# YOUNESELBOUKNIFY/Ctr_recommendation

Hardware: AMD Instinct MI355X
Metric: training samples/sec (FiBiNET d=128, MicroLens-shaped synthetic, full train step) (higher is better)
Workload: dtype bf16; 1 GPU; C3: FiBiNET emb_dim=128 + item_emb_d128, batch 8192/GPU, history 20, every GEMM operand bf16 (forward and backward) / fp32 accumulation + fp32 master weights, gradients and Adam; model=MM_FiBiNET, global_batch=8192, seq_len=20, item_rows=1250000, item_rows_per_gpu=1250000, emb_dim=128, parallelism=single, hipgraph=False, launch_mode=program

## Files before the change

ctr_recommendation_amd/_lib.py:

```python
from __future__ import annotations

import contextlib
import ctypes
import os
import struct
import threading
from typing import Optional

import torch

_HERE = os.path.dirname(os.path.abspath(__file__))
LIB_PATH = os.environ.get("FBN_LIB_PATH") or os.path.join(_HERE, "libfibinet_hip.so")

P = ctypes.c_void_p
I = ctypes.c_int
LL = ctypes.c_longlong
F = ctypes.c_float
D = ctypes.c_double
SZ = ctypes.c_size_t
U = ctypes.c_uint

SIGNATURES = {
    "fbn_version": (I, []),
    "fbn_last_error": (ctypes.c_char_p, []),
    "fbn_device_ok": (I, []),
    "fbn_gemm_workspace_size": (SZ, [I, I, I, I]),
    "fbn_gemm": (I, [P, P, P, P, I, I, I, I, I, I, I, I, I, I, I, I, I, I, F, I, I, I, P, P, SZ, P]),
    "fbn_gemm_split": (I, [P, P, P, P, I, I, I, I, I, I, I, I, I, I, I, F, P, P, SZ, P, I, I, P, I, I, P]),
    "fbn_gemm_bf16out": (I, [P, P, P, I, I, I, I, I, I, I, I, P]),
    "fbn_gemm_s3": (I, [P, P, P, I, I, I, I, I, I, I, I, LL, LL, F, P, SZ, P]),
    "fbn_gemm_bn_bwd_part_supported": (I, [I, I, I, I, I, I, I]),
    "fbn_gemm_bn_bwd_part": (I, [P, P, P, I, I, I, I, I, I, I, I, P, P, P, F, P, P]),
    "fbn_bn_tile_stats": (I, [P, I, I, P, P, P]),
    "fbn_bn_tile_moments": (I, [P, I, I, P, P]),
    "fbn_bn_moments_finalize": (I, [P, D, I, P, P, P, P, F, F, I, P]),
    "fbn_bn_tile_finalize": (I, [P, I, I, D, P, P, P, P, F, F, I, P]),
    "fbn_bn_colpart_size": (SZ, [I, I]),
    "fbn_row_chunks": (I, [I]),
    "fbn_bn_bwd_chunks": (I, [I, I]),
    "fbn_bn_bwd_fused": (I, [P, P, P, P, P, F, P, P, P, P, I, I, D, P, P, P, P, P, P, P, P, P]),
    "fbn_bn_bwd_fused_img": (I, [P, P, P, P, P, F, P, P, P, P, I, I, D, P, P, P, P, P, P, P, P, P]),
    "fbn_colsum_partial": (I, [P, I, I, I, P, P]),
    "fbn_sum_jobs": (I, [P, I, P]),
    "fbn_sum_jobs2": (I, [P, I, P, I, P]),
    "fbn_sum_jobs_sq": (I, [P, I, P, I, P, I, P, P]),
    "fbn_gemm_slabs_size": (SZ, [I, I, I]),
    "fbn_gemm_slabs": (I, [P, P, I, I, I, I, I, I, I, P, SZ, P, I, I, P, I, I, P, P]),
    "fbn_gemm_slabs_split": (I, [I, I, I]),
    "fbn_gemm_slabs_group": (I, [P, I, P]),
    "fbn_gemm_slabs_group_split": (I, [I, I, I]),
    "fbn_fields_fwd": (I, [P, P, P, P, P, P, P, F, P, I, P, LL, P, P, P, P, P, I, P, P, P, P, I, I, P, P, P, P, P, I, I, I, I,
                           P]),
    "fbn_fields_fwd_hot": (I, [P, P, P, P, P, P, P, F, P, I, P, LL, P, P, P, P, I, P, P, P, P, I, I, P, P, P, P, P,
                               I, I, I, P, P, I, P]),
    "fbn_hot_rows": (I, [P, P, I, I, LL, P, P, P, I, I, I, P]),
    "fbn_fields_bwd_partials_size": (I, [I, I, I]),
    "fbn_fields_bwd_grid": (I, [I, I]),
    "fbn_fields_bwd": (I, [P, P, P, P, P, P, P, F, P, P, P, I, I, P, P, P, P, P, P, P, P, P, P, P, P, LL, P, P, I, I,
                           I, I, P]),
    "fbn_fields_bwd_img": (I, [P, P, P, P, P, P, P, F, P, P, P, I, I, P, P, P, P, P, P, P, P, P, P, P, P, LL, P, P, I,
                               I, I, I, P]),
    "fbn_fields_bwd_slot": (I, [P, P, P, P, P, P, P, F, P, P, P, I, I, P, P, P, P, P, P, P, I, P, P, P, I, LL, P, P, P,
                                LL, I, I, I, P]),
    "fbn_pairs_fwd": (I, [P, P, P, P, I, I, I, I, I, P]),
    "fbn_pairs_bwd": (I, [P, P, P, P, P, P, P, I, I, I, I, P]),
    "fbn_pairs_fwd_img": (I, [P, P, P, P, I, I, I, P]),
    "fbn_pairs_bwd_img": (I, [P, P, P, P, P, I, I, I, P]),
    "fbn_bn_workspace_size": (SZ, [I, I]),
    "fbn_bn_stats_pass": (I, [P, I, I, P, P, P, P]),
    "fbn_bn_mean": (I, [P, D, I, P, P]),
    "fbn_bn_finalize": (I, [P, P, D, I, P, P, P, P, F, F, I, P]),
    "fbn_bn_stats": (I, [P, I, I, P, P, P, P, F, F, I, P, P]),
    "fbn_bn_eval_params": (I, [P, P, P, P, I, F, P]),
    "fbn_bn_act_fwd": (I, [P, P, I, I, P, P, P, P, F, P, U, P, P, P, P]),
    "fbn_bn_act_fwd_img": (I, [P, P, I, I, P, P, P, P, F, P, U, P, P, P, P]),
    "fbn_bn_act_head_fwd": (I, [P, P, I, I, P, P, P, P, F, P, U, P, P, P, P, P, P, P, P, P, F, P, F, P]),
    "fbn_bn_bwd_reduce": (I, [P, P, P, P, F, P, P, I, I, P, P, P]),
    "fbn_bn_bwd_apply": (I, [P, P, P, P, F, P, P, P, P, I, I, P, D, P, P, P, P, P, P, P]),
    "fbn_convert_bf16": (I, [P, I, P]),
    "fbn_bn_bwd": (I, [P, P, P, P, F, P, P, P, P, I, I, P, P, P, P, P, P]),
    "fbn_colsum_workspace_size": (SZ, [I, I]),
    "fbn_colsum": (I, [P, I, I, I, P, F, P, P]),
    "fbn_head_fwd": (I, [P, P, P, I, I, P, P, P, P, P, F, P]),
    "fbn_sigmoid_bwd": (I, [P, P, P, I, P]),
    "fbn_outer": (I, [P, P, P, I, I, P]),
    "fbn_sum": (I, [P, I, P, F, P]),
    "fbn_sumsq": (I, [P, LL, P, I, P, P]),
    "fbn_clip_coef": (I, [P, F, P, P, P]),
    "fbn_adam_dense": (I, [P, P, P, P, LL, P, P, P, F, F, F, P, F, P, P, P]),
    "fbn_sparse_fixup": (I, [P, P, P, I, I, LL, I, P, P, P, P, I, I, P]),
    "fbn_sumsq_sparse": (I, [P, P, P, I, I, I, P, P]),
    "fbn_sparse_fixup_dup": (I, [P, I, P, P, P, I, I, P]),
    "fbn_sumsq_sparse_norms": (I, [P, P, P, P, I, I, I, P, P, P, LL, P]),
    "fbn_sparse_fold_fx": (I, [P, P, I, P, P, I, I, P, P]),
    "fbn_adam_table": (I, [P, P, P, LL, I, P, P, P, P, I, P, P, P, F, F, F, I, P]),
    "fbn_adam_touched": (I, [P, P, P, I, P, P, P, P, I, I, P, P, P, F, F, F, P, P]),
    "fbn_adam_catchup": (I, [P, P, P, LL, I, P, I, P, I, I, P, P, P, F, F, F, P, P, P, LL, I, I, P]),
    "fbn_adam_claim_catchup": (I, [P, P, I, I, LL, P, P, P, P, P, P, P, P, LL, I, I, P, P, P, F, F, F, P, P, P, LL, I,
                                   I, P]),
    "fbn_adam_claim_catchup_conv": (I, [P, P, I, I, LL, P, P, P, P, P, P, P, P, LL, I, I, P, P, P, F, F, F, P, P, P,
                                        LL, I, I, P, I, P]),
    "fbn_adam_flush": (I, [P, P, P, LL, I, P, P, P, F, F, F, P, P, P, LL, I, I, P]),
    "fbn_adam_prefetch_rows": (I, [P, I, I, LL, P, P, P, P, P, I, P, P, P, F, F, F, P, P, P, LL, I, I, P]),
    "fbn_adam_prefetch": (I, [P, P, I, I, LL, P, P, P, P, P, I, P, P, P, F, F, F, P, P, P, LL, I, I, P]),
    "fbn_adam_prefetch_binned_ws_size": (SZ, [LL]),
    "fbn_adam_prefetch_binned": (I, [P, P, I, I, LL, P, P, P, P, P, I, P, P, P, F, F, F, P, P, P, LL, I, I, P, SZ, P]),
    "fbn_adam_selftest": (I, [I, ctypes.c_uint, P, P]),
    "fbn_adam_step_tail": (I, [P, P, P, P, LL, P, F, P, P, P, P, P, I, P, P, P, P, I, I, P, P, F, F, F, P, P, P, P, I,
                               LL, I, P, P, P, P, I, P, P]),
    "fbn_adam_commit": (I, [P, P, P, I, P, P, P, P, I, I, P, P, P, F, F, F, P, P, P, P, I, I, P]),
    "fbn_claim_rows": (I, [P, P, I, I, LL, P, P, P, P, P]),
    "fbn_pack_extras": (I, [P, P, P, P]),
    "fbn_unpack_extras": (I, [P, P, P, P]),
    "fbn_unpack_sumsq": (I, [P, P, P, LL, P, P]),
    "fbn_step_end": (I, [P, P, P, P, P, I, P, P]),
    "fbn_route": (I, [P, P, I, I, LL, LL, I, P, P, P, P, P, P, P]),
    "fbn_route_fc": (I, [P, P, I, I, LL, LL, I, I, P, P, P, P, P]),
    "fbn_route_fc_status": (I, [P, P, I, I, I, P, P, P]),
    "fbn_ring_slot": (I, [P, I, LL, P, P, P, I, LL, P, LL, LL, P]),
    "fbn_owner_gather_self": (I, [P, I, P, P, P, P, I, I, I, P, I, I, P]),
    "fbn_adam_owner_claim_catchup": (I, [P, I, I, P, P, P, P, P, P, LL, I, I, P, P, P, F, F, F, P, P, P, LL, I, I,
                                         P]),
    "fbn_owner_fold": (I, [P, I, I, P, P, P, I, P, LL, LL, P, I, LL, P, P, P, I, P, P, P]),
    "fbn_sumsq_flagged": (I, [P, I, P, P, I, P, P, P, I, P]),
    "fbn_owner_claim": (I, [P, I, P, P, I, P]),
    "fbn_owner_gather": (I, [P, I, P, P, P, P, I, I, I, P]),
    "fbn_widen_bf16": (I, [P, P, LL, P]),
    "fbn_pad_routes": (I, [P, P, P, I, I, P, P]),
    "fbn_compact_routes": (I, [P, I, I, P, P, P]),
    "fbn_copy_jobs": (I, [P, P, P, I, P]),
    "fbn_bilinear_supported": (I, [I]),
    "fbn_bilinear_fwd": (I, [P, P, P, I, I, I, P]),
    "fbn_bilinear_bwd": (I, [P, I, I, P, P, P, P, P, I, I, P]),
    "fbn_collate": (I, [P, I, P, P, I, I, P, P, P, P, P, LL, P, P, I, P, P, P, P, P, P, P, P, P]),
    "fbn_collate_zero_if": (I, [P, LL, P, P]),
    "fbn_eval_pack": (I, [P, P, LL, P, P, P]),
    "fbn_eval_workspace_size": (SZ, [LL]),
    "fbn_eval_reduce": (I, [P, LL, P, SZ, P, P, P]),
    "fbn_sort_u64_workspace_size": (SZ, [LL]),
    "fbn_sort_u64": (I, [P, LL, I, P, SZ, P, P]),
    "fbn_eval_pack_groups": (I, [P, LL, P, P, P]),
    "fbn_gauc_workspace_size": (SZ, [LL]),
    "fbn_gauc_reduce": (I, [P, P, LL, P, SZ, P, P, P, P]),
    "fbn_calib_workspace_size": (SZ, [LL]),
    "fbn_calib_reduce": (I, [P, LL, I, P, SZ, P, P, P]),
    "fbn_rec_item_cache": (I, [P, P, P, P, P, P, F, I, LL, P, P, I, I, P]),
    "fbn_rec_hist_pool": (I, [P, P, LL, P, P, I, I, I, P]),
    "fbn_rec_fields": (I, [P, P, P, P, P, P, I, P, LL, P, P, P, P, I, P, P, P, I, I, P, P, I, I, I, I, P]),
    "fbn_rec_topk_workspace_size": (SZ, [I, I, I]),
    "fbn_rec_topk": (I, [P, I, I, I, P, P, I, I, I, P, P, SZ, P, P, P, P, P, P]),
    "fbn_rec_rank": (I, [P, I, I, I, P, P, I, I, P, P, P, P, P]),
    "fbn_rank_hist": (I, [P, LL, P, P]),
    "fbn_rec_fields_list": (I, [P, P, P, P, P, P, I, P, LL, P, P, P, P, I, P, P, P, I, I, P, P, I, P, I, I, I, I, I, P]),
    "fbn_rec_topk_list": (I, [P, I, I, I, P, I, I, P, P, I, I, I, P, P, SZ, P, P, P, P, P, P, P]),
    "fbn_rec_rank_list": (I, [P, I, I, I, P, I, I, P, P, I, I, P, P, P, P, P]),
    "fbn_plan_create": (I, [P]),
    "fbn_plan_destroy": (I, [P]),
    "fbn_plan_size": (I, [P]),
    "fbn_plan_add_call": (I, [P, ctypes.c_char_p, P, I, P, I]),
    "fbn_plan_add_record": (I, [P, I, P]),
    "fbn_plan_add_wait": (I, [P, P, I]),
    "fbn_plan_run": (I, [P, P]),
    "fbn_plan_event_sync": (I, [P, I]),
    "fbn_probe_arm": (I, [I]),
    "fbn_probe_disarm": (I, []),
    "fbn_probe_elapsed": (F, [I]),
    "fbn_comm_load": (I, [ctypes.c_char_p]),
    "fbn_comm_id_bytes": (I, []),
    "fbn_comm_unique_id": (I, [P]),
    "fbn_comm_init": (I, [P, P, I, I]),
    "fbn_comm_destroy": (I, [P]),
    "fbn_comm_alltoallv": (I, [P, P, P, P, P, LL, P]),
    "fbn_comm_alltoall_peers": (I, [P, P, P, LL, P]),
    "fbn_comm_alltoall": (I, [P, P, P, LL, P]),
    "fbn_comm_allreduce": (I, [P, P, LL, I, P]),
    "fbn_comm_allgather": (I, [P, P, P, LL, P]),
    "fbn_sum_slices": (I, [P, I, LL, I, P, P]),
    "fbn_comm_watch": (I, [LL]),
    "fbn_comm_heartbeat": (I, [P]),
    "fbn_comm_abort": (I, [P]),
    "fbn_comm_watchdog_fired": (I, [P]),
}

FBN_SORT_TILE = 2048
FBN_GAUC_REC_WORDS = 8
FBN_CALIB_MAX_BINS = 1024
FBN_CALIB_BIN_WORDS = 8

_lib: Optional[ctypes.CDLL] = None


def lib() -> ctypes.CDLL:
    global _lib
    if _lib is None:
        if not os.path.exists(LIB_PATH):
            raise RuntimeError(
                f"{LIB_PATH} is missing: build it with `python -m ctr_recommendation_amd.build` "
                "(the FiBiNET path has no CPU fallback)")
        h = ctypes.CDLL(LIB_PATH)
        for name, (res, args) in SIGNATURES.items():
            fn = getattr(h, name)
            fn.restype = res
            fn.argtypes = args
        _lib = h
    return _lib


_fns = {}
_UNCHECKED = ("fbn_version", "fbn_device_ok", "fbn_probe_elapsed", "fbn_comm_watchdog_fired")
_tls = threading.local()


_DEBUG_SYNC = os.environ.get("FBN_DEBUG_SYNC")
_debug_log = None


def _debug_sync(name: str) -> None:
    global _debug_log
    if _debug_log is None:
        _debug_log = open(_DEBUG_SYNC, "a", buffering=1)
    _debug_log.write(name + "\n")
    torch.cuda.synchronize()


def call(name: str, *args) -> int:
    f = _fns.get(name)
    if f is None:
        f = _fns[name] = getattr(lib(), name)
    if _DEBUG_SYNC:
        _debug_sync("> " + name)
    rc = f(*args)
    if _DEBUG_SYNC:
        _debug_sync("< " + name)
    if rc and isinstance(rc, int) and name not in _UNCHECKED and not name.endswith(("_size", "_grid")):
        msg = lib().fbn_last_error().decode(errors="replace")
        raise RuntimeError(f"{name} failed (code {rc}): {msg}")
    prog = getattr(_tls, "prog", None)
    if prog is not None:
        prog.add_call(name, f, args)
    return rc


def keep(obj) -> None:
    prog = getattr(_tls, "prog", None)
    if prog is not None:
        prog.keep.append(obj)


def recording() -> bool:
    return getattr(_tls, "prog", None) is not None


def persistent(fn):
    prog = getattr(_tls, "prog", None)
    if prog is None:
        return fn()
    stream = torch.cuda.current_stream(prog.device)
    box = {}

    def run():
        try:
            torch.cuda.set_device(prog.device)
            with torch.cuda.stream(stream):
                box["out"] = fn()
        except BaseException as e:
            box["err"] = e

    t = threading.Thread(target=run, name="fbn-persistent-alloc")
    t.start()
    t.join()
    if "err" in box:
        raise box["err"]
    return box["out"]


def pool_segments(pool) -> list:
    pid = tuple(pool.id)
    out = []
    for seg in torch.cuda.memory_snapshot():
        if tuple(seg.get("segment_pool_id", ())) == pid:
            out.append((int(seg["address"]), int(seg["address"]) + int(seg["total_size"])))
    return sorted(out)


def tensors_of(obj, _seen=None, _path="", _depth=0):
    seen = set() if _seen is None else _seen
# ... 192 lines not shown
```

ctr_recommendation_amd/csrc/bilinear.hip:

```cpp
#include "common.h"
#include <algorithm>

namespace {

constexpr int TS = 16;

template <int D>
__device__ __forceinline__ int swz(int r, int k) {
  constexpr int CH = D / 8;
  return r * D + ((((k >> 3) ^ (r % CH))) << 3) + (k & 7);
}

template <int D> constexpr int nthreads() { return D >= 32 ? 2 * D : 64; }
template <int D> constexpr int row_blocks() { return D >= 32 ? 2 : 1; }

template <int D, int NT>
struct WStage {
  static constexpr int CH = D / 8, TOT = D * CH, N = (TOT + NT - 1) / NT;
  bf16x8 v[N];
  __device__ __forceinline__ void load(const short* __restrict__ src, int tid) {
#pragma unroll
    for (int j = 0; j < N; ++j)
      if (TOT % NT == 0 || tid + j * NT < TOT) v[j] = *reinterpret_cast<const bf16x8*>(src + (size_t)(tid + j * NT) * 8);
  }
  __device__ __forceinline__ void store(short* __restrict__ img, int tid) const {
#pragma unroll
    for (int j = 0; j < N; ++j) {
      const int i = tid + j * NT, r = i / CH, c = i % CH;
      if (TOT % NT == 0 || i < TOT) *reinterpret_cast<bf16x8*>(img + swz<D>(r, c * 8)) = v[j];
    }
  }
};
template <int D, int NT>
__device__ __forceinline__ void stage_w(short* __restrict__ img, const short* __restrict__ src, int tid) {
  WStage<D, NT> w;
  w.load(src, tid);
  w.store(img, tid);
}

template <int D, int NT>
__device__ __forceinline__ void stage_v(short* __restrict__ img, const short* __restrict__ V16, int b0, int ns,
                                        int tid) {
  constexpr int CH = D / 8, TOT = TS * 5 * CH, N = (TOT + NT - 1) / NT;
  const short* src = V16 + (size_t)b0 * 5 * D;
  bf16x8 v[N];
#pragma unroll
  for (int j = 0; j < N; ++j) {
    const int i = tid + j * NT, m = i / CH;
    v[j] = (bf16x8){0, 0, 0, 0, 0, 0, 0, 0};
    if ((TOT % NT == 0 || i < TOT) && m / 5 < ns) v[j] = *reinterpret_cast<const bf16x8*>(src + (size_t)i * 8);
  }
#pragma unroll
  for (int j = 0; j < N; ++j) {
    const int i = tid + j * NT, m = i / CH, c = i % CH;
    if (TOT % NT == 0 || i < TOT) *reinterpret_cast<bf16x8*>(img + swz<D>((m % 5) * TS + m / 5, c * 8)) = v[j];
  }
}

template <int D>
__device__ __forceinline__ bf16x8 frag(const short* img, int row, int k) {
  return *reinterpret_cast<const bf16x8*>(img + swz<D>(row, k));
}

template <int D>
__device__ __forceinline__ void mfma_5(f32x4 (&acc)[row_blocks<D>()][5], const short* A, const short* Bt, int w,
                                       int lane) {
  const int lr = lane & 15, lq = lane >> 4;
  if constexpr (D == 16) {
    const bf16x4 a = *reinterpret_cast<const bf16x4*>(A + swz<D>(lr, 4 * lq));
#pragma unroll
    for (int f = 0; f < 5; ++f) {
      const bf16x4 b = *reinterpret_cast<const bf16x4*>(Bt + swz<D>(f * TS + lr, 4 * lq));
      acc[0][f] = __builtin_amdgcn_mfma_f32_16x16x16bf16_1k(a, b, acc[0][f], 0, 0, 0);
    }
    return;
  }
#pragma unroll
  for (int ks = 0; ks < D / 32; ++ks) {
    bf16x8 b[5];
#pragma unroll
    for (int f = 0; f < 5; ++f) b[f] = frag<D>(Bt, f * TS + lr, 32 * ks + 8 * lq);
#pragma unroll
    for (int rb = 0; rb < 2; ++rb) {
      const bf16x8 a = frag<D>(A, 32 * w + 16 * rb + lr, 32 * ks + 8 * lq);
#pragma unroll
      for (int f = 0; f < 5; ++f) acc[rb][f] = __builtin_amdgcn_mfma_f32_16x16x32_bf16(a, b[f], acc[rb][f], 0, 0, 0);
    }
  }
}

__device__ __forceinline__ f32x4 ld_bf4(const short* p) {
  const bf16x4 t = *reinterpret_cast<const bf16x4*>(p);
  return (f32x4){bf2f(t[0]), bf2f(t[1]), bf2f(t[2]), bf2f(t[3])};
}
__device__ __forceinline__ bf16x4 to_bf4(const f32x4& v) { return (bf16x4){f2bf(v[0]), f2bf(v[1]), f2bf(v[2]), f2bf(v[3])}; }

constexpr int PI[10] = {0, 0, 0, 0, 1, 1, 1, 2, 2, 3};
constexpr int PJ[10] = {1, 2, 3, 4, 2, 3, 4, 3, 4, 4};

template <int D>
__global__ void __launch_bounds__(nthreads<D>()) bilinear_fwd_kernel(const short* __restrict__ V16,
                                                                    const short* __restrict__ WT16,
                                                                    short* __restrict__ c, int B, int ldc) {
  FBN_MAIN_PRIO();
  constexpr int NT = nthreads<D>(), RB = row_blocks<D>();
  __shared__ __attribute__((aligned(16))) short sV[5 * TS * D];
  __shared__ __attribute__((aligned(16))) short sW[D * D];
  const int tid = threadIdx.x, lane = tid & 63, w = tid >> 6;
  const int b0 = blockIdx.x * TS, ns = min(TS, B - b0);
  stage_v<D, NT>(sV, V16, b0, ns, tid);
  stage_w<D, NT>(sW, WT16, tid);
  __syncthreads();
  f32x4 acc[RB][5];
#pragma unroll
  for (int rb = 0; rb < RB; ++rb)
#pragma unroll
    for (int f = 0; f < 5; ++f) acc[rb][f] = (f32x4){0.f, 0.f, 0.f, 0.f};
  mfma_5<D>(acc, sW, sV, w, lane);
  const int s = lane & 15, lq = lane >> 4;
  if (s >= ns) return;
  short* crow = c + (size_t)(b0 + s) * ldc + 5 * D;
#pragma unroll
  for (int rb = 0; rb < RB; ++rb) {
    const int n0 = 32 * w + 16 * rb + 4 * lq;
    f32x4 v[4];
#pragma unroll
    for (int i = 0; i < 4; ++i) v[i] = ld_bf4(sV + swz<D>(i * TS + s, n0));
#pragma unroll
    for (int k = 0; k < 10; ++k) *reinterpret_cast<bf16x4*>(crow + k * D + n0) = to_bf4(v[PI[k]] * acc[rb][PJ[k]]);
  }
}

template <bool DC16>
__device__ __forceinline__ f32x4 ld_dc4(const void* __restrict__ row, int off) {
  if constexpr (DC16) return ld_bf4(reinterpret_cast<const short*>(row) + off);
  else return *reinterpret_cast<const f32x4*>(reinterpret_cast<const float*>(row) + off);
}

template <int D, bool DC16>
__global__ void __launch_bounds__(nthreads<D>(), 2) bilinear_bwd_kernel(const void* __restrict__ dc, int ldc,
                                                                       const short* __restrict__ V16,
                                                                       const short* __restrict__ WT16,
                                                                       const short* __restrict__ W16,
                                                                       float* __restrict__ dV,
                                                                       short* __restrict__ dU16, int B) {
  FBN_MAIN_PRIO();
  constexpr int NT = nthreads<D>(), RB = row_blocks<D>();
  __shared__ __attribute__((aligned(16))) short sV[5 * TS * D];
  __shared__ __attribute__((aligned(16))) short sW[D * D];
  const int tid = threadIdx.x, lane = tid & 63, w = tid >> 6;
  const int b0 = blockIdx.x * TS, ns = min(TS, B - b0);
  stage_v<D, NT>(sV, V16, b0, ns, tid);
  stage_w<D, NT>(sW, WT16, tid);
  __syncthreads();
  WStage<D, NT> wnext;
  wnext.load(W16, tid);
  f32x4 acc[RB][5];
#pragma unroll
  for (int rb = 0; rb < RB; ++rb)
#pragma unroll
    for (int f = 0; f < 5; ++f) acc[rb][f] = (f32x4){0.f, 0.f, 0.f, 0.f};
  mfma_5<D>(acc, sW, sV, w, lane);
  __syncthreads();
  const int s = lane & 15, lq = lane >> 4;
  const bool live = s < ns;
  const char* dcr = reinterpret_cast<const char*>(dc) + (size_t)(b0 + (live ? s : 0)) * ldc * (DC16 ? 2 : 4);
#pragma unroll
  for (int rb = 0; rb < RB; ++rb) {
    const int n0 = 32 * w + 16 * rb + 4 * lq;
    f32x4 v[5], gv[5], gu[5];
#pragma unroll
    for (int f = 0; f < 5; ++f) {
      v[f] = ld_bf4(sV + swz<D>(f * TS + s, n0));
      gv[f] = live ? ld_dc4<DC16>(dcr, f * D + n0) : (f32x4){0.f, 0.f, 0.f, 0.f};
      gu[f] = (f32x4){0.f, 0.f, 0.f, 0.f};
    }
#pragma unroll
    for (int k = 0; k < 10; ++k) {
      const f32x4 gp = live ? ld_dc4<DC16>(dcr, (5 + k) * D + n0) : (f32x4){0.f, 0.f, 0.f, 0.f};
      gv[PI[k]] += gp * acc[rb][PJ[k]];
      gu[PJ[k]] += gp * v[PI[k]];
    }
#pragma unroll
    for (int f = 0; f < 5; ++f) {
      const bf16x4 t = to_bf4(gu[f]);
      *reinterpret_cast<bf16x4*>(sV + swz<D>(f * TS + s, n0)) = t;
      if (live) *reinterpret_cast<bf16x4*>(dU16 + ((size_t)(b0 + s) * 5 + f) * D + n0) = t;
    }
#pragma unroll
    for (int f = 0; f < 5; ++f) acc[rb][f] = gv[f];
  }
  __syncthreads();
  wnext.store(sW, tid);
  __syncthreads();
  mfma_5<D>(acc, sW, sV, w, lane);
  if (!live) return;
#pragma unroll
  for (int rb = 0; rb < RB; ++rb) {
    const int k0 = 32 * w + 16 * rb + 4 * lq;
#pragma unroll
    for (int f = 0; f < 5; ++f) *reinterpret_cast<f32x4*>(dV + ((size_t)(b0 + s) * 5 + f) * D + k0) = acc[rb][f];
  }
}

}

extern "C" int fbn_bilinear_supported(int D) { return D == 16 || D == 32 || D == 64 || D == 128; }

extern "C" int fbn_bilinear_fwd(const short* V16, const short* WT16, short* c, int B, int D, int ldc, void* stream) {
  if (B <= 0) return FBN_OK;
  if (!V16 || !WT16 || !c || (ldc & 3) || ((uintptr_t)V16 & 15) || ((uintptr_t)WT16 & 15) || ((uintptr_t)c & 7)) {
    fbn_set_error("fbn_bilinear_fwd: bf16 V, W^T, c required; 16-B aligned V / W^T, 8-B aligned c, ldc % 4 == 0");
    return FBN_ERR_ARG;
  }
  const dim3 grid((unsigned)((B + TS - 1) / TS));
  hipStream_t st = (hipStream_t)stream;
  switch (D) {
    case 128: fbn_launch(bilinear_fwd_kernel<128>, grid, dim3(256), 0, st, V16, WT16, c, B, ldc); break;
    case 64: fbn_launch(bilinear_fwd_kernel<64>, grid, dim3(128), 0, st, V16, WT16, c, B, ldc); break;
    case 32: fbn_launch(bilinear_fwd_kernel<32>, grid, dim3(64), 0, st, V16, WT16, c, B, ldc); break;
    case 16: fbn_launch(bilinear_fwd_kernel<16>, grid, dim3(64), 0, st, V16, WT16, c, B, ldc); break;
    default: fbn_set_error("fbn_bilinear_fwd: D must be 16, 32, 64 or 128"); return FBN_ERR_UNSUPPORTED;
  }
  FBN_CHECK_LAUNCH();
  return FBN_OK;
}

extern "C" int fbn_bilinear_bwd(const void* dc, int ldc, int dc_bf16, const short* V16, const short* WT16,
                                const short* W16, float* dV, short* dU16, int B, int D, void* stream) {
  if (B <= 0) return FBN_OK;
  if (!dc || !V16 || !WT16 || !W16 || !dV || !dU16 || (ldc & 3) || ((uintptr_t)dc & 7) || ((uintptr_t)dV & 15) ||
      ((uintptr_t)V16 & 15) || ((uintptr_t)WT16 & 15) || ((uintptr_t)W16 & 15) || ((uintptr_t)dU16 & 7)) {
    fbn_set_error("fbn_bilinear_bwd: all operands required and aligned (16 B; dc, dU16 8 B), ldc % 4 == 0");
    return FBN_ERR_ARG;
  }
  const dim3 grid((unsigned)((B + TS - 1) / TS));
  hipStream_t st = (hipStream_t)stream;
  if (!dc_bf16 && ((uintptr_t)dc & 15)) { fbn_set_error("fbn_bilinear_bwd: f32 dc must be 16-B aligned"); return FBN_ERR_ARG; }
#define FBN_BILINEAR_BWD(DD, NTH)                                                                              \
  if (dc_bf16)                                                                                               \
    fbn_launch((bilinear_bwd_kernel<DD, true>), grid, dim3(NTH), 0, st, dc, ldc, V16, WT16, W16, dV, dU16, B); \
  else                                                                                                       \
    fbn_launch((bilinear_bwd_kernel<DD, false>), grid, dim3(NTH), 0, st, dc, ldc, V16, WT16, W16, dV, dU16, B)
  switch (D) {
    case 128: FBN_BILINEAR_BWD(128, 256); break;
    case 64: FBN_BILINEAR_BWD(64, 128); break;
    case 32: FBN_BILINEAR_BWD(32, 64); break;
    case 16: FBN_BILINEAR_BWD(16, 64); break;
    default: fbn_set_error("fbn_bilinear_bwd: D must be 16, 32, 64 or 128"); return FBN_ERR_UNSUPPORTED;
  }
#undef FBN_BILINEAR_BWD
  FBN_CHECK_LAUNCH();
  return FBN_OK;
}
```

ctr_recommendation_amd/csrc/fields.hip:

```cpp
#include <cstdlib>
#include "common.h"
#include "fields_common.h"

#ifndef FBN_HCH
#define FBN_HCH 10
#endif

struct FieldArgs {
  const int64_t* item_id;
  const int64_t* item_seq;
  const int64_t* likes;
  const int64_t* views;
  const float* hmm;
  const float* ln_g;
  const float* ln_b;
  const float* cate;
  const float* table;
  const int* pos;
  const float* w1; const float* b1; const float* w2; const float* b2;
  float* X;
  float* Vc;
  short* Vc16;
  void* c;
  float* a_out;
// ... 79 lines not shown
    const f32x4 c1 = *reinterpret_cast<const f32x4*>(p.cate + lk * D + 4 * q);
    const f32x4 c2 = *reinterpret_cast<const f32x4*>(p.cate + vw * D + 4 * q);
    const f32x4 h = *reinterpret_cast<const f32x4*>(p.hmm + (size_t)b * D + 4 * q);
    f32x4 rit = {0.f, 0.f, 0.f, 0.f};
    f32x4 hs = {0.f, 0.f, 0.f, 0.f};
    int nnz = 0;
    const int* pb = MODE >= 1 ? p.pos + (size_t)b * (L + 1) : nullptr;
    if (MODE == 0) {
      if (item < 0 || item >= p.V) { bad = true; item = -1; }
      if (item >= 0) rit = *reinterpret_cast<const f32x4*>(p.table + item * D + 4 * q);
    } else {
      const int pi = pb[0];
      if (pi >= 0) rit = load_row<D, MODE>(p, pi, q);
    }
    constexpr int IPL = (FBN_MAX_L + G - 1) / G;
    int sid[IPL];
#pragma unroll
    for (int j = 0; j < IPL; ++j) {
      const int t = q + j * G;
      int r = -1;
      if (t < L) {
        if (MODE == 0) {
          long long s = p.item_seq[(size_t)b * L + t];
          if (s < 0 || s >= p.V) { bad = true; s = 0; }
          r = s != 0 ? (int)s : -1;
        } else {
          r = pb[t + 1];
        }
      }
      sid[j] = r;
    }
    const int gbase = lane - q;
    if constexpr (CMP) {
      constexpr int SPB = 4 * SPW;
      __shared__ int lid[SPB][FBN_MAX_L];
      int* mine = lid[(threadIdx.x >> 6) * SPW + lane / G];
      const unsigned long long gmask = (G == 64 ? ~0ull : ((1ull << G) - 1)) << gbase;
      int nl = 0;
#pragma unroll
      for (int j = 0; j < IPL; ++j) {
        const unsigned long long mk = __ballot(sid[j] >= 0) & gmask;
        const int below = __popcll(mk & ((1ull << lane) - 1));
        if (sid[j] >= 0) mine[nl + below] = sid[j];
        nl += __popcll(mk);
      }
      __builtin_amdgcn_wave_barrier();
      __atomic_signal_fence(__ATOMIC_SEQ_CST);
      int nch = (nl + HCH - 1) / HCH;
#pragma unroll
      for (int o = 32; o > 0; o >>= 1) nch = max(nch, __shfl_xor(nch, o, 64));
      for (int c = 0; c < nch; ++c) {
        f32x4 hist[HCH];
        bool live[HCH];
#pragma unroll
        for (int u = 0; u < HCH; ++u) {
          const int k = c * HCH + u;
          live[u] = k < nl;
          const int r = mine[live[u] ? k : 0];
          if constexpr (BUF) {
            const unsigned off = live[u] ? ((unsigned)r * D + 4 * q) * 4u : 0xFFFFFFF0u;
            hist[u] = __builtin_bit_cast(f32x4, __builtin_amdgcn_raw_buffer_load_b128(rs, off, 0, 0));
          } else {
            hist[u] = load_row<D, MODE>(p, live[u] ? r : 0, q);
          }
        }
#pragma unroll
        for (int u = 0; u < HCH; ++u) hs += live[u] ? hist[u] : (f32x4){0.f, 0.f, 0.f, 0.f};
      }
      nnz = nl;
      __builtin_amdgcn_wave_barrier();
      __atomic_signal_fence(__ATOMIC_SEQ_CST);
    }
    for (int t0 = 0; t0 < (CMP ? 0 : L); t0 += HCH) {
      f32x4 hist[HCH];
      bool live[HCH];
#pragma unroll
      for (int u = 0; u < HCH; ++u) {
        const int t = t0 + u;
        int r = -1;
#pragma unroll
        for (int j = 0; j < IPL; ++j)
          if ((t / G) == j) r = __shfl(sid[j], gbase + (t % G), 64);
        live[u] = t < L && r >= 0;
        if constexpr (HOT) {
          int hi = -1;
          if (live[u] && nh > 0) {
            const unsigned h = hot_hash(r) >> (32 - __builtin_ctz(HT));
#pragma unroll
            for (int k = 0; k < 2; ++k) {
              const unsigned hk = (h + k) & (HT - 1);
              if (hi < 0 && hkey[hk] == r) hi = hval[hk];
            }
          }
          const unsigned off = (live[u] && hi < 0) ? ((unsigned)r * D + 4 * q) * 4u : 0xFFFFFFF0u;
          hist[u] = __builtin_bit_cast(f32x4, __builtin_amdgcn_raw_buffer_load_b128(rs, off, 0, 0));
          if (hi >= 0) hist[u] = hrow[hi * (D / 4) + q];
        } else if constexpr (BUF) {
          const unsigned off = live[u] ? ((unsigned)r * D + 4 * q) * 4u : 0xFFFFFFF0u;
          hist[u] = __builtin_bit_cast(f32x4, __builtin_amdgcn_raw_buffer_load_b128(rs, off, 0, 0));
        } else {
          hist[u] = load_row<D, MODE>(p, live[u] ? r : 0, q);
        }
      }
#pragma unroll
      for (int u = 0; u < HCH; ++u) {
        hs += live[u] ? hist[u] : (f32x4){0.f, 0.f, 0.f, 0.f};
        nnz += live[u] ? 1 : 0;
      }
    }
    if (bad) atomicOr(p.err, 1);

    const float cnt = fmaxf((float)nnz, 1.f);
    f32x4 x5 = hs / cnt;

    const f32x4 x4 = ln_relu<G>(h, p.ln_g, p.ln_b, p.ln_eps, q);

    const f32x4 xs[5] = {c1, c2, rit, x4, x5};
    float z[6];
    z[0] = 0.f;
#pragma unroll
    for (int f = 0; f < 5; ++f) z[f + 1] = group_sum<G>(xs[f][0] + xs[f][1] + xs[f][2] + xs[f][3]) / (float)D;
    float qv[FBN_MAXR], a[6];
    senet_excite<D>(z, p.w1, p.b1, p.w2, p.b2, p.R, qv, a);

    float* Xb = p.X + (size_t)b * 2 * D + 4 * q;
    *reinterpret_cast<f32x4*>(Xb) = rit;
    *reinterpret_cast<f32x4*>(Xb + D) = x5;
    float* Vb = p.Vc ? p.Vc + (size_t)b * 5 * D + 4 * q : nullptr;
    float* cb = (p.c && !p.c16) ? (float*)p.c + (size_t)b * p.ldc + 4 * q : nullptr;
    short* cb16 = (p.c && p.c16) ? (short*)p.c + (size_t)b * p.ldc + 4 * q : nullptr;
#pragma unroll
    for (int f = 0; f < 5; ++f) {
      const f32x4 v = xs[f] * a[f + 1];
      if (p.Vc) *reinterpret_cast<f32x4*>(Vb + f * D) = v;
      const bf16x4 v16 = (bf16x4){f2bf(v[0]), f2bf(v[1]), f2bf(v[2]), f2bf(v[3])};
      if (cb16) *reinterpret_cast<bf16x4*>(cb16 + f * D) = v16;
      else if (cb) *reinterpret_cast<f32x4*>(cb + f * D) = v;
      if (p.Vc16) *reinterpret_cast<bf16x4*>(p.Vc16 + ((size_t)b * 5 + f) * D + 4 * q) = v16;
    }
#pragma unroll
    for (int f = 0; f < 6; ++f)
      if (f % G == q) p.a_out[(size_t)b * 6 + f] = a[f];
    if (q == 0) p.cnt_out[b] = cnt;

    if (MODE == 0 && p.map) {
      for (int t = q; t <= L; t += G) {
        long long r = (t == 0) ? item : p.item_seq[(size_t)b * L + (t - 1)];
        if (r > 0 && r < p.V) map_claim(p.map, p.slot_row, (int)r, b * (L + 1) + t);
      }
    }
  }
}

struct FieldBwdArgs {
  const int64_t* item_id; const int64_t* item_seq; const int64_t* likes; const int64_t* views;
  const float* hmm; const float* ln_g;
  const float* w1; const float* b1; const float* w2;
  const float* X;
  const float* cate;
  const float* ln_b;
  const float* a;
  const float* cnt;
  const float* dV;
  float* dhmm;
  short* dhmm16;
  long long dhmm16_lo;
  float* partials;
  float* gtab; float* gvec;
  double* gnorm;
  const int* slot_step; float** slot_cell; long long ring_stride; int ring_n;
  const int* pos; void* sendbuf;
  long long V;
  int B, L, R, n_cate;
  float ln_eps;
};

template <int G>
__device__ __forceinline__ f32x4 transpose_cols(const f32x4& v, int lane) {
  const int base = lane - lane % G, q = lane % G;
  f32x4 t;
#pragma unroll
  for (int e = 0; e < 4; ++e) {
    const int src = base + e * (G / 4) + q / 4;
    const float x0 = __shfl(v[0], src, 64), x1 = __shfl(v[1], src, 64);
    const float x2 = __shfl(v[2], src, 64), x3 = __shfl(v[3], src, 64);
    const int c = q & 3;
    t[e] = c == 0 ? x0 : (c == 1 ? x1 : (c == 2 ? x2 : x3));
  }
  return t;
}
template <int G>
__device__ __forceinline__ void atomic_add_row_t(float* row, const f32x4& t, int q) {
  atomicAdd(row + q, t[0]); atomicAdd(row + G + q, t[1]); atomicAdd(row + 2 * G + q, t[2]);
  atomicAdd(row + 3 * G + q, t[3]);
}

template <int D, int MODE, int RMAX, bool SLOT = false>
__global__ void __launch_bounds__(256) fields_bwd_kernel(FieldBwdArgs p) {
  FBN_MAIN_PRIO();
  constexpr int G = D / 4;
  constexpr int SPW = 64 / G;
  constexpr int NPMAX = 13 * RMAX + 6;
  constexpr int SJ = (NPMAX + G - 1) / G;
  extern __shared__ __attribute__((aligned(16))) float sp[];
  const int R = p.R;
  const int NP = 13 * R + 6;
  const int P = NP + 3 * D + p.n_cate * D;
  const int wave = threadIdx.x >> 6;
  float* ws = sp + wave * P;
  float* sv = sp + 4 * P + (wave * SPW + (threadIdx.x & 63) / G) * (12 + 2 * RMAX);
  for (int i = threadIdx.x; i < 4 * P; i += blockDim.x) sp[i] = 0.f;
  __syncthreads();
  float* w_lg = ws + NP;
  float* w_ct = w_lg + 2 * D;
  float* w_hb = w_ct + p.n_cate * D;

  const int lane = threadIdx.x & 63;
  const int q = lane % G, grp = lane / G;
  const int gw = (blockIdx.x * blockDim.x + threadIdx.x) >> 6;
  const int nwaves = (gridDim.x * blockDim.x) >> 6;
  const int L = p.L;
  float* gvec = p.gvec;
  if constexpr (SLOT) {
    gvec += (size_t)(__builtin_amdgcn_readfirstlane(*p.slot_step) % p.ring_n) * p.ring_stride;
    if (blockIdx.x == 0 && threadIdx.x == 0) *p.slot_cell = gvec;
  }
  f32x4 acc_lg = {0.f, 0.f, 0.f, 0.f}, acc_lb = {0.f, 0.f, 0.f, 0.f}, acc_hb = {0.f, 0.f, 0.f, 0.f};
  float acc_se[SJ];
#pragma unroll
  for (int j = 0; j < SJ; ++j) acc_se[j] = 0.f;

  for (int b0 = gw * SPW; b0 < p.B; b0 += nwaves * SPW) {
    const int b = b0 + grp;
    const bool live = b < p.B;
    f32x4 dx0 = {0.f, 0.f, 0.f, 0.f}, dx1 = {0.f, 0.f, 0.f, 0.f};
    long long lk = -1, vw = -1;
    if (live) {
      const float* Xb = p.X + (size_t)b * 2 * D + 4 * q;
      const float* dVb = p.dV + (size_t)b * 5 * D + 4 * q;
      f32x4 x[5], dv[5];
      lk = p.likes[b];
      vw = p.views[b];
      const long long lkc = (lk >= 0 && lk < p.n_cate) ? lk : 0, vwc = (vw >= 0 && vw < p.n_cate) ? vw : 0;
      x[0] = *reinterpret_cast<const f32x4*>(p.cate + lkc * D + 4 * q);
      x[1] = *reinterpret_cast<const f32x4*>(p.cate + vwc * D + 4 * q);
      x[2] = *reinterpret_cast<const f32x4*>(Xb);
      x[4] = *reinterpret_cast<const f32x4*>(Xb + D);
#pragma unroll
      for (int f = 0; f < 5; ++f) dv[f] = *reinterpret_cast<const f32x4*>(dVb + f * D);
      const f32x4 h = *reinterpret_cast<const f32x4*>(p.hmm + (size_t)b * D + 4 * q);
      x[3] = ln_relu<G>(h, p.ln_g, p.ln_b, p.ln_eps, q);
      float a[6];
#pragma unroll
      for (int f = 0; f < 6; ++f) a[f] = p.a[(size_t)b * 6 + f];
      float z[6];
      z[0] = 0.f;
#pragma unroll
      for (int f = 0; f < 5; ++f) z[f + 1] = group_sum<G>(x[f][0] + x[f][1] + x[f][2] + x[f][3]) / (float)D;
      float qv[RMAX], rj[RMAX], dq[RMAX];
#pragma unroll
      for (int j = 0; j < RMAX; ++j) {
        float s = 0.f;
        if (j < R) {
          s = p.b1[j];
#pragma unroll
          for (int f = 0; f < 6; ++f) s += p.w1[j * 6 + f] * z[f];
        }
        qv[j] = s;
        rj[j] = fmaxf(s, 0.f);
      }
      float ds[6];
      ds[0] = 0.f;
#pragma unroll
      for (int f = 0; f < 5; ++f) {
        const float da = group_sum<G>(dv[f][0] * x[f][0] + dv[f][1] * x[f][1] + dv[f][2] * x[f][2] + dv[f][3] * x[f][3]);
        ds[f + 1] = da * (1.f - a[f + 1]) * a[f + 1];
      }
      float dz[6] = {0.f, 0.f, 0.f, 0.f, 0.f, 0.f};
#pragma unroll
      for (int j = 0; j < RMAX; ++j) {
        float dr = 0.f;
        if (j < R) {
#pragma unroll
          for (int f = 0; f < 6; ++f) dr += p.w2[f * R + j] * ds[f];
        }
        dq[j] = (j < R && qv[j] > 0.f) ? dr : 0.f;
        if (j < R) {
#pragma unroll
          for (int f = 0; f < 6; ++f) dz[f] += p.w1[j * 6 + f] * dq[j];
        }
      }
      if (q == 0) {
#pragma unroll
        for (int f = 0; f < 6; ++f) { sv[f] = ds[f]; sv[6 + f] = z[f]; }
#pragma unroll
        for (int jj = 0; jj < RMAX; ++jj) { sv[12 + jj] = dq[jj]; sv[12 + RMAX + jj] = rj[jj]; }
      }
      __builtin_amdgcn_wave_barrier();
#pragma unroll
      for (int j = 0; j < SJ; ++j) {
        const int k = q + j * G;
        float v = 0.f;
        if (k < 6 * R) v = sv[12 + k / 6] * sv[6 + k % 6];
        else if (k < 7 * R) v = sv[12 + (k - 6 * R)];
        else if (k < 13 * R) v = sv[(k - 7 * R) / R] * sv[12 + RMAX + (k - 7 * R) % R];
        else if (k < NP) v = sv[k - 13 * R];
        acc_se[j] += v;
      }
      __builtin_amdgcn_wave_barrier();
      f32x4 dx[5];
#pragma unroll
      for (int f = 0; f < 5; ++f) dx[f] = dv[f] * a[f + 1] + dz[f + 1] / (float)D;
      dx0 = dx[0];
      dx1 = dx[1];

      {
        const float mean = group_sum<G>(h[0] + h[1] + h[2] + h[3]) / (float)D;
        const f32x4 dh = h - mean;
        const float s2 = group_sum<G>(dh[0] * dh[0] + dh[1] * dh[1] + dh[2] * dh[2] + dh[3] * dh[3]);
        const float rstd = 1.f / sqrtf(s2 / (float)D + p.ln_eps);
        const f32x4 gam = *reinterpret_cast<const f32x4*>(p.ln_g + 4 * q);
        f32x4 gl, xh, gx;
#pragma unroll
        for (int e = 0; e < 4; ++e) {
          gl[e] = x[3][e] > 0.f ? dx[3][e] : 0.f;
          xh[e] = dh[e] * rstd;
          gx[e] = gl[e] * gam[e];
          acc_lg[e] += gl[e] * xh[e];
          acc_lb[e] += gl[e];
        }
        const float m1 = group_sum<G>(gx[0] + gx[1] + gx[2] + gx[3]) / (float)D;
        const float m2 = group_sum<G>(gx[0] * xh[0] + gx[1] * xh[1] + gx[2] * xh[2] + gx[3] * xh[3]) / (float)D;
        f32x4 out;
#pragma unroll
        for (int e = 0; e < 4; ++e) out[e] = rstd * (gx[e] - m1 - xh[e] * m2);
        *reinterpret_cast<f32x4*>(p.dhmm + (size_t)b * D + 4 * q) = out;
        acc_hb += out;
        if (p.dhmm16) {
          const bf16x4 hi = (bf16x4){f2bf(out[0]), f2bf(out[1]), f2bf(out[2]), f2bf(out[3])};
          *reinterpret_cast<bf16x4*>(p.dhmm16 + (size_t)b * D + 4 * q) = hi;
          if (p.dhmm16_lo)
            *reinterpret_cast<bf16x4*>(p.dhmm16 + p.dhmm16_lo + (size_t)b * D + 4 * q) =
                (bf16x4){f2bf(out[0] - bf2f(hi[0])), f2bf(out[1] - bf2f(hi[1])), f2bf(out[2] - bf2f(hi[2])),
                         f2bf(out[3] - bf2f(hi[3]))};
        }
      }
      const f32x4 gh = dx[4] / p.cnt[b];
      if (MODE == 0 && p.gvec) {
        *reinterpret_cast<f32x4*>(gvec + (size_t)b * 2 * D + 4 * q) = dx[2];
        *reinterpret_cast<f32x4*>(gvec + ((size_t)b * 2 + 1) * D + 4 * q) = gh;
        if (p.gnorm) {
          double si = 0.0, sh = 0.0;
#pragma unroll
          for (int e = 0; e < 4; ++e) {
            si += (double)(dx[2][e] * dx[2][e]);
            sh += (double)(gh[e] * gh[e]);
          }
#pragma unroll
          for (int o = G / 2; o > 0; o >>= 1) {
            si += __shfl_xor(si, o, 64);
            sh += __shfl_xor(sh, o, 64);
          }
          if (q == 0) {
            p.gnorm[(size_t)b * 2] = si;
            p.gnorm[(size_t)b * 2 + 1] = sh;
          }
        }
      } else if (MODE == 0) {
        const f32x4 ti = transpose_cols<G>(dx[2], lane);
        const f32x4 th = transpose_cols<G>(gh, lane);
        const long long item = p.item_id[b];
        if (item > 0 && item < p.V) atomic_add_row_t<G>(p.gtab + item * D, ti, q);
        for (int t = 0; t < L; ++t) {
          const long long s = p.item_seq[(size_t)b * L + t];
          if (s > 0 && s < p.V) atomic_add_row_t<G>(p.gtab + s * D, th, q);
        }
      } else {
        const int* pb = p.pos + (size_t)b * (L + 1);
        auto put = [&](int row, const f32x4& x) {
          if constexpr (MODE == 2) {
            *reinterpret_cast<bf16x4*>(reinterpret_cast<short*>(p.sendbuf) + (size_t)row * D + 4 * q) =
                (bf16x4){f2bf(x[0]), f2bf(x[1]), f2bf(x[2]), f2bf(x[3])};
          } else {
            *reinterpret_cast<f32x4*>(reinterpret_cast<float*>(p.sendbuf) + (size_t)row * D + 4 * q) = x;
          }
        };
        if (pb[0] >= 0) put(pb[0], dx[2]);
        for (int t = 0; t < L; ++t)
          if (pb[t + 1] >= 0) put(pb[t + 1], gh);
      }
    }
#pragma unroll
    for (int gi = 0; gi < SPW; ++gi) {
      if (grp == gi && live) {
        if (lk >= 0 && lk < p.n_cate) {
          f32x4* c = reinterpret_cast<f32x4*>(w_ct + lk * D + 4 * q);
          *c = *c + dx0;
        }
        if (vw >= 0 && vw < p.n_cate) {
          f32x4* c = reinterpret_cast<f32x4*>(w_ct + vw * D + 4 * q);
          *c = *c + dx1;
        }
      }
    }
  }
#pragma unroll
  for (int o = G; o < 64; o <<= 1) {
#pragma unroll
    for (int e = 0; e < 4; ++e) {
      acc_lg[e] += __shfl_xor(acc_lg[e], o, 64);
      acc_lb[e] += __shfl_xor(acc_lb[e], o, 64);
      acc_hb[e] += __shfl_xor(acc_hb[e], o, 64);
    }
#pragma unroll
    for (int j = 0; j < SJ; ++j) acc_se[j] += __shfl_xor(acc_se[j], o, 64);
  }
  if (grp == 0) {
    *reinterpret_cast<f32x4*>(w_lg + 4 * q) = acc_lg;
    *reinterpret_cast<f32x4*>(w_lg + D + 4 * q) = acc_lb;
    *reinterpret_cast<f32x4*>(w_hb + 4 * q) = acc_hb;
#pragma unroll
    for (int j = 0; j < SJ; ++j) {
      const int k = q + j * G;
      if (k < NP) ws[k] = acc_se[j];
    }
  }
  __syncthreads();
  float* out = p.partials + (size_t)blockIdx.x * P;
  for (int i = threadIdx.x; i < P; i += blockDim.x) out[i] = (sp[i] + sp[P + i]) + (sp[2 * P + i] + sp[3 * P + i]);
}

struct GradOuts {
  float* p[8];
  int off[9];
};
__global__ void __launch_bounds__(1024) reduce_partials_one16(const float* __restrict__ part, int nblk, int P, GradOuts o) {
  __shared__ float red[64][16];
  const int col = threadIdx.x & 15, str = threadIdx.x >> 4;
  const int i = blockIdx.x * 16 + col;
  float s = 0.f;
  if (i < P)
    for (int r = str; r < nblk; r += 64) s += part[(size_t)r * P + i];
  red[str][col] = s;
  __syncthreads();
  if (threadIdx.x < 16 && i < P) {
    float t = 0.f;
    for (int k = 0; k < 64; ++k) t += red[k][col];
    int seg = 0;
#pragma unroll
    for (int j = 1; j < 8; ++j) seg += (i >= o.off[j]) ? 1 : 0;
    if (o.p[seg]) o.p[seg][i - o.off[seg]] = t;
  }
}


#ifndef FBN_FB_MAXBLK
#define FBN_FB_MAXBLK 512
#endif
static int fields_grid(int B, int D, int cap = 1024) {
  const int spw = 64 / (D / 4);
  const int waves = (B + spw - 1) / spw;
  int blocks = (waves + 3) / 4;
  return blocks < 1 ? 1 : (blocks > cap ? cap : blocks);
}

template <int MODE, int HCH, bool BUF, bool HOT = false, bool CMP = false>
static int launch_fields_fwd_hb(const FieldArgs& a, int D, hipStream_t st) {
  const int grid = fields_grid(a.B, D, HOT ? 256 : 1024);
  switch (D) {
    case 16: fbn_launch((fields_fwd_kernel<16, MODE, HCH, BUF, HOT, CMP>), dim3(grid), dim3(256), 0, st, a); break;
    case 32: fbn_launch((fields_fwd_kernel<32, MODE, HCH, BUF, HOT, CMP>), dim3(grid), dim3(256), 0, st, a); break;
    case 64: fbn_launch((fields_fwd_kernel<64, MODE, HCH, BUF, HOT, CMP>), dim3(grid), dim3(256), 0, st, a); break;
    case 128: fbn_launch((fields_fwd_kernel<128, MODE, HCH, BUF, HOT, CMP>), dim3(grid), dim3(256), 0, st, a); break;
    case 256: fbn_launch((fields_fwd_kernel<256, MODE, HCH, BUF, HOT, CMP>), dim3(grid), dim3(256), 0, st, a); break;
    default: fbn_set_error("fields: embedding_dim must be one of 16,32,64,128,256"); return FBN_ERR_UNSUPPORTED;
  }
  FBN_CHECK_LAUNCH();
  return FBN_OK;
}

template <int MODE, int HCH, bool CMP>
static int launch_fields_fwd_h(const FieldArgs& a, int D, hipStream_t st) {
  if constexpr (MODE == 0) {
    if (a.hot) return launch_fields_fwd_hb<0, HCH, true, true>(a, D, st);
    if ((unsigned long long)a.V * D * 4 < 0xFFFFFF00ull)
      return launch_fields_fwd_hb<0, HCH, true, false, CMP>(a, D, st);
  }
  return launch_fields_fwd_hb<MODE, HCH, false, false, CMP>(a, D, st);
}

template <int MODE>
static int launch_fields_fwd(const FieldArgs& a, int D, hipStream_t st) {
  const char* he = getenv("FBN_FIELDS_HCH");
  const int hch = he ? atoi(he) : FBN_HCH;
  const char* ce = getenv("FBN_FIELDS_CMP");
  if (ce && atoi(ce) == 1) {
    if (hch == 10) return launch_fields_fwd_h<MODE, 10, true>(a, D, st);
    if (hch == 8) return launch_fields_fwd_h<MODE, 8, true>(a, D, st);
    return launch_fields_fwd_h<MODE, 5, true>(a, D, st);
  }
  if (hch == 20) return launch_fields_fwd_h<MODE, 20, false>(a, D, st);
  if (hch == 5) return launch_fields_fwd_h<MODE, 5, false>(a, D, st);
  return launch_fields_fwd_h<MODE, 10, false>(a, D, st);
}

static int fields_fwd_impl(const int64_t* item_id, const int64_t* item_seq, const int64_t* likes,
                           const int64_t* views, const float* hmm, const float* ln_g, const float* ln_b,
                           float ln_eps, const float* cate, int n_cate, const float* table, long long V,
                           const int* pos, const float* w1, const float* b1, const float* w2,
                           const float* b2, int R, float* X, float* Vc, short* Vc16, void* c, int ldc, int c_bf16,
                           float* a_out, float* cnt_out, int* err, int* map, int* slot_row, int B, int L,
                           int D, int rows_bf16, const int* hot, const int* hot_n, int H, void* stream);

extern "C" int fbn_fields_fwd(const int64_t* item_id, const int64_t* item_seq, const int64_t* likes,
                              const int64_t* views, const float* hmm, const float* ln_g, const float* ln_b,
                              float ln_eps, const float* cate, int n_cate, const float* table, long long V,
                              const int* pos, const float* w1, const float* b1, const float* w2,
                              const float* b2, int R, float* X, float* Vc, short* Vc16, void* c, int ldc, int c_bf16,
                              float* a_out,
                              float* cnt_out, int* err, int* map, int* slot_row, int B, int L,
                              int D, int rows_bf16, void* stream) {
  return fields_fwd_impl(item_id, item_seq, likes, views, hmm, ln_g, ln_b, ln_eps, cate, n_cate, table, V, pos, w1,
                         b1, w2, b2, R, X, Vc, Vc16, c, ldc, c_bf16, a_out, cnt_out, err, map, slot_row, B, L, D,
                         rows_bf16, nullptr, nullptr, 0, stream);
}

extern "C" int fbn_fields_fwd_hot(const int64_t* item_id, const int64_t* item_seq, const int64_t* likes,
                                  const int64_t* views, const float* hmm, const float* ln_g, const float* ln_b,
                                  float ln_eps, const float* cate, int n_cate, const float* table, long long V,
                                  const float* w1, const float* b1, const float* w2, const float* b2, int R, float* X,
                                  float* Vc, short* Vc16, void* c, int ldc, int c_bf16, float* a_out, float* cnt_out,
                                  int* err, int* map, int* slot_row, int B, int L, int D, const int* hot,
                                  const int* hot_n, int H, void* stream) {
  if (!hot || !hot_n || (unsigned long long)V * D * 4 >= 0xFFFFFF00ull) {
    fbn_set_error("fbn_fields_fwd_hot: needs the hot list and a table under 4 GB");
    return FBN_ERR_ARG;
  }
  return fields_fwd_impl(item_id, item_seq, likes, views, hmm, ln_g, ln_b, ln_eps, cate, n_cate, table, V, nullptr,
                         w1, b1, w2, b2, R, X, Vc, Vc16, c, ldc, c_bf16, a_out, cnt_out, err, map, slot_row, B, L, D, 0,
                         hot, hot_n, H, stream);
}

__global__ void hot_rows_kernel(const int64_t* __restrict__ item, const int64_t* __restrict__ seq, int B, int L,
                                long long V, int* __restrict__ cnt, int* __restrict__ hot, int* __restrict__ hot_n,
                                int H, int tau, int clear) {
  const long long i = (long long)blockIdx.x * blockDim.x + threadIdx.x;
  if (clear && i == 0) *hot_n = 0;
  if (i >= (long long)B * (L + 1)) return;
  const long long b = i / (L + 1), t = i - b * (L + 1);
  const long long id = t == 0 ? item[b] : seq[b * L + (t - 1)];
  if (id <= 0 || id >= V) return;
  if (clear) {
    cnt[id] = 0;
    return;
  }
  if (atomicAdd(cnt + id, 1) == tau - 1) {
    const int s = atomicAdd(hot_n, 1);
    if (s < H) hot[s] = (int)id;
  }
}

extern "C" int fbn_hot_rows(const int64_t* item, const int64_t* seq, int B, int L, long long V, int* cnt, int* hot,
                            int* hot_n, int H, int tau, int clear, void* stream) {
  const long long n = (long long)B * (L + 1);
  if (n <= 0) return FBN_OK;
  fbn_launch(hot_rows_kernel, dim3((unsigned)((n + 255) / 256)), dim3(256), 0, (hipStream_t)stream, item,
                     L > 0 ? seq : nullptr, B, L, V, cnt, hot, hot_n, H, tau < 1 ? 1 : tau, clear);
  FBN_CHECK_LAUNCH();
  return FBN_OK;
}

static int fields_fwd_impl(const int64_t* item_id, const int64_t* item_seq, const int64_t* likes,
                           const int64_t* views, const float* hmm, const float* ln_g, const float* ln_b,
                           float ln_eps, const float* cate, int n_cate, const float* table, long long V,
                           const int* pos, const float* w1, const float* b1, const float* w2,
                           const float* b2, int R, float* X, float* Vc, short* Vc16, void* c, int ldc, int c_bf16,
                           float* a_out, float* cnt_out, int* err, int* map, int* slot_row, int B, int L,
                           int D, int rows_bf16, const int* hot, const int* hot_n, int H, void* stream) {
  if (B <= 0) return FBN_OK;
  if (L < 0 || L > 32 || R < 1 || R > FBN_MAXR || (ldc & 3)) {
    fbn_set_error("fbn_fields_fwd: need 0 <= L <= 32, 1 <= R <= 8, ldc % 4 == 0");
    return FBN_ERR_ARG;
  }
  FieldArgs a;
  a.item_id = item_id; a.item_seq = L > 0 ? item_seq : nullptr; a.likes = likes; a.views = views;
  a.hmm = hmm; a.ln_g = ln_g; a.ln_b = ln_b; a.cate = cate; a.table = table; a.pos = pos;
  a.w1 = w1; a.b1 = b1; a.w2 = w2; a.b2 = b2;
  a.X = X; a.Vc = Vc; a.Vc16 = Vc16; a.c = c; a.a_out = a_out; a.cnt_out = cnt_out; a.err = err;
  a.map = map; a.slot_row = slot_row;
  a.V = V; a.B = B; a.L = L; a.ldc = ldc; a.R = R; a.n_cate = n_cate; a.ln_eps = ln_eps; a.c16 = c_bf16;
  a.hot = hot; a.hot_n = hot_n; a.H = H;
  if (pos && rows_bf16) return launch_fields_fwd<2>(a, D, (hipStream_t)stream);
  if (pos) return launch_fields_fwd<1>(a, D, (hipStream_t)stream);
  return launch_fields_fwd<0>(a, D, (hipStream_t)stream);
}

extern "C" int fbn_fields_bwd_partials_size(int D, int R, int n_cate) { return 13 * R + 6 + 3 * D + n_cate * D; }
extern "C" int fbn_fields_bwd_grid(int B, int D) { return fields_grid(B, D, FBN_FB_MAXBLK); }

template <int MODE, int RMAX, bool SLOT = false>
static int launch_fields_bwd_r(const FieldBwdArgs& a, int D, hipStream_t st) {
  const int grid = fields_grid(a.B, D, FBN_FB_MAXBLK);
  const size_t lds = (4 * (size_t)(13 * a.R + 6 + 3 * D + a.n_cate * D) + 4 * (64 / (D / 4)) * (12 + 2 * RMAX)) *
                     sizeof(float);
  switch (D) {
    case 16: fbn_launch((fields_bwd_kernel<16, MODE, RMAX, SLOT>), dim3(grid), dim3(256), lds, st, a); break;
    case 32: fbn_launch((fields_bwd_kernel<32, MODE, RMAX, SLOT>), dim3(grid), dim3(256), lds, st, a); break;
    case 64: fbn_launch((fields_bwd_kernel<64, MODE, RMAX, SLOT>), dim3(grid), dim3(256), lds, st, a); break;
    case 128: fbn_launch((fields_bwd_kernel<128, MODE, RMAX, SLOT>), dim3(grid), dim3(256), lds, st, a); break;
    case 256: fbn_launch((fields_bwd_kernel<256, MODE, RMAX, SLOT>), dim3(grid), dim3(256), lds, st, a); break;
    default: fbn_set_error("fields: embedding_dim must be one of 16,32,64,128,256"); return FBN_ERR_UNSUPPORTED;
  }
  FBN_CHECK_LAUNCH();
  return FBN_OK;
}

template <int MODE>
static int launch_fields_bwd(const FieldBwdArgs& a, int D, hipStream_t st) {
  if constexpr (MODE == 0)
    if (a.slot_step)
      return a.R <= 3 ? launch_fields_bwd_r<0, 3, true>(a, D, st) : launch_fields_bwd_r<0, FBN_MAXR, true>(a, D, st);
  return a.R <= 3 ? launch_fields_bwd_r<MODE, 3>(a, D, st) : launch_fields_bwd_r<MODE, FBN_MAXR>(a, D, st);
}

static int fields_bwd_impl(const int64_t* item_id, const int64_t* item_seq, const int64_t* likes,
                           const int64_t* views, const float* hmm, const float* ln_g, const float* ln_b,
                           float ln_eps, const float* w1, const float* b1, const float* w2, int R, int n_cate,
                           const float* cate, const float* X, const float* a, const float* cnt, const float* dV,
                           float* dhmm, short* dhmm16, float* partials, float* const* param_grads, float* gtab,
                           float* gvec, double* gnorm, long long V, const int* pos, void* sendbuf, int send_bf16,
                           int B, int L, int D, void* stream, long long dhmm16_lo, const int* slot_step = nullptr,
                           void* slot_cell = nullptr, int ring_n = 0, long long ring_stride = 0);
extern "C" int fbn_fields_bwd(const int64_t* item_id, const int64_t* item_seq, const int64_t* likes,
                              const int64_t* views, const float* hmm, const float* ln_g, const float* ln_b,
                              float ln_eps, const float* w1, const float* b1, const float* w2, int R, int n_cate,
                              const float* cate, const float* X, const float* a, const float* cnt, const float* dV, float* dhmm,
                              short* dhmm16, float* partials, float* const* param_grads, float* gtab, float* gvec,
                              double* gnorm, long long V, const int* pos, void* sendbuf, int send_bf16, int B,
                              int L, int D, void* stream) {
  return fields_bwd_impl(item_id, item_seq, likes, views, hmm, ln_g, ln_b, ln_eps, w1, b1, w2, R, n_cate, cate, X, a,
                         cnt, dV, dhmm, dhmm16, partials, param_grads, gtab, gvec, gnorm, V, pos, sendbuf, send_bf16, B,
                         L, D, stream, 0);
}
extern "C" int fbn_fields_bwd_img(const int64_t* item_id, const int64_t* item_seq, const int64_t* likes,
                                  const int64_t* views, const float* hmm, const float* ln_g, const float* ln_b,
                                  float ln_eps, const float* w1, const float* b1, const float* w2, int R, int n_cate,
                                  const float* cate, const float* X, const float* a, const float* cnt, const float* dV,
                                  float* dhmm, void* dhmm_img, float* partials, float* const* param_grads,
                                  float* gtab, float* gvec, double* gnorm, long long V, const int* pos, void* sendbuf,
                                  int send_bf16, int B, int L, int D, void* stream) {
  if (!dhmm_img) { fbn_set_error("fbn_fields_bwd_img: dhmm_img"); return FBN_ERR_ARG; }
  return fields_bwd_impl(item_id, item_seq, likes, views, hmm, ln_g, ln_b, ln_eps, w1, b1, w2, R, n_cate, cate, X, a,
                         cnt, dV, dhmm, (short*)dhmm_img, partials, param_grads, gtab, gvec, gnorm, V, pos, sendbuf,
                         send_bf16, B, L, D, stream, (long long)B * D);
}
extern "C" int fbn_fields_bwd_slot(const int64_t* item_id, const int64_t* item_seq, const int64_t* likes,
                                   const int64_t* views, const float* hmm, const float* ln_g, const float* ln_b,
                                   float ln_eps, const float* w1, const float* b1, const float* w2, int R, int n_cate,
                                   const float* cate, const float* X, const float* a, const float* cnt, const float* dV,
                                   float* dhmm, void* dhmm16, int dhmm_is_img, float* partials,
                                   float* const* param_grads, float* ring, int ring_n, long long ring_stride,
                                   const int* step, void* cell, double* gnorm, long long V, int B, int L, int D,
                                   void* stream) {
  if (!ring || !step || !cell || ring_n < 1 || ring_stride < (long long)B * 2 * D || (ring_stride & 3) ||
      ((uintptr_t)ring & 15) || (dhmm_is_img && !dhmm16)) {
    fbn_set_error("fbn_fields_bwd_slot: ring (16-B aligned), step, cell; ring_n >= 1, ring_stride >= B*2*D, % 4 == 0");
    return FBN_ERR_ARG;
  }
  return fields_bwd_impl(item_id, item_seq, likes, views, hmm, ln_g, ln_b, ln_eps, w1, b1, w2, R, n_cate, cate, X, a,
                         cnt, dV, dhmm, (short*)dhmm16, partials, param_grads, nullptr, ring, gnorm, V, nullptr, nullptr,
                         0, B, L, D, stream, dhmm_is_img ? (long long)B * D : 0, step, cell, ring_n, ring_stride);
}
static int fields_bwd_impl(const int64_t* item_id, const int64_t* item_seq, const int64_t* likes,
                           const int64_t* views, const float* hmm, const float* ln_g, const float* ln_b,
                           float ln_eps, const float* w1, const float* b1, const float* w2, int R, int n_cate,
                           const float* cate, const float* X, const float* a, const float* cnt, const float* dV,
                           float* dhmm, short* dhmm16, float* partials, float* const* param_grads, float* gtab,
                           float* gvec, double* gnorm, long long V, const int* pos, void* sendbuf, int send_bf16,
                           int B, int L, int D, void* stream, long long dhmm16_lo, const int* slot_step,
                           void* slot_cell, int ring_n, long long ring_stride) {
  if (B <= 0) return FBN_OK;
  if (L < 0 || L > 32 || R < 1 || R > FBN_MAXR) { fbn_set_error("fbn_fields_bwd: bad L/R"); return FBN_ERR_ARG; }
  FieldBwdArgs p;
  p.item_id = item_id; p.item_seq = L > 0 ? item_seq : nullptr; p.likes = likes; p.views = views;
  p.hmm = hmm; p.ln_g = ln_g; p.ln_b = ln_b; p.w1 = w1; p.b1 = b1; p.w2 = w2; p.cate = cate;
  p.X = X; p.a = a; p.cnt = cnt; p.dV = dV; p.dhmm = dhmm; p.dhmm16 = dhmm16; p.partials = partials;
  p.dhmm16_lo = dhmm16_lo;
  p.slot_step = slot_step; p.slot_cell = (float**)slot_cell; p.ring_n = ring_n; p.ring_stride = ring_stride;
  p.gtab = gtab; p.gvec = gvec; p.gnorm = gvec ? gnorm : nullptr; p.pos = pos; p.sendbuf = sendbuf;
  p.V = V; p.B = B; p.L = L; p.R = R; p.n_cate = n_cate; p.ln_eps = ln_eps;
  hipStream_t st = (hipStream_t)stream;
  int rc = !pos ? launch_fields_bwd<0>(p, D, st) : send_bf16 ? launch_fields_bwd<2>(p, D, st)
                                                               : launch_fields_bwd<1>(p, D, st);
  if (rc) return rc;
  if (!param_grads) return FBN_OK;
  const int P = 13 * R + 6 + 3 * D + n_cate * D;
  const int nblk = fields_grid(B, D, FBN_FB_MAXBLK);

  GradOuts o;
  const int sizes[8] = {6 * R, R, 6 * R, 6, D, D, n_cate * D, D};
  o.off[0] = 0;
  for (int j = 0; j < 8; ++j) {
    if (j < 7 && !param_grads[j]) {
      fbn_set_error("fbn_fields_bwd: null parameter-gradient destination");
      return FBN_ERR_ARG;
    }
    o.p[j] = param_grads[j];
    o.off[j + 1] = o.off[j] + sizes[j];
  }
  fbn_launch(reduce_partials_one16, dim3(fbn_cdiv(P, 16)), dim3(1024), 0, st, (const float*)partials, nblk, P, o);
  FBN_CHECK_LAUNCH();
  return FBN_OK;
}
```

ctr_recommendation_amd/csrc/fields_common.h:

```cpp
#pragma once
#include "common.h"

#define FBN_MAXR 8
#define FBN_MAX_L 32

template <int G>
__device__ __forceinline__ f32x4 ln_relu(const f32x4& h, const float* ln_g, const float* ln_b, float eps, int q) {
  constexpr int D = 4 * G;
  const float s1 = group_sum<G>(h[0] + h[1] + h[2] + h[3]);
  const float mean = s1 / (float)D;
  const f32x4 dh = h - mean;
  const float s2 = group_sum<G>(dh[0] * dh[0] + dh[1] * dh[1] + dh[2] * dh[2] + dh[3] * dh[3]);
  const float rstd = 1.f / sqrtf(s2 / (float)D + eps);
  const f32x4 g4 = *reinterpret_cast<const f32x4*>(ln_g + 4 * q);
  const f32x4 bb4 = *reinterpret_cast<const f32x4*>(ln_b + 4 * q);
  f32x4 x4;
#pragma unroll
  for (int e = 0; e < 4; ++e) x4[e] = fmaxf(dh[e] * rstd * g4[e] + bb4[e], 0.f);
  return x4;
}

template <int D>
__device__ __forceinline__ void senet_excite(const float (&z)[6], const float* w1, const float* b1,
                                             const float* w2, const float* b2, int R, float (&q)[FBN_MAXR],
                                             float (&a)[6]) {
  for (int j = 0; j < R; ++j) {
    float s = b1[j];
#pragma unroll
    for (int f = 0; f < 6; ++f) s += w1[j * 6 + f] * z[f];
    q[j] = s;
  }
#pragma unroll
  for (int f = 0; f < 6; ++f) {
    float s = b2[f];
    for (int j = 0; j < R; ++j) s += w2[f * R + j] * fmaxf(q[j], 0.f);
    a[f] = 1.f / (1.f + __expf(-s));
  }
}
```

ctr_recommendation_amd/csrc/plan_thunks.inc:

```

static int th_fbn_adam_catchup(const uint64_t* i, const double* f) {
  return fbn_adam_catchup(reinterpret_cast<float*>(static_cast<uintptr_t>(i[0])),
      reinterpret_cast<float*>(static_cast<uintptr_t>(i[1])),
      reinterpret_cast<float*>(static_cast<uintptr_t>(i[2])),
      static_cast<long long>(i[3]),
      static_cast<int>(i[4]),
      reinterpret_cast<const int*>(static_cast<uintptr_t>(i[5])),
      static_cast<int>(i[6]),
      reinterpret_cast<const int*>(static_cast<uintptr_t>(i[7])),
      static_cast<int>(i[8]),
      static_cast<int>(i[9]),
      reinterpret_cast<int*>(static_cast<uintptr_t>(i[10])),
      reinterpret_cast<const void*>(static_cast<uintptr_t>(i[11])),
      reinterpret_cast<const int*>(static_cast<uintptr_t>(i[12])),
      plan_f32(f[0]),
      plan_f32(f[1]),
      plan_f32(f[2]),
      reinterpret_cast<int*>(static_cast<uintptr_t>(i[13])),
      reinterpret_cast<const float*>(static_cast<uintptr_t>(i[14])),
      reinterpret_cast<const float*>(static_cast<uintptr_t>(i[15])),
      static_cast<long long>(i[16]),
      static_cast<int>(i[17]),
      static_cast<int>(i[18]),
      reinterpret_cast<void*>(static_cast<uintptr_t>(i[19])));
// ... 182 lines not shown
  return fbn_adam_prefetch_binned(reinterpret_cast<const int64_t*>(static_cast<uintptr_t>(i[0])),
      reinterpret_cast<const int64_t*>(static_cast<uintptr_t>(i[1])),
      static_cast<int>(i[2]),
      static_cast<int>(i[3]),
      static_cast<long long>(i[4]),
      reinterpret_cast<const int*>(static_cast<uintptr_t>(i[5])),
      reinterpret_cast<unsigned long long*>(static_cast<uintptr_t>(i[6])),
      reinterpret_cast<float*>(static_cast<uintptr_t>(i[7])),
      reinterpret_cast<float*>(static_cast<uintptr_t>(i[8])),
      reinterpret_cast<float*>(static_cast<uintptr_t>(i[9])),
      static_cast<int>(i[10]),
      reinterpret_cast<int*>(static_cast<uintptr_t>(i[11])),
      reinterpret_cast<const void*>(static_cast<uintptr_t>(i[12])),
      reinterpret_cast<const int*>(static_cast<uintptr_t>(i[13])),
      plan_f32(f[0]),
      plan_f32(f[1]),
      plan_f32(f[2]),
      reinterpret_cast<int*>(static_cast<uintptr_t>(i[14])),
      reinterpret_cast<const float*>(static_cast<uintptr_t>(i[15])),
      reinterpret_cast<const float*>(static_cast<uintptr_t>(i[16])),
      static_cast<long long>(i[17]),
      static_cast<int>(i[18]),
      static_cast<int>(i[19]),
      reinterpret_cast<void*>(static_cast<uintptr_t>(i[20])),
      static_cast<size_t>(i[21]),
      reinterpret_cast<void*>(static_cast<uintptr_t>(i[22])));
}
static int th_fbn_adam_prefetch_rows(const uint64_t* i, const double* f) {
  return fbn_adam_prefetch_rows(reinterpret_cast<const int*>(static_cast<uintptr_t>(i[0])),
      static_cast<int>(i[1]),
      static_cast<int>(i[2]),
      static_cast<long long>(i[3]),
      reinterpret_cast<const int*>(static_cast<uintptr_t>(i[4])),
      reinterpret_cast<unsigned long long*>(static_cast<uintptr_t>(i[5])),
      reinterpret_cast<float*>(static_cast<uintptr_t>(i[6])),
      reinterpret_cast<float*>(static_cast<uintptr_t>(i[7])),
      reinterpret_cast<float*>(static_cast<uintptr_t>(i[8])),
      static_cast<int>(i[9]),
      reinterpret_cast<int*>(static_cast<uintptr_t>(i[10])),
      reinterpret_cast<const void*>(static_cast<uintptr_t>(i[11])),
      reinterpret_cast<const int*>(static_cast<uintptr_t>(i[12])),
      plan_f32(f[0]),
      plan_f32(f[1]),
      plan_f32(f[2]),
      reinterpret_cast<int*>(static_cast<uintptr_t>(i[13])),
      reinterpret_cast<const float*>(static_cast<uintptr_t>(i[14])),
      reinterpret_cast<const float*>(static_cast<uintptr_t>(i[15])),
      static_cast<long long>(i[16]),
      static_cast<int>(i[17]),
      static_cast<int>(i[18]),
      reinterpret_cast<void*>(static_cast<uintptr_t>(i[19])));
}
static int th_fbn_adam_selftest(const uint64_t* i, const double* f) {
  (void)f;
  return fbn_adam_selftest(static_cast<int>(i[0]),
      static_cast<unsigned>(i[1]),
      reinterpret_cast<unsigned long long*>(static_cast<uintptr_t>(i[2])),
      reinterpret_cast<void*>(static_cast<uintptr_t>(i[3])));
}
static int th_fbn_adam_step_tail(const uint64_t* i, const double* f) {
  return fbn_adam_step_tail(reinterpret_cast<float*>(static_cast<uintptr_t>(i[0])),
      reinterpret_cast<const float*>(static_cast<uintptr_t>(i[1])),
      reinterpret_cast<float*>(static_cast<uintptr_t>(i[2])),
      reinterpret_cast<float*>(static_cast<uintptr_t>(i[3])),
      static_cast<long long>(i[4]),
      reinterpret_cast<const double*>(static_cast<uintptr_t>(i[5])),
      plan_f32(f[0]),
      reinterpret_cast<float*>(static_cast<uintptr_t>(i[6])),
      reinterpret_cast<float*>(static_cast<uintptr_t>(i[7])),
      reinterpret_cast<float*>(static_cast<uintptr_t>(i[8])),
      reinterpret_cast<float*>(static_cast<uintptr_t>(i[9])),
      reinterpret_cast<float*>(static_cast<uintptr_t>(i[10])),
      static_cast<int>(i[11]),
      reinterpret_cast<int*>(static_cast<uintptr_t>(i[12])),
      reinterpret_cast<const float*>(static_cast<uintptr_t>(i[13])),
      reinterpret_cast<float*>(static_cast<uintptr_t>(i[14])),
      reinterpret_cast<int*>(static_cast<uintptr_t>(i[15])),
      static_cast<int>(i[16]),
      static_cast<int>(i[17]),
      reinterpret_cast<const void*>(static_cast<uintptr_t>(i[18])),
      reinterpret_cast<int*>(static_cast<uintptr_t>(i[19])),
      plan_f32(f[1]),
      plan_f32(f[2]),
      plan_f32(f[3]),
      reinterpret_cast<int*>(static_cast<uintptr_t>(i[20])),
      reinterpret_cast<int*>(static_cast<uintptr_t>(i[21])),
      reinterpret_cast<float*>(static_cast<uintptr_t>(i[22])),
      reinterpret_cast<float*>(static_cast<uintptr_t>(i[23])),
      static_cast<int>(i[24]),
      static_cast<long long>(i[25]),
      static_cast<int>(i[26]),
      reinterpret_cast<unsigned long long*>(static_cast<uintptr_t>(i[27])),
      reinterpret_cast<long long*>(static_cast<uintptr_t>(i[28])),
      reinterpret_cast<long long*>(static_cast<uintptr_t>(i[29])),
      reinterpret_cast<unsigned*>(static_cast<uintptr_t>(i[30])),
      static_cast<int>(i[31]),
      reinterpret_cast<int*>(static_cast<uintptr_t>(i[32])),
      reinterpret_cast<void*>(static_cast<uintptr_t>(i[33])));
}
static int th_fbn_adam_table(const uint64_t* i, const double* f) {
  return fbn_adam_table(reinterpret_cast<float*>(static_cast<uintptr_t>(i[0])),
      reinterpret_cast<float*>(static_cast<uintptr_t>(i[1])),
      reinterpret_cast<float*>(static_cast<uintptr_t>(i[2])),
      static_cast<long long>(i[3]),
      static_cast<int>(i[4]),
      reinterpret_cast<int*>(static_cast<uintptr_t>(i[5])),
      reinterpret_cast<const float*>(static_cast<uintptr_t>(i[6])),
      reinterpret_cast<float*>(static_cast<uintptr_t>(i[7])),
      reinterpret_cast<int*>(static_cast<uintptr_t>(i[8])),
      static_cast<int>(i[9]),
      reinterpret_cast<const float*>(static_cast<uintptr_t>(i[10])),
      reinterpret_cast<const void*>(static_cast<uintptr_t>(i[11])),
      reinterpret_cast<const int*>(static_cast<uintptr_t>(i[12])),
      plan_f32(f[0]),
      plan_f32(f[1]),
      plan_f32(f[2]),
      static_cast<int>(i[13]),
      reinterpret_cast<void*>(static_cast<uintptr_t>(i[14])));
}
static int th_fbn_adam_touched(const uint64_t* i, const double* f) {
  return fbn_adam_touched(reinterpret_cast<float*>(static_cast<uintptr_t>(i[0])),
      reinterpret_cast<float*>(static_cast<uintptr_t>(i[1])),
      reinterpret_cast<float*>(static_cast<uintptr_t>(i[2])),
      static_cast<int>(i[3]),
      reinterpret_cast<int*>(static_cast<uintptr_t>(i[4])),
      reinterpret_cast<const float*>(static_cast<uintptr_t>(i[5])),
      reinterpret_cast<float*>(static_cast<uintptr_t>(i[6])),
      reinterpret_cast<int*>(static_cast<uintptr_t>(i[7])),
      static_cast<int>(i[8]),
      static_cast<int>(i[9]),
      reinterpret_cast<const float*>(static_cast<uintptr_t>(i[10])),
      reinterpret_cast<const void*>(static_cast<uintptr_t>(i[11])),
      reinterpret_cast<const int*>(static_cast<uintptr_t>(i[12])),
      plan_f32(f[0]),
      plan_f32(f[1]),
      plan_f32(f[2]),
      reinterpret_cast<int*>(static_cast<uintptr_t>(i[13])),
      reinterpret_cast<void*>(static_cast<uintptr_t>(i[14])));
}
static int th_fbn_bilinear_bwd(const uint64_t* i, const double* f) {
  (void)f;
  return fbn_bilinear_bwd(reinterpret_cast<const void*>(static_cast<uintptr_t>(i[0])),
      static_cast<int>(i[1]),
      static_cast<int>(i[2]),
      reinterpret_cast<const short*>(static_cast<uintptr_t>(i[3])),
      reinterpret_cast<const short*>(static_cast<uintptr_t>(i[4])),
      reinterpret_cast<const short*>(static_cast<uintptr_t>(i[5])),
      reinterpret_cast<float*>(static_cast<uintptr_t>(i[6])),
      reinterpret_cast<short*>(static_cast<uintptr_t>(i[7])),
      static_cast<int>(i[8]),
      static_cast<int>(i[9]),
      reinterpret_cast<void*>(static_cast<uintptr_t>(i[10])));
}
static int th_fbn_bilinear_fwd(const uint64_t* i, const double* f) {
  (void)f;
  return fbn_bilinear_fwd(reinterpret_cast<const short*>(static_cast<uintptr_t>(i[0])),
      reinterpret_cast<const short*>(static_cast<uintptr_t>(i[1])),
      reinterpret_cast<short*>(static_cast<uintptr_t>(i[2])),
      static_cast<int>(i[3]),
      static_cast<int>(i[4]),
      static_cast<int>(i[5]),
      reinterpret_cast<void*>(static_cast<uintptr_t>(i[6])));
}
static int th_fbn_bilinear_supported(const uint64_t* i, const double* f) {
  (void)f;
  return fbn_bilinear_supported(static_cast<int>(i[0]));
}
static int th_fbn_bn_act_fwd(const uint64_t* i, const double* f) {
  return fbn_bn_act_fwd(reinterpret_cast<const float*>(static_cast<uintptr_t>(i[0])),
      reinterpret_cast<float*>(static_cast<uintptr_t>(i[1])),
      static_cast<int>(i[2]),
      static_cast<int>(i[3]),
      reinterpret_cast<const float*>(static_cast<uintptr_t>(i[4])),
      reinterpret_cast<const float*>(static_cast<uintptr_t>(i[5])),
      reinterpret_cast<const float*>(static_cast<uintptr_t>(i[6])),
      reinterpret_cast<const float*>(static_cast<uintptr_t>(i[7])),
      plan_f32(f[0]),
      reinterpret_cast<const unsigned long long*>(static_cast<uintptr_t>(i[8])),
      static_cast<unsigned>(i[9]),
      reinterpret_cast<unsigned char*>(static_cast<uintptr_t>(i[10])),
      reinterpret_cast<const unsigned char*>(static_cast<uintptr_t>(i[11])),
      reinterpret_cast<short*>(static_cast<uintptr_t>(i[12])),
      reinterpret_cast<void*>(static_cast<uintptr_t>(i[13])));
}
static int th_fbn_bn_act_fwd_img(const uint64_t* i, const double* f) {
  return fbn_bn_act_fwd_img(reinterpret_cast<const float*>(static_cast<uintptr_t>(i[0])),
      reinterpret_cast<float*>(static_cast<uintptr_t>(i[1])),
      static_cast<int>(i[2]),
      static_cast<int>(i[3]),
      reinterpret_cast<const float*>(static_cast<uintptr_t>(i[4])),
      reinterpret_cast<const float*>(static_cast<uintptr_t>(i[5])),
      reinterpret_cast<const float*>(static_cast<uintptr_t>(i[6])),
      reinterpret_cast<const float*>(static_cast<uintptr_t>(i[7])),
      plan_f32(f[0]),
      reinterpret_cast<const unsigned long long*>(static_cast<uintptr_t>(i[8])),
      static_cast<unsigned>(i[9]),
      reinterpret_cast<unsigned char*>(static_cast<uintptr_t>(i[10])),
      reinterpret_cast<const unsigned char*>(static_cast<uintptr_t>(i[11])),
      reinterpret_cast<void*>(static_cast<uintptr_t>(i[12])),
      reinterpret_cast<void*>(static_cast<uintptr_t>(i[13])));
}
static int th_fbn_bn_act_head_fwd(const uint64_t* i, const double* f) {
  return fbn_bn_act_head_fwd(reinterpret_cast<const float*>(static_cast<uintptr_t>(i[0])),
      reinterpret_cast<float*>(static_cast<uintptr_t>(i[1])),
      static_cast<int>(i[2]),
      static_cast<int>(i[3]),
      reinterpret_cast<const float*>(static_cast<uintptr_t>(i[4])),
      reinterpret_cast<const float*>(static_cast<uintptr_t>(i[5])),
      reinterpret_cast<const float*>(static_cast<uintptr_t>(i[6])),
      reinterpret_cast<const float*>(static_cast<uintptr_t>(i[7])),
      plan_f32(f[0]),
      reinterpret_cast<const unsigned long long*>(static_cast<uintptr_t>(i[8])),
      static_cast<unsigned>(i[9]),
      reinterpret_cast<unsigned char*>(static_cast<uintptr_t>(i[10])),
      reinterpret_cast<const unsigned char*>(static_cast<uintptr_t>(i[11])),
      reinterpret_cast<const float*>(static_cast<uintptr_t>(i[12])),
      reinterpret_cast<const float*>(static_cast<uintptr_t>(i[13])),
      reinterpret_cast<float*>(static_cast<uintptr_t>(i[14])),
      reinterpret_cast<float*>(static_cast<uintptr_t>(i[15])),
      reinterpret_cast<const float*>(static_cast<uintptr_t>(i[16])),
      reinterpret_cast<float*>(static_cast<uintptr_t>(i[17])),
      reinterpret_cast<float*>(static_cast<uintptr_t>(i[18])),
      plan_f32(f[1]),
      reinterpret_cast<double*>(static_cast<uintptr_t>(i[19])),
      plan_f32(f[2]),
      reinterpret_cast<void*>(static_cast<uintptr_t>(i[20])));
}
static int th_fbn_bn_bwd(const uint64_t* i, const double* f) {
  return fbn_bn_bwd(reinterpret_cast<const float*>(static_cast<uintptr_t>(i[0])),
      reinterpret_cast<const float*>(static_cast<uintptr_t>(i[1])),
      reinterpret_cast<const float*>(static_cast<uintptr_t>(i[2])),
      reinterpret_cast<const float*>(static_cast<uintptr_t>(i[3])),
      plan_f32(f[0]),
      reinterpret_cast<const float*>(static_cast<uintptr_t>(i[4])),
      reinterpret_cast<const float*>(static_cast<uintptr_t>(i[5])),
      reinterpret_cast<const float*>(static_cast<uintptr_t>(i[6])),
      reinterpret_cast<const float*>(static_cast<uintptr_t>(i[7])),
      static_cast<int>(i[8]),
      static_cast<int>(i[9]),
      reinterpret_cast<float*>(static_cast<uintptr_t>(i[10])),
      reinterpret_cast<float*>(static_cast<uintptr_t>(i[11])),
      reinterpret_cast<float*>(static_cast<uintptr_t>(i[12])),
      reinterpret_cast<float*>(static_cast<uintptr_t>(i[13])),
      reinterpret_cast<void*>(static_cast<uintptr_t>(i[14])),
      reinterpret_cast<void*>(static_cast<uintptr_t>(i[15])));
}
static int th_fbn_bn_bwd_apply(const uint64_t* i, const double* f) {
  return fbn_bn_bwd_apply(reinterpret_cast<const float*>(static_cast<uintptr_t>(i[0])),
      reinterpret_cast<const float*>(static_cast<uintptr_t>(i[1])),
      reinterpret_cast<const float*>(static_cast<uintptr_t>(i[2])),
      reinterpret_cast<const float*>(static_cast<uintptr_t>(i[3])),
      plan_f32(f[0]),
      reinterpret_cast<const float*>(static_cast<uintptr_t>(i[4])),
      reinterpret_cast<const float*>(static_cast<uintptr_t>(i[5])),
      reinterpret_cast<const float*>(static_cast<uintptr_t>(i[6])),
      reinterpret_cast<const float*>(static_cast<uintptr_t>(i[7])),
      static_cast<int>(i[8]),
      static_cast<int>(i[9]),
      reinterpret_cast<const double*>(static_cast<uintptr_t>(i[10])),
      f[1],
      reinterpret_cast<float*>(static_cast<uintptr_t>(i[11])),
      reinterpret_cast<short*>(static_cast<uintptr_t>(i[12])),
      reinterpret_cast<float*>(static_cast<uintptr_t>(i[13])),
      reinterpret_cast<float*>(static_cast<uintptr_t>(i[14])),
      reinterpret_cast<float*>(static_cast<uintptr_t>(i[15])),
      reinterpret_cast<void*>(static_cast<uintptr_t>(i[16])),
      reinterpret_cast<void*>(static_cast<uintptr_t>(i[17])));
}
static int th_fbn_bn_bwd_chunks(const uint64_t* i, const double* f) {
  (void)f;
  return fbn_bn_bwd_chunks(static_cast<int>(i[0]),
      static_cast<int>(i[1]));
}
static int th_fbn_bn_bwd_fused(const uint64_t* i, const double* f) {
  return fbn_bn_bwd_fused(reinterpret_cast<const float*>(static_cast<uintptr_t>(i[0])),
      reinterpret_cast<const float*>(static_cast<uintptr_t>(i[1])),
      reinterpret_cast<const float*>(static_cast<uintptr_t>(i[2])),
      reinterpret_cast<const float*>(static_cast<uintptr_t>(i[3])),
      reinterpret_cast<const short*>(static_cast<uintptr_t>(i[4])),
      plan_f32(f[0]),
      reinterpret_cast<const float*>(static_cast<uintptr_t>(i[5])),
      reinterpret_cast<const float*>(static_cast<uintptr_t>(i[6])),
      reinterpret_cast<const float*>(static_cast<uintptr_t>(i[7])),
      reinterpret_cast<const float*>(static_cast<uintptr_t>(i[8])),
      static_cast<int>(i[9]),
      static_cast<int>(i[10]),
      f[1],
      reinterpret_cast<float*>(static_cast<uintptr_t>(i[11])),
      reinterpret_cast<short*>(static_cast<uintptr_t>(i[12])),
      reinterpret_cast<float*>(static_cast<uintptr_t>(i[13])),
      reinterpret_cast<float*>(static_cast<uintptr_t>(i[14])),
      reinterpret_cast<float*>(static_cast<uintptr_t>(i[15])),
      reinterpret_cast<float*>(static_cast<uintptr_t>(i[16])),
      reinterpret_cast<const double*>(static_cast<uintptr_t>(i[17])),
      reinterpret_cast<void*>(static_cast<uintptr_t>(i[18])),
      reinterpret_cast<void*>(static_cast<uintptr_t>(i[19])));
}
static int th_fbn_bn_bwd_fused_img(const uint64_t* i, const double* f) {
  return fbn_bn_bwd_fused_img(reinterpret_cast<const float*>(static_cast<uintptr_t>(i[0])),
      reinterpret_cast<const float*>(static_cast<uintptr_t>(i[1])),
      reinterpret_cast<const float*>(static_cast<uintptr_t>(i[2])),
      reinterpret_cast<const float*>(static_cast<uintptr_t>(i[3])),
      reinterpret_cast<const short*>(static_cast<uintptr_t>(i[4])),
      plan_f32(f[0]),
      reinterpret_cast<const float*>(static_cast<uintptr_t>(i[5])),
      reinterpret_cast<const float*>(static_cast<uintptr_t>(i[6])),
// ... 1144 lines not shown
      static_cast<int>(i[2]),
      reinterpret_cast<const float*>(static_cast<uintptr_t>(i[3])),
      reinterpret_cast<int*>(static_cast<uintptr_t>(i[4])),
      static_cast<int>(i[5]),
      static_cast<int>(i[6]),
      reinterpret_cast<unsigned long long*>(static_cast<uintptr_t>(i[7])),
      reinterpret_cast<void*>(static_cast<uintptr_t>(i[8])));
}
static int th_fbn_step_end(const uint64_t* i, const double* f) {
  (void)f;
  return fbn_step_end(reinterpret_cast<int*>(static_cast<uintptr_t>(i[0])),
      reinterpret_cast<unsigned long long*>(static_cast<uintptr_t>(i[1])),
      reinterpret_cast<double*>(static_cast<uintptr_t>(i[2])),
      reinterpret_cast<long long*>(static_cast<uintptr_t>(i[3])),
      reinterpret_cast<long long*>(static_cast<uintptr_t>(i[4])),
      static_cast<int>(i[5]),
      reinterpret_cast<int*>(static_cast<uintptr_t>(i[6])),
      reinterpret_cast<void*>(static_cast<uintptr_t>(i[7])));
}
static int th_fbn_sum(const uint64_t* i, const double* f) {
  return fbn_sum(reinterpret_cast<const float*>(static_cast<uintptr_t>(i[0])),
      static_cast<int>(i[1]),
      reinterpret_cast<float*>(static_cast<uintptr_t>(i[2])),
      plan_f32(f[0]),
      reinterpret_cast<void*>(static_cast<uintptr_t>(i[3])));
}
static int th_fbn_sum_jobs(const uint64_t* i, const double* f) {
  (void)f;
  return fbn_sum_jobs(reinterpret_cast<const void*>(static_cast<uintptr_t>(i[0])),
      static_cast<int>(i[1]),
      reinterpret_cast<void*>(static_cast<uintptr_t>(i[2])));
}
static int th_fbn_sum_jobs2(const uint64_t* i, const double* f) {
  (void)f;
  return fbn_sum_jobs2(reinterpret_cast<const void*>(static_cast<uintptr_t>(i[0])),
      static_cast<int>(i[1]),
      reinterpret_cast<const void*>(static_cast<uintptr_t>(i[2])),
      static_cast<int>(i[3]),
      reinterpret_cast<void*>(static_cast<uintptr_t>(i[4])));
}
static int th_fbn_sum_jobs_sq(const uint64_t* i, const double* f) {
  (void)f;
  return fbn_sum_jobs_sq(reinterpret_cast<const void*>(static_cast<uintptr_t>(i[0])),
      static_cast<int>(i[1]),
      reinterpret_cast<const void*>(static_cast<uintptr_t>(i[2])),
      static_cast<int>(i[3]),
      reinterpret_cast<const void*>(static_cast<uintptr_t>(i[4])),
      static_cast<int>(i[5]),
      reinterpret_cast<double*>(static_cast<uintptr_t>(i[6])),
      reinterpret_cast<void*>(static_cast<uintptr_t>(i[7])));
}
static int th_fbn_sum_slices(const uint64_t* i, const double* f) {
  (void)f;
  return fbn_sum_slices(reinterpret_cast<const void*>(static_cast<uintptr_t>(i[0])),
      static_cast<int>(i[1]),
      static_cast<long long>(i[2]),
      static_cast<int>(i[3]),
      reinterpret_cast<void*>(static_cast<uintptr_t>(i[4])),
      reinterpret_cast<void*>(static_cast<uintptr_t>(i[5])));
}
static int th_fbn_sumsq(const uint64_t* i, const double* f) {
  (void)f;
  return fbn_sumsq(reinterpret_cast<const float*>(static_cast<uintptr_t>(i[0])),
      static_cast<long long>(i[1]),
      reinterpret_cast<const int*>(static_cast<uintptr_t>(i[2])),
      static_cast<int>(i[3]),
      reinterpret_cast<double*>(static_cast<uintptr_t>(i[4])),
      reinterpret_cast<void*>(static_cast<uintptr_t>(i[5])));
}
static int th_fbn_sumsq_flagged(const uint64_t* i, const double* f) {
  (void)f;
  return fbn_sumsq_flagged(reinterpret_cast<const int*>(static_cast<uintptr_t>(i[0])),
      static_cast<int>(i[1]),
      reinterpret_cast<const void*>(static_cast<uintptr_t>(i[2])),
      reinterpret_cast<float*>(static_cast<uintptr_t>(i[3])),
      static_cast<int>(i[4]),
      reinterpret_cast<const double*>(static_cast<uintptr_t>(i[5])),
      reinterpret_cast<double*>(static_cast<uintptr_t>(i[6])),
      reinterpret_cast<unsigned long long*>(static_cast<uintptr_t>(i[7])),
      static_cast<int>(i[8]),
      reinterpret_cast<void*>(static_cast<uintptr_t>(i[9])));
}
static int th_fbn_sumsq_sparse(const uint64_t* i, const double* f) {
  (void)f;
  return fbn_sumsq_sparse(reinterpret_cast<const float*>(static_cast<uintptr_t>(i[0])),
      reinterpret_cast<float*>(static_cast<uintptr_t>(i[1])),
      reinterpret_cast<int*>(static_cast<uintptr_t>(i[2])),
      static_cast<int>(i[3]),
      static_cast<int>(i[4]),
      static_cast<int>(i[5]),
      reinterpret_cast<double*>(static_cast<uintptr_t>(i[6])),
      reinterpret_cast<void*>(static_cast<uintptr_t>(i[7])));
}
static int th_fbn_sumsq_sparse_norms(const uint64_t* i, const double* f) {
  (void)f;
  return fbn_sumsq_sparse_norms(reinterpret_cast<const double*>(static_cast<uintptr_t>(i[0])),
      reinterpret_cast<const float*>(static_cast<uintptr_t>(i[1])),
      reinterpret_cast<float*>(static_cast<uintptr_t>(i[2])),
      reinterpret_cast<int*>(static_cast<uintptr_t>(i[3])),
      static_cast<int>(i[4]),
      static_cast<int>(i[5]),
      static_cast<int>(i[6]),
      reinterpret_cast<double*>(static_cast<uintptr_t>(i[7])),
      reinterpret_cast<unsigned long long*>(static_cast<uintptr_t>(i[8])),
      reinterpret_cast<const float*>(static_cast<uintptr_t>(i[9])),
      static_cast<long long>(i[10]),
      reinterpret_cast<void*>(static_cast<uintptr_t>(i[11])));
}
static int th_fbn_unpack_extras(const uint64_t* i, const double* f) {
  (void)f;
  return fbn_unpack_extras(reinterpret_cast<const float*>(static_cast<uintptr_t>(i[0])),
      reinterpret_cast<float*>(static_cast<uintptr_t>(i[1])),
      reinterpret_cast<double*>(static_cast<uintptr_t>(i[2])),
      reinterpret_cast<void*>(static_cast<uintptr_t>(i[3])));
}
static int th_fbn_unpack_sumsq(const uint64_t* i, const double* f) {
  (void)f;
  return fbn_unpack_sumsq(reinterpret_cast<const float*>(static_cast<uintptr_t>(i[0])),
      reinterpret_cast<float*>(static_cast<uintptr_t>(i[1])),
      reinterpret_cast<const float*>(static_cast<uintptr_t>(i[2])),
      static_cast<long long>(i[3]),
      reinterpret_cast<double*>(static_cast<uintptr_t>(i[4])),
      reinterpret_cast<void*>(static_cast<uintptr_t>(i[5])));
}
static int th_fbn_version(const uint64_t* i, const double* f) {
  (void)i;
  (void)f;
  return fbn_version();
}
static int th_fbn_widen_bf16(const uint64_t* i, const double* f) {
  (void)f;
  return fbn_widen_bf16(reinterpret_cast<const void*>(static_cast<uintptr_t>(i[0])),
      reinterpret_cast<float*>(static_cast<uintptr_t>(i[1])),
      static_cast<long long>(i[2]),
      reinterpret_cast<void*>(static_cast<uintptr_t>(i[3])));
}

static const PlanThunk kPlanThunks[] = {
    {"fbn_adam_catchup", th_fbn_adam_catchup, 20, 3},
    {"fbn_adam_claim_catchup", th_fbn_adam_claim_catchup, 26, 3},
    {"fbn_adam_claim_catchup_conv", th_fbn_adam_claim_catchup_conv, 28, 3},
    {"fbn_adam_commit", th_fbn_adam_commit, 20, 3},
    {"fbn_adam_dense", th_fbn_adam_dense, 12, 4},
    {"fbn_adam_flush", th_fbn_adam_flush, 15, 3},
    {"fbn_adam_owner_claim_catchup", th_fbn_adam_owner_claim_catchup, 22, 3},
    {"fbn_adam_prefetch", th_fbn_adam_prefetch, 21, 3},
    {"fbn_adam_prefetch_binned", th_fbn_adam_prefetch_binned, 23, 3},
    {"fbn_adam_prefetch_rows", th_fbn_adam_prefetch_rows, 20, 3},
    {"fbn_adam_selftest", th_fbn_adam_selftest, 4, 0},
    {"fbn_adam_step_tail", th_fbn_adam_step_tail, 34, 4},
    {"fbn_adam_table", th_fbn_adam_table, 15, 3},
    {"fbn_adam_touched", th_fbn_adam_touched, 15, 3},
    {"fbn_bilinear_bwd", th_fbn_bilinear_bwd, 11, 0},
    {"fbn_bilinear_fwd", th_fbn_bilinear_fwd, 7, 0},
    {"fbn_bilinear_supported", th_fbn_bilinear_supported, 1, 0},
    {"fbn_bn_act_fwd", th_fbn_bn_act_fwd, 14, 1},
    {"fbn_bn_act_fwd_img", th_fbn_bn_act_fwd_img, 14, 1},
    {"fbn_bn_act_head_fwd", th_fbn_bn_act_head_fwd, 21, 3},
    {"fbn_bn_bwd", th_fbn_bn_bwd, 16, 1},
    {"fbn_bn_bwd_apply", th_fbn_bn_bwd_apply, 18, 2},
    {"fbn_bn_bwd_chunks", th_fbn_bn_bwd_chunks, 2, 0},
    {"fbn_bn_bwd_fused", th_fbn_bn_bwd_fused, 20, 2},
    {"fbn_bn_bwd_fused_img", th_fbn_bn_bwd_fused_img, 20, 2},
    {"fbn_bn_bwd_reduce", th_fbn_bn_bwd_reduce, 11, 1},
    {"fbn_bn_eval_params", th_fbn_bn_eval_params, 6, 1},
    {"fbn_bn_finalize", th_fbn_bn_finalize, 9, 3},
    {"fbn_bn_mean", th_fbn_bn_mean, 4, 1},
    {"fbn_bn_moments_finalize", th_fbn_bn_moments_finalize, 8, 3},
    {"fbn_bn_stats", th_fbn_bn_stats, 10, 2},
    {"fbn_bn_stats_pass", th_fbn_bn_stats_pass, 7, 0},
    {"fbn_bn_tile_finalize", th_fbn_bn_tile_finalize, 9, 3},
    {"fbn_bn_tile_moments", th_fbn_bn_tile_moments, 5, 0},
    {"fbn_bn_tile_stats", th_fbn_bn_tile_stats, 6, 0},
    {"fbn_calib_reduce", th_fbn_calib_reduce, 8, 0},
    {"fbn_claim_rows", th_fbn_claim_rows, 10, 0},
    {"fbn_clip_coef", th_fbn_clip_coef, 4, 1},
    {"fbn_collate", th_fbn_collate, 24, 0},
    {"fbn_collate_zero_if", th_fbn_collate_zero_if, 4, 0},
    {"fbn_colsum", th_fbn_colsum, 7, 1},
    {"fbn_colsum_partial", th_fbn_colsum_partial, 6, 0},
    {"fbn_comm_allgather", th_fbn_comm_allgather, 5, 0},
    {"fbn_comm_allreduce", th_fbn_comm_allreduce, 5, 0},
    {"fbn_comm_alltoall", th_fbn_comm_alltoall, 5, 0},
    {"fbn_comm_alltoall_peers", th_fbn_comm_alltoall_peers, 5, 0},
    {"fbn_comm_alltoallv", th_fbn_comm_alltoallv, 7, 0},
    {"fbn_comm_heartbeat", th_fbn_comm_heartbeat, 1, 0},
    {"fbn_comm_id_bytes", th_fbn_comm_id_bytes, 0, 0},
    {"fbn_compact_routes", th_fbn_compact_routes, 6, 0},
    {"fbn_convert_bf16", th_fbn_convert_bf16, 3, 0},
    {"fbn_copy_jobs", th_fbn_copy_jobs, 5, 0},
    {"fbn_device_ok", th_fbn_device_ok, 0, 0},
    {"fbn_eval_pack", th_fbn_eval_pack, 6, 0},
    {"fbn_eval_pack_groups", th_fbn_eval_pack_groups, 5, 0},
    {"fbn_eval_reduce", th_fbn_eval_reduce, 7, 0},
    {"fbn_fields_bwd", th_fbn_fields_bwd, 32, 1},
    {"fbn_fields_bwd_grid", th_fbn_fields_bwd_grid, 2, 0},
    {"fbn_fields_bwd_img", th_fbn_fields_bwd_img, 32, 1},
    {"fbn_fields_bwd_partials_size", th_fbn_fields_bwd_partials_size, 3, 0},
    {"fbn_fields_bwd_slot", th_fbn_fields_bwd_slot, 33, 1},
    {"fbn_fields_fwd", th_fbn_fields_fwd, 33, 1},
    {"fbn_fields_fwd_hot", th_fbn_fields_fwd_hot, 34, 1},
    {"fbn_gauc_reduce", th_fbn_gauc_reduce, 9, 0},
    {"fbn_gemm", th_fbn_gemm, 25, 1},
    {"fbn_gemm_bf16out", th_fbn_gemm_bf16out, 12, 0},
    {"fbn_gemm_bn_bwd_part", th_fbn_gemm_bn_bwd_part, 16, 1},
    {"fbn_gemm_bn_bwd_part_supported", th_fbn_gemm_bn_bwd_part_supported, 7, 0},
    {"fbn_gemm_s3", th_fbn_gemm_s3, 16, 1},
    {"fbn_gemm_slabs", th_fbn_gemm_slabs, 19, 0},
    {"fbn_gemm_slabs_group", th_fbn_gemm_slabs_group, 3, 0},
    {"fbn_gemm_slabs_group_split", th_fbn_gemm_slabs_group_split, 3, 0},
    {"fbn_gemm_slabs_split", th_fbn_gemm_slabs_split, 3, 0},
    {"fbn_gemm_split", th_fbn_gemm_split, 25, 1},
    {"fbn_head_fwd", th_fbn_head_fwd, 11, 1},
    {"fbn_hot_rows", th_fbn_hot_rows, 12, 0},
    {"fbn_outer", th_fbn_outer, 6, 0},
    {"fbn_owner_claim", th_fbn_owner_claim, 6, 0},
    {"fbn_owner_fold", th_fbn_owner_fold, 20, 0},
    {"fbn_owner_gather", th_fbn_owner_gather, 10, 0},
    {"fbn_owner_gather_self", th_fbn_owner_gather_self, 13, 0},
    {"fbn_pack_extras", th_fbn_pack_extras, 4, 0},
    {"fbn_pad_routes", th_fbn_pad_routes, 7, 0},
    {"fbn_pairs_bwd", th_fbn_pairs_bwd, 12, 0},
    {"fbn_pairs_bwd_img", th_fbn_pairs_bwd_img, 9, 0},
    {"fbn_pairs_fwd", th_fbn_pairs_fwd, 10, 0},
    {"fbn_pairs_fwd_img", th_fbn_pairs_fwd_img, 8, 0},
    {"fbn_probe_arm", th_fbn_probe_arm, 1, 0},
    {"fbn_probe_disarm", th_fbn_probe_disarm, 0, 0},
    {"fbn_rank_hist", th_fbn_rank_hist, 4, 0},
    {"fbn_rec_fields", th_fbn_rec_fields, 26, 0},
    {"fbn_rec_fields_list", th_fbn_rec_fields_list, 29, 0},
    {"fbn_rec_hist_pool", th_fbn_rec_hist_pool, 9, 0},
    {"fbn_rec_item_cache", th_fbn_rec_item_cache, 13, 1},
    {"fbn_rec_rank", th_fbn_rec_rank, 13, 0},
    {"fbn_rec_rank_list", th_fbn_rec_rank_list, 16, 0},
    {"fbn_rec_topk", th_fbn_rec_topk, 18, 0},
    {"fbn_rec_topk_list", th_fbn_rec_topk_list, 22, 0},
    {"fbn_ring_slot", th_fbn_ring_slot, 12, 0},
    {"fbn_route", th_fbn_route, 14, 0},
    {"fbn_route_fc", th_fbn_route_fc, 13, 0},
    {"fbn_route_fc_status", th_fbn_route_fc_status, 8, 0},
    {"fbn_row_chunks", th_fbn_row_chunks, 1, 0},
    {"fbn_sigmoid_bwd", th_fbn_sigmoid_bwd, 5, 0},
    {"fbn_sort_u64", th_fbn_sort_u64, 7, 0},
    {"fbn_sparse_fixup", th_fbn_sparse_fixup, 14, 0},
    {"fbn_sparse_fixup_dup", th_fbn_sparse_fixup_dup, 8, 0},
    {"fbn_sparse_fold_fx", th_fbn_sparse_fold_fx, 9, 0},
    {"fbn_step_end", th_fbn_step_end, 8, 0},
    {"fbn_sum", th_fbn_sum, 4, 1},
    {"fbn_sum_jobs", th_fbn_sum_jobs, 3, 0},
    {"fbn_sum_jobs2", th_fbn_sum_jobs2, 5, 0},
    {"fbn_sum_jobs_sq", th_fbn_sum_jobs_sq, 8, 0},
    {"fbn_sum_slices", th_fbn_sum_slices, 6, 0},
    {"fbn_sumsq", th_fbn_sumsq, 6, 0},
    {"fbn_sumsq_flagged", th_fbn_sumsq_flagged, 10, 0},
    {"fbn_sumsq_sparse", th_fbn_sumsq_sparse, 8, 0},
    {"fbn_sumsq_sparse_norms", th_fbn_sumsq_sparse_norms, 12, 0},
    {"fbn_unpack_extras", th_fbn_unpack_extras, 4, 0},
    {"fbn_unpack_sumsq", th_fbn_unpack_sumsq, 6, 0},
    {"fbn_version", th_fbn_version, 0, 0},
    {"fbn_widen_bf16", th_fbn_widen_bf16, 4, 0},
};
```

ctr_recommendation_amd/ops.py:

```python
from __future__ import annotations

import os

import ctypes
from dataclasses import dataclass
from typing import Callable, Dict, Optional

import torch

from . import _lib
from ._lib import call, ptr

INT_MAX = 0x7FFFFFFF
NO_REMAP = (INT_MAX, 0, 0)
H1, H2 = 512, 256
LN_EPS = 1e-5
BN_EPS = 1e-5
BN_MOMENTUM = 0.1


_BN2_BWD_IN_FWD = os.environ.get("FBN_BN2_BWD_IN_FWD", "1") == "1"
_SPLIT_BWD = os.environ.get("FBN_SPLIT_BWD", "0") == "1"
_SPLIT3 = os.environ.get("FBN_SPLIT3", "1") != "0"
_BN1_BWD_IN_GEMM = os.environ.get("FBN_BN1_BWD_IN_GEMM", "1") == "1"


def wa_remap(d: int):
    return (5 * d, d, 6 * d)


def _ws(nbytes: int, device) -> Optional[torch.Tensor]:
    if nbytes <= 0:
        return None
    return torch.empty((nbytes + 7) // 8, dtype=torch.float64, device=device)


def gemm(A, B, C, M, N, K, lda, ldb, ldc, transA, transB, bias=None, rB=NO_REMAP, rC=NO_REMAP, beta=0.0,
         bf16=False, stream=None, stats=None):
    nbytes = _lib.lib().fbn_gemm_workspace_size(M, N, K, int(bf16))
    ws = _ws(nbytes, C.device)
    a16, b16 = int(A.dtype == torch.bfloat16), int(B.dtype == torch.bfloat16)
    call("fbn_gemm", ptr(A), ptr(B), ptr(C), ptr(bias), M, N, K, lda, ldb, ldc, int(transA), int(transB),
         rB[0], rB[1], rB[2], rC[0], rC[1], rC[2], float(beta), int(bf16 or a16 or b16), a16, b16, ptr(stats),
         ptr(ws), nbytes,
         stream if stream is not None else _lib.stream_handle())


def _probe_start(probe, name):
    if probe is None:
        return None
    kp = _lib.KernelProbe()
    probe.setdefault(name, []).append((kp, None))
    return kp


def _probe_end(kp) -> None:
    if kp is not None:
        kp.done()


def fused_bilinear(d: int) -> bool:
    return os.environ.get("FBN_NO_FUSED_BILINEAR") != "1" and bool(_lib.lib().fbn_bilinear_supported(d))


def split_mlp_input(d: int) -> bool:
    return (5 * d) % 128 == 0


def wa_ld(d: int) -> int:
    kc = 15 * d
    return kc if (kc % 64 == 0 or split_mlp_input(d)) else (kc + 63) // 64 * 64


def gemm_split(A, B, C, M, N, K, lda, ldb, ldc, transA, transB, bias=None, rC=NO_REMAP, beta=0.0, stream=None,
               stats=None, A2=None, lda2=0, kseg=INT_MAX, B2=None, ldb2=0, nseg=INT_MAX):
    nbytes = _lib.lib().fbn_gemm_workspace_size(M, N, K, 1)
    ws = _ws(nbytes, C.device)
    call("fbn_gemm_split", ptr(A), ptr(B), ptr(C), ptr(bias), M, N, K, lda, ldb, ldc, int(transA), int(transB),
         rC[0], rC[1], rC[2], float(beta), ptr(stats), ptr(ws), nbytes, ptr(A2), lda2, kseg, ptr(B2), ldb2, nseg,
         stream if stream is not None else _lib.stream_handle())


class _ConvJob(ctypes.Structure):
    _fields_ = [("src", ctypes.c_void_p), ("dst", ctypes.c_void_p), ("rows", ctypes.c_int), ("cols", ctypes.c_int),
                ("ld", ctypes.c_int), ("trans", ctypes.c_int), ("seg", ctypes.c_int), ("off0", ctypes.c_int),
                ("off1", ctypes.c_int), ("part", ctypes.c_int), ("dld", ctypes.c_int), ("pst", ctypes.c_int)]
CONV_MAX = 16


def split_images(specs, stream) -> None:
    jobs = (_ConvJob * CONV_MAX)()
    _lib.keep(jobs)
    for i, (src, dst, rows, cols, ld, trans, rm) in enumerate(specs):
        jobs[i] = _ConvJob(src.data_ptr(), dst.data_ptr(), rows, cols, ld, trans, rm[0], rm[1], rm[2], 2, 0,
                           rows * cols)
    call("fbn_convert_bf16", ctypes.cast(jobs, ctypes.c_void_p).value, len(specs), stream)


def s3_ok(M, N, K0, lda, ldb, transA, transB) -> bool:
    return K0 % 64 == 0 and lda % 8 == 0 and ldb % 8 == 0 and (not transA or M % 8 == 0) and (transB or N % 8 == 0)


def gemm_s3(A, B, C, M, N, K0, lda, ldb, ldc, transA, transB, beta=0.0, stream=None):
    nbytes = _lib.lib().fbn_gemm_workspace_size(M, N, 3 * K0, 1)
    ws = _ws(nbytes, C.device)
    call("fbn_gemm_s3", ptr(A), ptr(B), ptr(C), M, N, K0, lda, ldb, ldc, int(transA), int(transB), A[0].numel(),
         B[0].numel(), float(beta), ptr(ws), nbytes, stream if stream is not None else _lib.stream_handle())


def bf16_weights(p: Dict[str, torch.Tensor], d: int, a: Dict[str, torch.Tensor], stream,
                 x: Optional[torch.Tensor] = None, images: bool = False) -> Dict[str, torch.Tensor]:
    jobs, n, out = bf16_weight_jobs(p, d, a, x, images)
    call("fbn_convert_bf16", ctypes.cast(jobs, ctypes.c_void_p).value, n, stream)
    return out


def bf16_weight_jobs(p: Dict[str, torch.Tensor], d: int, a: Dict[str, torch.Tensor],
                     x: Optional[torch.Tensor] = None, images: bool = False):
    dev = p["mlp.0.weight"].device
    KC = 15 * d
    spec = [("Wa", p["mlp.0.weight"], H1, KC, 21 * d, 0, wa_remap(d)),
            ("WaT", p["mlp.0.weight"], KC, H1, 21 * d, 1, wa_remap(d)),
            ("Wb", p["mlp.4.weight"], H2, H1, H1, 0, NO_REMAP),
            ("WbT", p["mlp.4.weight"], H1, H2, H1, 1, NO_REMAP),
            ("Wp", p["mm_proj.0.weight"], d, 128, 128, 0, NO_REMAP)]
    if "bilinear.W" in p:
        spec += [("W", p["bilinear.W"], d, d, d, 0, NO_REMAP), ("WT", p["bilinear.W"], d, d, d, 1, NO_REMAP)]
    if x is not None:
        spec.append(("x", x, x.shape[0], x.shape[1], x.shape[1], 0, NO_REMAP))
    jobs = (_ConvJob * CONV_MAX)()
    a["_conv_jobs"] = jobs
    _lib.keep(jobs)
    out = {}
    for i, (name, src, rows, cols, ld, trans, rm) in enumerate(spec):
        img = images and name in ("WaT", "WbT", "W", "x")
        key = ("s3w_" if img else "w16_") + name
        dld = wa_ld(d) if name == "Wa" else cols
        shape = (2, rows, cols) if img else (rows, dld)
        t = a.get(key)
        if t is None or tuple(t.shape) != shape:
            t = _lib.persistent(lambda: torch.zeros(shape, dtype=torch.bfloat16, device=dev))
            a[key] = t
        out[name] = t[0] if img else (t[:, :cols] if dld != cols else t)
        if name == "Wa":
            out["Wa_full"] = t
        jobs[i] = _ConvJob(src.data_ptr(), t.data_ptr(), rows, cols, ld, trans, rm[0], rm[1], rm[2],
                           2 if img else 0, dld if dld != cols else 0, rows * cols if img else 0)
    return jobs, len(spec), out


class _SumJob(ctypes.Structure):
    _fields_ = [("part", ctypes.c_void_p), ("out", ctypes.c_void_p), ("nch", ctypes.c_int), ("C", ctypes.c_int),
                ("scale", ctypes.c_float), ("beta", ctypes.c_float), ("ld", ctypes.c_int), ("pad", ctypes.c_int)]


class _SlabJob(ctypes.Structure):
    _fields_ = [("ws", ctypes.c_void_p), ("out", ctypes.c_void_p), ("M", ctypes.c_int), ("N", ctypes.c_int),
                ("ldc", ctypes.c_int), ("nsplit", ctypes.c_int), ("seg", ctypes.c_int), ("off0", ctypes.c_int),
                ("off1", ctypes.c_int), ("beta", ctypes.c_float)]


_DEFER_REDUCE = os.environ.get("FBN_DEFER_REDUCE", "1") != "0"
_WGRAD_GROUP = os.environ.get("FBN_WGRAD_GROUP", "1") != "0"


class _SqRange(ctypes.Structure):
    _fields_ = [("x", ctypes.c_void_p), ("n", ctypes.c_longlong)]


class _SlabGemm(ctypes.Structure):
    _fields_ = [("A", ctypes.c_void_p), ("B", ctypes.c_void_p), ("ws", ctypes.c_void_p), ("ws_bytes", ctypes.c_size_t),
                ("A2", ctypes.c_void_p), ("B2", ctypes.c_void_p), ("M", ctypes.c_int), ("N", ctypes.c_int),
                ("K", ctypes.c_int), ("lda", ctypes.c_int), ("ldb", ctypes.c_int), ("transA", ctypes.c_int),
                ("transB", ctypes.c_int), ("lda2", ctypes.c_int), ("kseg", ctypes.c_int), ("ldb2", ctypes.c_int),
                ("nseg", ctypes.c_int), ("s3k0", ctypes.c_int), ("lo_a", ctypes.c_longlong),
                ("lo_b", ctypes.c_longlong)]
_nsplit = ctypes.c_int(0)
# ... 474 lines not shown


def backward(p: Dict[str, torch.Tensor], batch: Dict[str, torch.Tensor], a: Dict[str, torch.Tensor],
             gout: torch.Tensor, g: Dict[str, torch.Tensor], cfg: FwdConfig, *,
             table_grad: Optional[torch.Tensor] = None, gvec: Optional[torch.Tensor] = None,
             gnorm: Optional[torch.Tensor] = None, gslot=None, dense_sumsq: Optional[torch.Tensor] = None,
             pos: Optional[torch.Tensor] = None,
             sendbuf: Optional[torch.Tensor] = None, coll: Collective = NO_COLLECTIVE,
             ntot: Optional[int] = None, extra_sums=(), side: Optional["torch.cuda.Stream"] = None,
             probe: Optional[Dict[str, list]] = None, hooks: Optional[Dict[str, object]] = None):
    d, L = cfg.d, cfg.L
    B = a["B"]
    dev = gout.device
    st = _lib.stream_handle(dev)
    ntot = B if ntot is None else ntot
    KC = 15 * d
    scale = 1.0 / (1.0 - cfg.p_drop) if (cfg.training and cfg.p_drop > 0) else 1.0
    f32 = dict(dtype=torch.float32, device=dev)
    bf = cfg.bf16
    w16 = a.get("w16")
    bf16_ = dict(dtype=torch.bfloat16, device=dev)
    lean = bf and coll.world <= 1

    def tmp(name, shape, dtype=torch.float32):
        t = a.get("bwd_" + name)
        if t is None or tuple(t.shape) != tuple(shape) or t.dtype != dtype:
            t = _lib.persistent(lambda: torch.empty(shape, dtype=dtype, device=dev))
            a["bwd_" + name] = t
        return t

    sb = 2 if (cfg.fwd16 and _SPLIT_BWD) else False
    s3 = cfg.fwd16 and _SPLIT3 and not bf and not cfg.bilinear_each
    s3img = s3 and bool(a.get("s3img"))
    im = {}

    def img(name, rows, cols):
        return tmp("s3_" + name, (2, rows, cols), torch.bfloat16)

    if s3:
        jobs = []
        for name, src, rows, cols, ld, trans, rm in (("WbT", p["mlp.4.weight"], H1, H2, H1, 1, NO_REMAP),
                                                     ("WaT", p["mlp.0.weight"], KC, H1, 21 * d, 1, wa_remap(d)),
                                                     ("W", p["bilinear.W"], d, d, d, 0, NO_REMAP),
                                                     ("x", batch["item_emb_d128"], B, 128, 128, 0, NO_REMAP)):
            t = a.get("s3w_" + name) if a.get("s3w") else None
            if t is not None and tuple(t.shape) == (2, rows, cols):
                im[name] = t
            else:
                im[name] = img(name, rows, cols)
                jobs.append((src, im[name], rows, cols, ld, trans, rm))
        if s3img:
            im["h1"] = a["s3_h1"]
        else:
            im["h1"] = img("h1", B, H1)
            jobs.append((a["h1"], im["h1"], B, H1, H1, 0, NO_REMAP))
        if a.get("s3img"):
            im["Vc"] = a["s3_vc"]
        else:
            im["Vc"] = img("Vc", 5 * B, d)
            jobs.append((a["Vc"], im["Vc"], 5 * B, d, d, 0, NO_REMAP))
        if a.get("s3_c") is not None and tuple(a["s3_c"].shape) == (2, B, KC):
            im["c"] = a["s3_c"]
        else:
            im["c"] = img("c", B, KC)
            jobs.append((a["c"], im["c"], B, KC, KC, 0, NO_REMAP))
        if jobs:
            split_images(jobs, st)
    dh2pre = None if (lean or s3img) else tmp("dh2pre", (B, H2))
    dh2 = img("dh2", B, H2) if s3 else None
    dh2pre16 = tmp("dh2pre16", (B, H2), torch.bfloat16) if bf else None
    sums = DeferredSums(a)
    wg = _SideWork(side, dev)
    bn_backward(None, gout, p["mlp.8.weight"], a["h2"], scale, a["h2pre"], a["mean2"], a["inv2"],
                p["mlp.5.weight"], B, H2, ntot, dh2pre, g["mlp.5.weight"], g["mlp.5.bias"], g["mlp.8.weight"],
                coll, st, dpre16=dh2pre16, bias_grad=g["mlp.4.bias"], sums=sums,
                part_pre=a.get("bn2_bwd_part") if (gout is a.get("gout")) else None, tag="bn2",
                dpre_img=dh2 if s3img else None)
    sums.add(gout, B, 1, g["mlp.8.bias"])
    dh1 = tmp("dh1", (B, H1))
    part1 = None
    lean_h1 = a.get("lean_h1", False)
    if bf:
        if not sums.gemm_slabs(dh2pre16, a["h1_16"], g["mlp.4.weight"], H2, H1, B, H2, H1, H1, True, False,
                               stream=st):
            wg.run(lambda s: gemm(dh2pre16, a["h1_16"], g["mlp.4.weight"], H2, H1, B, H2, H1, H1, True, False,
                                  stream=s))
        if (_BN1_BWD_IN_GEMM and lean_h1 and coll.world <= 1
                and _lib.lib().fbn_gemm_bn_bwd_part_supported(B, H1, H2, H2, H2, 0, 1)):
            part1 = tmp("part1", (_lib.lib().fbn_bn_bwd_chunks(B, H1) * 3 * H1,), torch.float64)
            call("fbn_gemm_bn_bwd_part", ptr(dh2pre16), ptr(w16["WbT"]), ptr(dh1), B, H1, H2, H2, H2, H1, 0, 1,
                 ptr(a["h1_16"]), ptr(a["h1pre"]), ptr(a["mean1"]), float(scale), ptr(part1), st)
        else:
            gemm(dh2pre16, w16["WbT"], dh1, B, H1, H2, H2, H2, H1, False, True, stream=st)
    elif s3:
        if not s3img:
            split_images([(dh2pre, dh2, B, H2, H2, 0, NO_REMAP)], st)
        if not sums.gemm_slabs(dh2, im["h1"], g["mlp.4.weight"], H2, H1, B, H2, H1, H1, True, False, stream=st,
                               s3=True):
            if s3_ok(H2, H1, B, H2, H1, True, False):
                wg.run(lambda s: gemm_s3(dh2, im["h1"], g["mlp.4.weight"], H2, H1, B, H2, H1, H1, True, False,
                                         stream=s))
            else:
                wg.run(lambda s: gemm(dh2pre, a["h1"], g["mlp.4.weight"], H2, H1, B, H2, H1, H1, True, False,
                                      stream=s))
        if s3_ok(B, H1, H2, H2, H2, False, True):
            gemm_s3(dh2, im["WbT"], dh1, B, H1, H2, H2, H2, H1, False, True, stream=st)
        else:
            gemm(dh2pre, p["mlp.4.weight"], dh1, B, H1, H2, H2, H1, H1, False, False, stream=st)
    else:
        wg.run(lambda s: gemm(dh2pre, a["h1"], g["mlp.4.weight"], H2, H1, B, H2, H1, H1, True, False, bf16=sb,
                              stream=s))
        gemm(dh2pre, p["mlp.4.weight"], dh1, B, H1, H2, H2, H1, H1, False, False, bf16=sb, stream=st)
    dh1pre = None if (lean or s3img) else tmp("dh1pre", (B, H1))
    dh1pre16 = tmp("dh1pre16", (B, H1), torch.bfloat16) if bf else None
    dh1i = img("dh1", B, H1) if s3 else None
    bn_backward(dh1, None, None, None if lean_h1 else a["h1"], scale, a["h1pre"], a["mean1"], a["inv1"],
                p["mlp.1.weight"], B, H1, ntot, dh1pre, g["mlp.1.weight"], g["mlp.1.bias"], None, coll, st,
                dpre16=dh1pre16, bias_grad=g["mlp.0.bias"], sums=sums, hact16=a["h1_16"] if lean_h1 else None,
                part_pre=part1, tag="bn1", dpre_img=dh1i if s3img else None)
    if s3:
        if not s3img:
            split_images([(dh1pre, dh1i, B, H1, H1, 0, NO_REMAP)], st)
        if not sums.gemm_slabs(dh1i, im["c"], g["mlp.0.weight"], H1, KC, B, H1, KC, 21 * d, True, False,
                               rC=wa_remap(d), stream=st, s3=True):
            wg.run(lambda s: gemm(dh1pre, a["c"], g["mlp.0.weight"], H1, KC, B, H1, KC, 21 * d, True, False,
                                  rC=wa_remap(d), stream=s))
    elif a.get("split_c"):
        if not sums.gemm_slabs(dh1pre16, a["Vc16"], g["mlp.0.weight"], H1, KC, B, H1, 5 * d, 21 * d, True, False,
                               rC=wa_remap(d), stream=st, B2=a["c"][:, 5 * d:], ldb2=KC, nseg=5 * d):
            wg.run(lambda s: gemm_split(dh1pre16, a["Vc16"], g["mlp.0.weight"], H1, KC, B, H1, 5 * d, 21 * d, True,
                                        False, rC=wa_remap(d), stream=s, B2=a["c"][:, 5 * d:], ldb2=KC, nseg=5 * d))
    elif bf:
        ldcc = a["c"].shape[1]
        if not sums.gemm_slabs(dh1pre16, a["c"], g["mlp.0.weight"], H1, KC, B, H1, ldcc, 21 * d, True, False,
                               rC=wa_remap(d), stream=st):
            wg.run(lambda s: gemm(dh1pre16, a["c"], g["mlp.0.weight"], H1, KC, B, H1, ldcc, 21 * d, True, False,
                                  rC=wa_remap(d), stream=s))
    else:
        wg.run(lambda s: gemm(dh1pre, a["c"], g["mlp.0.weight"], H1, KC, B, H1, KC, 21 * d, True, False,
                              rC=wa_remap(d), bf16=sb, stream=s))
    if a.get("fused_bilinear"):
        dc = tmp("dc16", (B, KC), torch.bfloat16)
        call("fbn_gemm_bf16out", ptr(dh1pre16), ptr(w16["WaT"]), ptr(dc), B, KC, H1, H1, H1, KC, 0, 1, st)
    elif bf:
        dc = torch.empty((B, KC), **f32)
        gemm(dh1pre16, w16["WaT"], dc, B, KC, H1, H1, H1, KC, False, True, stream=st)
    elif s3 and s3_ok(B, KC, H1, H1, H1, False, True):
        dc = torch.empty((B, KC), **f32)
        gemm_s3(dh1i, im["WaT"], dc, B, KC, H1, H1, H1, KC, False, True, stream=st)
    else:
        dc = torch.empty((B, KC), **f32)
        gemm(dh1pre, p["mlp.0.weight"], dc, B, KC, H1, H1, 21 * d, KC, False, False, rB=wa_remap(d), bf16=sb,
             stream=st)
    dV = tmp("dV", (B, 5, d))
    v16 = bf and not cfg.bilinear_each
    dU16 = tmp("dU16", (B, 5, d), torch.bfloat16) if v16 else None
    if a.get("fused_bilinear"):
        call("fbn_bilinear_bwd", ptr(dc), KC, int(dc.dtype == torch.bfloat16), ptr(a["Vc16"]), ptr(w16["WT"]),
             ptr(w16["W"]), ptr(dV), ptr(dU16), B, d, st)
        if not sums.gemm_slabs(a["Vc16"], dU16, g["bilinear.W"], d, d, 5 * B, d, d, d, True, False, stream=st):
            wg.run(lambda s: gemm(a["Vc16"], dU16, g["bilinear.W"], d, d, 5 * B, d, d, d, True, False, stream=s))
    elif s3 and a.get("s3img"):
        dU = None
        dU2 = img("dU", 5 * B, d)
        call("fbn_pairs_bwd_img", ptr(dc), ptr(a["Vc"]), ptr(a["U"]), ptr(dV), ptr(dU2), B, d, KC, st)
    else:
        dU = torch.empty((B, 5, d), **f32)
        call("fbn_pairs_bwd", ptr(dc), None if v16 else ptr(a["Vc"]), ptr(a["Vc16"]) if v16 else None, ptr(a["U"]),
             ptr(dV), ptr(dU), ptr(dU16), B, d, KC, int(cfg.bilinear_each), st)
    if a.get("fused_bilinear"):
        pass
    elif not cfg.bilinear_each:
        if bf:
            if not sums.gemm_slabs(a["Vc16"], dU16, g["bilinear.W"], d, d, 5 * B, d, d, d, True, False, stream=st):
                wg.run(lambda s: gemm(a["Vc16"], dU16, g["bilinear.W"], d, d, 5 * B, d, d, d, True, False, stream=s))
            gemm(dU16, w16["W"], dV, 5 * B, d, d, d, d, d, False, True, beta=1.0, stream=st)
        elif s3:
            if dU is not None:
                dU2 = img("dU", 5 * B, d)
                split_images([(dU, dU2, 5 * B, d, d, 0, NO_REMAP)], st)
            if not sums.gemm_slabs(im["Vc"], dU2, g["bilinear.W"], d, d, 5 * B, d, d, d, True, False, stream=st,
                                   s3=True):
                wg.run(lambda s: gemm(a["Vc"], dU, g["bilinear.W"], d, d, 5 * B, d, d, d, True, False, stream=s))
            if s3_ok(5 * B, d, d, d, d, False, True):
                gemm_s3(dU2, im["W"], dV, 5 * B, d, d, d, d, d, False, True, beta=1.0, stream=st)
            else:
                gemm(dU, p["bilinear.W"], dV, 5 * B, d, d, d, d, d, False, True, beta=1.0, stream=st)
        else:
            wg.run(lambda s: gemm(a["Vc"], dU, g["bilinear.W"], d, d, 5 * B, d, d, d, True, False, bf16=sb,
                                  stream=s))
            gemm(dU, p["bilinear.W"], dV, 5 * B, d, d, d, d, d, False, True, beta=1.0, bf16=sb, stream=st)
    else:
        g["bilinear.W_list.0"].zero_()
        for f in range(1, 5):
            gemm(dU[:, f - 1], p[f"bilinear.W_list.{f}"], dV[:, f - 1], B, d, d, 5 * d, d, 5 * d, False, True,
                 beta=1.0, bf16=cfg.bf16, stream=st)
            gemm(a["Vc"][:, f - 1], dU[:, f - 1], g[f"bilinear.W_list.{f}"], d, d, B, 5 * d, 5 * d, d, True, False,
                 bf16=cfg.bf16, stream=st)
    if hooks and "after_bilinear_bwd" in hooks:
        hooks["after_bilinear_bwd"](sums)
    R = cfg.R
    ncate = p["cate_emb.weight"].shape[0]
    P = _lib.lib().fbn_fields_bwd_partials_size(d, R, ncate)
    nblk = _lib.lib().fbn_fields_bwd_grid(B, d)
    partials = tmp("partials", (nblk, P))
    dhmm = tmp("dhmm", (B, d))
    dhmm16 = tmp("dhmm16", (B, d), torch.bfloat16) if bf else None
    dhs = img("dhmm", B, d) if s3 else None
    seq = batch.get("item_seq", None)
    Lr = 0 if seq is None else L
    V = p["item_emb.weight"].shape[0] if pos is None else 0
    keys = ("senet.excitation.0.weight", "senet.excitation.0.bias", "senet.excitation.2.weight",
            "senet.excitation.2.bias", "mm_proj.1.weight", "mm_proj.1.bias", "cate_emb.weight", "mm_proj.0.bias")
    if _DEFER_REDUCE:
        outs = None
        o = 0
        for k, n in zip(keys, (6 * R, R, 6 * R, 6, d, d, ncate * d, d)):
            sums.add(partials[:, o:], nblk, n, g[k], ld=P)
            o += n
    else:
        outs_arr = (ctypes.c_void_p * 8)(*[g[k].data_ptr() for k in keys])
        _lib.keep(outs_arr)
        outs = ctypes.cast(outs_arr, ctypes.c_void_p).value
    evb = _probe_start(probe, "fields_bwd")
    if gslot is not None:
        ring, ring_n, ring_stride, step, cell = gslot
        call("fbn_fields_bwd_slot", ptr(batch["item_id"]), ptr(seq) if Lr else None, ptr(batch["likes_level"]),
             ptr(batch["views_level"]), ptr(a["hmm"]), ptr(p["mm_proj.1.weight"]), ptr(p["mm_proj.1.bias"]), LN_EPS,
             ptr(p["senet.excitation.0.weight"]), ptr(p["senet.excitation.0.bias"]),
             ptr(p["senet.excitation.2.weight"]), R, ncate, ptr(p["cate_emb.weight"]), ptr(a["X"]), ptr(a["a"]),
             ptr(a["cnt"]), ptr(dV), ptr(dhmm), ptr(dhs if s3img else dhmm16), int(bool(s3img)), ptr(partials), outs,
             ptr(ring), ring_n, ring_stride, ptr(step), ptr(cell), ptr(gnorm), V, B, Lr, d, st)
    else:
        call("fbn_fields_bwd_img" if s3img else "fbn_fields_bwd", ptr(batch["item_id"]), ptr(seq) if Lr else None,
             ptr(batch["likes_level"]),
             ptr(batch["views_level"]), ptr(a["hmm"]), ptr(p["mm_proj.1.weight"]), ptr(p["mm_proj.1.bias"]), LN_EPS,
             ptr(p["senet.excitation.0.weight"]), ptr(p["senet.excitation.0.bias"]),
             ptr(p["senet.excitation.2.weight"]),
             R, ncate, ptr(p["cate_emb.weight"]), ptr(a["X"]), ptr(a["a"]), ptr(a["cnt"]), ptr(dV), ptr(dhmm),
             ptr(dhs if s3img else dhmm16), ptr(partials), outs,
             ptr(table_grad), ptr(gvec), ptr(gnorm), V, ptr(pos), ptr(sendbuf),
             int(sendbuf is not None and sendbuf.dtype == torch.bfloat16), B, Lr, d, st)
    _probe_end(evb)
    if hooks and "after_fields_bwd" in hooks:
        hooks["after_fields_bwd"]()
    if bf:
        if not sums.gemm_slabs(dhmm16, w16["x"], g["mm_proj.0.weight"], d, 128, B, d, 128, 128, True, False,
                               stream=st):
            wg.run(lambda s: gemm(dhmm16, w16["x"], g["mm_proj.0.weight"], d, 128, B, d, 128, 128, True, False,
                                  stream=s))
    elif s3:
        if not s3img:
            split_images([(dhmm, dhs, B, d, d, 0, NO_REMAP)], st)
        if not sums.gemm_slabs(dhs, im["x"], g["mm_proj.0.weight"], d, 128, B, d, 128, 128, True, False,
                               stream=st, s3=True):
            wg.run(lambda s: gemm(dhmm, batch["item_emb_d128"], g["mm_proj.0.weight"], d, 128, B, d, 128, 128, True,
                                  False, stream=s))
    else:
        wg.run(lambda s: gemm(dhmm, batch["item_emb_d128"], g["mm_proj.0.weight"], d, 128, B, d, 128, 128, True,
                              False, bf16=sb, stream=s))
    for job in extra_sums:
        sums.add(*job)
    if hooks and "before_flush" in hooks:
        hooks["before_flush"]()
    if dense_sumsq is not None and side is not None:
        raise ValueError("dense_sumsq needs the weight gradients on the main stream (side=None)")
    partial = sums.flush(st, probe, sumsq=dense_sumsq, grads=g if dense_sumsq is not None else None)
    wg.join()
    return partial
```

include/fibinet.h:

```cpp
#ifndef FIBINET_H
#define FIBINET_H

#include <stddef.h>
#include <stdint.h>

#ifdef __cplusplus
extern "C" {
#endif

#define FBN_OK 0
#define FBN_ERR_ARG 1
#define FBN_ERR_LAUNCH 2
#define FBN_ERR_UNSUPPORTED 3

const char* fbn_last_error(void);
int fbn_probe_arm(int slot);
int fbn_probe_disarm(void);
float fbn_probe_elapsed(int slot);
int fbn_version(void);
int fbn_device_ok(void);

size_t fbn_gemm_workspace_size(int M, int N, int K, int bf16);
int fbn_gemm(const void* A, const void* B, float* C, const float* bias, int M, int N, int K, int lda, int ldb,
             int ldc, int transA, int transB, int rB_seg, int rB_off0, int rB_off1, int rC_seg, int rC_off0,
// ... 94 lines not shown
int fbn_bn_bwd_apply(const float* G, const float* gvec, const float* w, const float* hact, float scale,
                     const float* Xpre, const float* mean, const float* invstd, const float* gamma, int B, int C,
                     const double* red_d, double ntot, float* dXpre, short* dXpre16, float* dgamma, float* dbeta,
                     float* dw, void* ws, void* stream);
int fbn_bn_bwd(const float* G, const float* gvec, const float* w, const float* hact, float scale, const float* Xpre,
               const float* mean, const float* invstd, const float* gamma, int B, int C, float* dXpre, float* dgamma,
               float* dbeta, float* dw, void* ws, void* stream);
size_t fbn_bn_colpart_size(int B, int C);
int fbn_row_chunks(int B);
int fbn_bn_bwd_chunks(int B, int C);
int fbn_bn_bwd_fused(const float* G, const float* gvec, const float* w, const float* hact, const short* hact16,
                     float scale, const float* Xpre, const float* mean, const float* invstd, const float* gamma, int B,
                     int C, double ntot, float* dXpre, short* dXpre16, float* dgamma, float* dbeta, float* dw,
                     float* colpart, const double* part_pre, void* ws, void* stream);
int fbn_bn_bwd_fused_img(const float* G, const float* gvec, const float* w, const float* hact, const short* hact16,
                         float scale, const float* Xpre, const float* mean, const float* invstd, const float* gamma,
                         int B, int C, double ntot, float* dXpre, void* dXpre_img, float* dgamma, float* dbeta,
                         float* dw, float* colpart, const double* part_pre, void* ws, void* stream);
int fbn_convert_bf16(const void* jobs, int n, void* stream);
size_t fbn_colsum_workspace_size(int B, int C);
int fbn_colsum(const float* X, int B, int C, int ldx, float* out, float beta, void* ws, void* stream);
int fbn_colsum_partial(const float* X, int B, int C, int ldx, float* part, void* stream);
int fbn_sum_jobs(const void* jobs, int n, void* stream);
int fbn_sum_jobs2(const void* jobs, int n, const void* slabs, int ns, void* stream);
int fbn_sum_jobs_sq(const void* jobs, int n, const void* slabs, int ns, const void* ranges, int nr, double* sumsq,
                    void* stream);

int fbn_head_fwd(const float* H, const float* w, const float* bias, int B, int C, float* logits, float* probs,
                 const float* labels, float* loss_terms, float* gout, float denom, void* stream);
int fbn_sigmoid_bwd(const float* gp, const float* probs, float* gout, int B, void* stream);
int fbn_outer(const float* g, const float* w, float* out, int B, int C, void* stream);
int fbn_sum(const float* x, int n, float* out, float scale, void* stream);

int fbn_sumsq(const float* x, long long n, const int* n_rows, int row_len, double* out, void* stream);
int fbn_clip_coef(const double* sumsq, float max_norm, float* coef, float* norm, void* stream);
int fbn_adam_dense(float* p, const float* g, float* m, float* v, long long n, const float* coef,
                   const void* consts_table, const int* step, float wd, float beta2, float eps, const double* sumsq,
                   float max_norm, float* coef_out, float* norm_out, void* stream);
int fbn_sparse_fixup(const int64_t* item, const int64_t* seq, const int* ids, int n, int L, long long V, int rank,
                     const int* map, const float* gvec, float* extra, int* slot_row, int Lp1, int D, void* stream);
int fbn_sumsq_sparse(const float* gvec, float* extra, int* slot_row, int Lp1, int n, int D, double* out,
                     void* stream);
int fbn_sparse_fixup_dup(const int* dup, int n, const float* gvec, float* extra, int* slot_row, int Lp1, int D,
                         void* stream);
int fbn_sumsq_sparse_norms(const double* gnorm, const float* gvec, float* extra, int* slot_row, int Lp1, int n, int D,
                           double* out, unsigned long long* fx, const float* dense, long long n_dense, void* stream);
#define FBN_GRAD_FULL 0x10000
#define FBN_GRAD_CELL 0x20000
#define FBN_GRAD_BF16 0x40000
#define FBN_RING_BF16 0x40000000
int fbn_sparse_fold_fx(const int* dup, int* hasdup, int n, const float* gvec, int* slot_row, int Lp1, int D,
                       unsigned long long* acc, void* stream);
int fbn_adam_table(float* p, float* m, float* v, long long nrows, int D, int* map, const float* gvec, float* extra,
                   int* slot_row, int Lp1, const float* coef, const void* consts_table, const int* step, float wd,
                   float beta2, float eps, int mode, void* stream);
int fbn_adam_touched(float* p, float* m, float* v, int D, int* map, const float* gvec, float* extra, int* slot_row,
                     int Lp1, int n, const float* coef, const void* consts_table, const int* step, float wd,
                     float beta2, float eps, int* last, void* stream);
#define FBN_ROW_STATE_BYTES 16
int fbn_adam_catchup(float* p, float* m, float* v, long long nrows, int D, const int* slot_row, int n_ent,
                     const int* map, int F, int parts, int* last, const void* consts_table, const int* step, float wd,
                     float beta2, float eps, int* pend, const float* ring, const float* coef_hist,
                     long long ring_stride, int ring_n, int decoupled, void* stream);
int fbn_adam_owner_claim_catchup(const int* lids, int n, int skip0, int* map, int* slot_row,
                                 unsigned long long* preclaim, float* p, float* m, float* v, long long nrows, int D,
                                 int F, int* last, const void* consts_table, const int* step, float wd, float beta2,
                                 float eps, int* pend, const float* ring, const float* coef_hist, long long ring_stride,
                                 int ring_n, int decoupled, void* stream);
int fbn_adam_claim_catchup(const int64_t* item, const int64_t* seq, int B, int L, long long V, int* map, int* slot_row,
                           int* dup, int* hasdup, unsigned long long* preclaim, float* p, float* m, float* v,
                           long long nrows, int D, int F, int* last,
                           const void* consts_table, const int* step, float wd, float beta2, float eps, int* pend,
                           const float* ring, const float* coef_hist, long long ring_stride, int ring_n, int decoupled,
                           void* stream);
int fbn_adam_claim_catchup_conv(const int64_t* item, const int64_t* seq, int B, int L, long long V, int* map,
                                int* slot_row, int* dup, int* hasdup, unsigned long long* preclaim, float* p,
                                float* m, float* v, long long nrows, int D, int F, int* last,
                                const void* consts_table, const int* step, float wd, float beta2, float eps,
                                int* pend, const float* ring, const float* coef_hist, long long ring_stride,
                                int ring_n, int decoupled, const void* conv_jobs, int n_conv, void* stream);
int fbn_adam_prefetch(const int64_t* item, const int64_t* seq, int B, int L, long long V, const int* map,
                      unsigned long long* preclaim, float* p, float* m, float* v, int D, int* last,
                      const void* consts_table, const int* step, float wd, float beta2, float eps, int* pend,
                      const float* ring, const float* coef_hist, long long ring_stride, int ring_n, int decoupled,
                      void* stream);

size_t fbn_adam_prefetch_binned_ws_size(long long n);
int fbn_adam_prefetch_binned(const int64_t* item, const int64_t* seq, int B, int L, long long V, const int* map,
                             unsigned long long* preclaim, float* p, float* m, float* v, int D, int* last,
                             const void* consts_table, const int* step, float wd, float beta2, float eps, int* pend,
                             const float* ring, const float* coef_hist, long long ring_stride, int ring_n,
                             int decoupled, void* ws, size_t ws_bytes, void* stream);

int fbn_adam_prefetch_rows(const int* lids, int n, int skip0, long long nrows, const int* map,
                           unsigned long long* preclaim, float* p, float* m, float* v, int D, int* last,
                           const void* consts_table, const int* step, float wd, float beta2, float eps, int* pend,
                           const float* ring, const float* coef_hist, long long ring_stride, int ring_n,
                           int decoupled, void* stream);
int fbn_adam_flush(float* p, float* m, float* v, long long nrows, int D, int* last, const void* consts_table,
                   const int* step, float wd, float beta2, float eps, int* pend, const float* ring,
                   const float* coef_hist, long long ring_stride, int ring_n, int decoupled, void* stream);
#define FBN_TICKET_WORDS 17
int fbn_adam_step_tail(float* dp, const float* dg, float* dm, float* dv, long long n_dense, const double* sumsq,
                       float max_norm, float* coef_out, float* norm_out, float* p, float* m, float* v, int D, int* map,
                       const float* gvec, float* extra, int* slot_row, int Lp1, int n, const void* consts_table,
                       int* step, float wd, float beta2, float eps, int* last, int* pend, float* ring,
                       float* coef_hist, int ring_n, long long ring_stride, int B, unsigned long long* rng,
                       long long* nbt0, long long* nbt1, unsigned* ticket, int max_step, int* err, void* stream);
int fbn_adam_selftest(int n, unsigned seed, unsigned long long* dev, void* stream);
int fbn_adam_commit(float* p, float* m, float* v, int D, int* map, const float* gvec, float* extra, int* slot_row,
                    int Lp1, int n, const float* coef, const void* consts_table, const int* step, float wd,
                    float beta2, float eps, int* last, int* pend, float* ring, float* coef_hist, int ring_n, int B,
                    void* stream);

#define FBN_SUMSQ_SLOTS 64
int fbn_claim_rows(const int64_t* item, const int64_t* seq, int B, int L, long long V, int* map, int* slot_row,
                   int* dup, int* hasdup, void* stream);
int fbn_pack_extras(const float* loss, double* tab_slots, float* out, void* stream);
int fbn_unpack_extras(const float* in, float* loss, double* sumsq, void* stream);
int fbn_unpack_sumsq(const float* in, float* loss, const float* x, long long n, double* sumsq, void* stream);
int fbn_step_end(int* step, unsigned long long* rng, double* sumsq, long long* nbt0, long long* nbt1, int max_step,
                 int* err, void* stream);

int fbn_route(const int64_t* item, const int64_t* seq, int B, int L, long long V, long long Vl, int nranks,
              int* counts, int* offsets, int* cursor, int* send_ids, int* pos, int* err, void* stream);
int fbn_route_fc(const int64_t* item, const int64_t* seq, int B, int L, long long V, long long Vl, int nranks,
                 int cap, int* send_ids, int* pos, int* stat, int* err, void* stream);
int fbn_route_fc_status(const int* send_ids, int* recv_ids, int nranks, int rank, int cap, int* stat, int* host,
                        void* stream);
int fbn_owner_gather_self(const int* ids, int n, const float* E, void* out, int* map, int* slot_row, int rank, int D,
                          int out_bf16, void* self_out, int self_lo, int self_n, void* stream);
int fbn_owner_claim(const int* ids, int n, int* map, int* slot_row, int rank, void* stream);
int fbn_owner_gather(const int* ids, int n, const float* E, void* out, int* map, int* slot_row, int rank, int D,
                     int out_bf16, void* stream);
int fbn_ring_slot(float* ring, int ring_n, long long stride, const int* step, void* cell, const void* wire,
                  int wire_bf16, long long n, const void* wire_self, long long self_lo, long long self_n,
                  void* stream);
int fbn_owner_fold(const int* ids, int n, int rank, const int* map, int* slot_row, const void* wire, int wire_bf16,
                   const void* wire_self, long long self_lo, long long self_n, float* ring, int ring_n,
                   long long stride, const int* step, void* cell, float* extra, int D, double* part,
                   unsigned long long* fx, void* stream);
int fbn_sumsq_flagged(const int* slot_row, int n, const void* cell, float* extra, int D, const double* part,
                      double* sumsq, unsigned long long* fx, int ring_bf16, void* stream);
int fbn_widen_bf16(const void* in, float* out, long long n, void* stream);
int fbn_pad_routes(const int* send_ids, const int* offsets, const int* counts, int world, int cap, int* out,
                   void* stream);
int fbn_compact_routes(const int* padded, int world, int cap, int* ids, int* counts, void* stream);
int fbn_copy_jobs(const void* const* src, void* const* dst, const long long* bytes, int n, void* stream);

int fbn_bilinear_supported(int D);
int fbn_bilinear_fwd(const short* V16, const short* WT16, short* c, int B, int D, int ldc, void* stream);
int fbn_bilinear_bwd(const void* dc, int ldc, int dc_bf16, const short* V16, const short* WT16, const short* W16,
                     float* dV, short* dU16, int B, int D, void* stream);

int fbn_collate(const int64_t* perm, int B, const int64_t* item, const int64_t* seq, int Ls, int L,
                const int64_t* likes, const int64_t* views, const int64_t* user, const float* label,
                const int* slot_of_id, long long n_ids, const int64_t* sorted_ids, const float* emb, int E,
                int64_t* o_item, int64_t* o_seq,
                int64_t* o_likes, int64_t* o_views, int64_t* o_user, float* o_label, float* o_emb, int* missing,
                void* stream);
int fbn_collate_zero_if(float* x, long long n, const int* flag, void* stream);

int fbn_eval_pack(const float* probs, const float* labels, long long n, uint32_t* keys_out, unsigned* status,
                  void* stream);
size_t fbn_eval_workspace_size(long long n);
int fbn_eval_reduce(const uint32_t* keys, long long n, void* ws, size_t ws_bytes, void* out, unsigned* status,
                    void* stream);

#define FBN_SORT_TILE 2048
size_t fbn_sort_u64_workspace_size(long long n);
int fbn_sort_u64(const uint64_t* in, long long n, int bits, void* ws, size_t ws_bytes, uint64_t* out, void* stream);

#define FBN_GAUC_REC_WORDS 8
int fbn_eval_pack_groups(const long long* ids, long long n, uint32_t* gids_out, unsigned* status, void* stream);
size_t fbn_gauc_workspace_size(long long n);
int fbn_gauc_reduce(const uint32_t* keys, const uint32_t* gids, long long n, void* ws, size_t ws_bytes,
                    unsigned long long* table, void* out, unsigned* status, void* stream);

#define FBN_CALIB_MAX_BINS 1024
#define FBN_CALIB_BIN_WORDS 8
size_t fbn_calib_workspace_size(long long n);
int fbn_calib_reduce(const uint32_t* keys, long long n, int bins, void* ws, size_t ws_bytes, uint64_t* out,
                     unsigned* status, void* stream);

int fbn_rec_item_cache(const int64_t* item_id, const int64_t* likes, const int64_t* views, const float* hmm,
                       const float* ln_g, const float* ln_b, float ln_eps, int n_cate, long long V, float* cache,
                       int* err, int M, int D, void* stream);
int fbn_rec_hist_pool(const int64_t* item_seq, const float* table, long long V, float* hist, int* err, int U, int L,
                      int D, void* stream);
int fbn_rec_fields(const int64_t* item_id, const int64_t* likes, const int64_t* views, const float* cache,
                   const float* hist, const float* cate, int n_cate, const float* table, long long V, const float* w1,
                   const float* b1, const float* w2, const float* b2, int R, float* Vc, short* Vc16, void* c, int ldc,
                   int c_bf16, float* a_out, int* err, int U, int m0, int Mc, int D, void* stream);
size_t fbn_rec_topk_workspace_size(int U, int Mc, int K);
int fbn_rec_topk(const float* logits, int U, int m0, int Mc, const int64_t* item_id, const int64_t* item_seq, int L,
                 int exclude, int K, unsigned long long* carry, void* ws, size_t ws_bytes, int64_t* out_index,
                 int64_t* out_item, float* out_logit, float* out_prob, unsigned* status, void* stream);
int fbn_rec_rank(const float* logits, int ld, int U, int M, const int64_t* item_id, const int64_t* item_seq, int L,
                 int exclude, const int64_t* target_pos, int* rank, int* n_eligible, unsigned* status, void* stream);
#define FBN_RANK_REC_WORDS 260
int fbn_rank_hist(const int* rank, long long n, unsigned long long* rec, void* stream);

int fbn_rec_fields_list(const int64_t* item_id, const int64_t* likes, const int64_t* views, const float* cache,
                        const float* hist, const float* cate, int n_cate, const float* table, long long V,
                        const float* w1, const float* b1, const float* w2, const float* b2, int R, float* Vc,
                        short* Vc16, void* c, int ldc, int c_bf16, float* a_out, int* err, int U,
                        const int64_t* cand_pos, int ldp, int c0, int Cc, int M, int D, void* stream);
int fbn_rec_topk_list(const float* logits, int U, int c0, int Cc, const int64_t* cand_pos, int ldp, int M,
                      const int64_t* item_id, const int64_t* item_seq, int L, int exclude, int K,
                      unsigned long long* carry, void* ws, size_t ws_bytes, int64_t* out_slot, int64_t* out_index,
                      int64_t* out_item, float* out_logit, float* out_prob, unsigned* status, void* stream);
int fbn_rec_rank_list(const float* logits, int ld, int U, int C, const int64_t* cand_pos, int ldp, int M,
                      const int64_t* item_id, const int64_t* item_seq, int L, int exclude,
                      const int64_t* target_slot, int* rank, int* n_eligible, unsigned* status, void* stream);

int fbn_plan_create(void** plan);
int fbn_plan_destroy(void* plan);
int fbn_plan_size(void* plan);
int fbn_plan_add_call(void* plan, const char* name, const unsigned long long* iargs, int ni, const double* fargs,
                      int nf);
int fbn_plan_add_record(void* plan, int slot, void* stream);
int fbn_plan_add_wait(void* plan, void* stream, int slot);
int fbn_plan_run(void* plan, int* failed);
int fbn_plan_event_sync(void* plan, int slot);

int fbn_comm_load(const char* path);
int fbn_comm_id_bytes(void);
int fbn_comm_unique_id(void* out);
int fbn_comm_init(void** comm, const void* id, int world, int rank);
int fbn_comm_destroy(void* comm);
int fbn_comm_alltoallv(void* comm, const void* send, const int* send_counts, void* recv, const int* recv_counts,
                       long long row_bytes, void* stream);
int fbn_comm_alltoall(void* comm, const void* send, void* recv, long long bytes_per_peer, void* stream);
int fbn_comm_alltoall_peers(void* comm, const void* send, void* recv, long long bytes_per_peer, void* stream);
int fbn_comm_allreduce(void* comm, void* buf, long long n, int dtype, void* stream);
int fbn_comm_allgather(void* comm, const void* send, void* recv, long long bytes_per_rank, void* stream);
int fbn_sum_slices(const void* in, int ns, long long n, int dtype, void* out, void* stream);
int fbn_comm_watch(long long timeout_ms);
int fbn_comm_heartbeat(void* stream);
int fbn_comm_abort(void* comm);
int fbn_comm_watchdog_fired(void* comm);

#ifdef __cplusplus
}
#endif
#endif
```

Before: 20.47 million samples/s.

## Fuse bilinear backward with fields backward into one kernel

Adds a kernel that computes the bilinear backward (dV, dU) and keeps dV in LDS, then runs the fields backward (SENET, LayerNorm, category grads) inside the same block. This removes the fp32 dV round trip through global memory and one kernel launch. It makes the fields-backward helpers shared through a common header. The bilinear weight-gradient GEMM now runs after the fused kernel. The fused kernel uses more LDS and a fixed sample-to-block mapping, which may lower occupancy and constrain the grid size.

```diff
diff --git a/ctr_recommendation_amd/_lib.py b/ctr_recommendation_amd/_lib.py
--- a/ctr_recommendation_amd/_lib.py
+++ b/ctr_recommendation_amd/_lib.py
@@ -132,6 +132,9 @@
     "fbn_bilinear_supported": (I, [I]),
     "fbn_bilinear_fwd": (I, [P, P, P, I, I, I, P]),
     "fbn_bilinear_bwd": (I, [P, I, I, P, P, P, P, P, I, I, P]),
+    "fbn_bilinear_fields_bwd_supported": (I, [I, I, I, I]),
+    "fbn_bilinear_fields_bwd": (I, [P, I, P, P, P, P, P, P, P, P, P, F, P, P, P, I, I, P, P, P, P, P, P, P, P, P, P, P,
+                                    I, LL, P, I, I, P]),
     "fbn_collate": (I, [P, I, P, P, I, I, P, P, P, P, P, LL, P, P, I, P, P, P, P, P, P, P, P, P]),
     "fbn_collate_zero_if": (I, [P, LL, P, P]),
     "fbn_eval_pack": (I, [P, P, LL, P, P, P]),
diff --git a/ctr_recommendation_amd/csrc/bilinear.hip b/ctr_recommendation_amd/csrc/bilinear.hip
--- a/ctr_recommendation_amd/csrc/bilinear.hip
+++ b/ctr_recommendation_amd/csrc/bilinear.hip
@@ -1,4 +1,5 @@
 #include "common.h"
+#include "fields_common.h"
 #include <algorithm>
 
 namespace {
@@ -203,6 +204,132 @@
   }
 }
 
+constexpr int FB_PITCH = 5 * 128 + 4;
+constexpr int FB_RMAX = 3;
+
+__device__ __forceinline__ int fb_sample(int blk, int nblk, int s) { return 8 * blk + (s & 7) + (s >> 3) * 8 * nblk; }
+
+template <bool SLOT>
+__global__ void __launch_bounds__(256, 2) bilinear_fields_bwd_kernel(const short* __restrict__ dc, int ldc,
+                                                                    const short* __restrict__ V16,
+                                                                    const short* __restrict__ WT16,
+                                                                    const short* __restrict__ W16,
+                                                                    short* __restrict__ dU16, FieldBwdArgs p) {
+  FBN_MAIN_PRIO();
+  constexpr int D = 128, NT = 256, RB = 2, G = D / 4, SPW = 64 / G, CH = D / 8;
+  extern __shared__ __attribute__((aligned(16))) float smem[];
+  short* sV = reinterpret_cast<short*>(smem);
+  short* sW = sV + 5 * TS * D;
+  const int tid = threadIdx.x, lane = tid & 63, w = tid >> 6;
+  const int blk = blockIdx.x, nblk = gridDim.x, B = p.B;
+  {
+    constexpr int N = TS * 5 * CH / NT;
+    bf16x8 v[N];
+#pragma unroll
+    for (int j = 0; j < N; ++j) {
+      const int i = tid + j * NT, m = i / CH, b = fb_sample(blk, nblk, m / 5);
+      v[j] = (bf16x8){0, 0, 0, 0, 0, 0, 0, 0};
+      if (b < B) v[j] = *reinterpret_cast<const bf16x8*>(V16 + ((size_t)b * 5 + m % 5) * D + (i % CH) * 8);
+    }
+#pragma unroll
+    for (int j = 0; j < N; ++j) {
+      const int i = tid + j * NT, m = i / CH;
+      *reinterpret_cast<bf16x8*>(sV + swz<D>((m % 5) * TS + m / 5, (i % CH) * 8)) = v[j];
+    }
+  }
+  stage_w<D, NT>(sW, WT16, tid);
+  __syncthreads();
+  WStage<D, NT> wnext;
+  wnext.load(W16, tid);
+  f32x4 acc[RB][5];
+#pragma unroll
+  for (int rb = 0; rb < RB; ++rb)
+#pragma unroll
+    for (int f = 0; f < 5; ++f) acc[rb][f] = (f32x4){0.f, 0.f, 0.f, 0.f};
+  mfma_5<D>(acc, sW, sV, w, lane);
+  __syncthreads();
+  const int s = lane & 15, lq = lane >> 4;
+  const int bs = fb_sample(blk, nblk, s);
+  const bool live = bs < B;
+  const short* dcr = dc + (size_t)(live ? bs : 0) * ldc;
+#pragma unroll
+  for (int rb = 0; rb < RB; ++rb) {
+    const int n0 = 32 * w + 16 * rb + 4 * lq;
+    f32x4 v[5], gv[5], gu[5];
+#pragma unroll
+    for (int f = 0; f < 5; ++f) {
+      v[f] = ld_bf4(sV + swz<D>(f * TS + s, n0));
+      gv[f] = live ? ld_bf4(dcr + f * D + n0) : (f32x4){0.f, 0.f, 0.f, 0.f};
+      gu[f] = (f32x4){0.f, 0.f, 0.f, 0.f};
+    }
+#pragma unroll
+    for (int k = 0; k < 10; ++k) {
+      const f32x4 gp = live ? ld_bf4(dcr + (5 + k) * D + n0) : (f32x4){0.f, 0.f, 0.f, 0.f};
+      gv[PI[k]] += gp * acc[rb][PJ[k]];
+      gu[PJ[k]] += gp * v[PI[k]];
+    }
+#pragma unroll
+    for (int f = 0; f < 5; ++f) {
+      const bf16x4 t = to_bf4(gu[f]);
+      *reinterpret_cast<bf16x4*>(sV + swz<D>(f * TS + s, n0)) = t;
+      if (live) *reinterpret_cast<bf16x4*>(dU16 + ((size_t)bs * 5 + f) * D + n0) = t;
+    }
+#pragma unroll
+    for (int f = 0; f < 5; ++f) acc[rb][f] = gv[f];
+  }
+  __syncthreads();
+  wnext.store(sW, tid);
+  const int q = lane % G, grp = lane / G;
+  const int b_0 = (4 * blk + w) * SPW + grp, b_1 = b_0 + 4 * nblk * SPW;
+  FieldsBwdIn in = fields_bwd_load<D>(p, b_0 < B ? b_0 : 0, q);
+  float* gvec = p.gvec;
+  if constexpr (SLOT) {
+    gvec += (size_t)(__builtin_amdgcn_readfirstlane(*p.slot_step) % p.ring_n) * p.ring_stride;
+    if (blk == 0 && tid == 0) *p.slot_cell = gvec;
+  }
+  __syncthreads();
+  mfma_5<D>(acc, sW, sV, w, lane);
+  __syncthreads();
+  float* tile = smem;
+  float* sp = smem + TS * FB_PITCH;
+  const int P = 13 * p.R + 6 + 3 * D + p.n_cate * D;
+#pragma unroll
+  for (int rb = 0; rb < RB; ++rb) {
+    const int k0 = 32 * w + 16 * rb + 4 * lq;
+#pragma unroll
+    for (int f = 0; f < 5; ++f) *reinterpret_cast<f32x4*>(tile + s * FB_PITCH + f * D + k0) = acc[rb][f];
+  }
+  for (int i = tid; i < 4 * P; i += NT) sp[i] = 0.f;
+  __syncthreads();
+
+  float* sv = sp + 4 * P + (w * SPW + grp) * (12 + 2 * FB_RMAX);
+  float* w_ct = sp + w * P + 13 * p.R + 6 + 2 * D;
+  FieldsBwdAcc<D, FB_RMAX> facc;
+  facc.zero();
+#pragma unroll
+  for (int it = 0; it < 2; ++it) {
+    const int b = it ? b_1 : b_0;
+    if (b - grp >= B) break;
+    const bool blive = b < B;
+    FieldsBwdIn nxt;
+    if (it == 0) nxt = fields_bwd_load<D>(p, b_1 < B ? b_1 : 0, q);
+    f32x4 dx0 = {0.f, 0.f, 0.f, 0.f}, dx1 = {0.f, 0.f, 0.f, 0.f};
+    long long lk = -1, vw = -1;
+    if (blive) {
+      const float* dvs = tile + (8 * it + SPW * w + grp) * FB_PITCH + 4 * q;
+      f32x4 dv[5];
+#pragma unroll
+      for (int f = 0; f < 5; ++f) dv[f] = *reinterpret_cast<const f32x4*>(dvs + f * D);
+      lk = in.lk;
+      vw = in.vw;
+      fields_bwd_sample<D, 0, FB_RMAX>(p, gvec, b, lane, in, dv, sv, facc, dx0, dx1);
+    }
+    fields_bwd_cate<D>(w_ct, p.n_cate, lane, blive, lk, vw, dx0, dx1);
+    if (it == 0) in = nxt;
+  }
+  fields_bwd_fold<D, FB_RMAX>(p, sp, facc);
+}
+
 }
 
 extern "C" int fbn_bilinear_supported(int D) { return D == 16 || D == 32 || D == 64 || D == 128; }
@@ -253,3 +380,62 @@
   FBN_CHECK_LAUNCH();
   return FBN_OK;
 }
+
+static size_t bilinear_fields_lds(int R, int n_cate) {
+  const size_t a = (size_t)(5 * TS * 128 + 128 * 128) * sizeof(short);
+  const size_t b = (size_t)TS * FB_PITCH * sizeof(float) + fields_bwd_lds(128, R, n_cate, FB_RMAX);
+  return std::max(a, b);
+}
+
+extern "C" int fbn_bilinear_fields_bwd_supported(int B, int D, int R, int n_cate) {
+  if (D != 128 || B <= 0 || R < 1 || R > FB_RMAX || n_cate < 0) return 0;
+  if ((long long)B > 16LL * fields_grid(B, D, FBN_FB_MAXBLK)) return 0;
+  return bilinear_fields_lds(R, n_cate) <= 80 * 1024;
+}
+
+extern "C" int fbn_bilinear_fields_bwd(const void* dc, int ldc, const short* V16, const short* WT16, const short* W16,
+                                       short* dU16, const int64_t* likes, const int64_t* views, const float* hmm,
+                                       const float* ln_g, const float* ln_b, float ln_eps, const float* w1,
+                                       const float* b1, const float* w2, int R, int n_cate, const float* cate,
+                                       const float* X, const float* a, const float* cnt, float* dhmm, short* dhmm16,
+                                       float* partials, float* const* param_grads, float* gvec, const int* slot_step,
+                                       void* slot_cell, int ring_n, long long ring_stride, double* gnorm, int B, int D,
+                                       void* stream) {
+  if (B <= 0) return FBN_OK;
+  if (!fbn_bilinear_fields_bwd_supported(B, D, R, n_cate)) {
+    fbn_set_error("fbn_bilinear_fields_bwd: needs D = 128, R <= 3, at most 16 samples per fields-backward block and "
+                  "80 KB of LDS (fbn_bilinear_fields_bwd_supported)");
+    return FBN_ERR_UNSUPPORTED;
+  }
+  if (!dc || !V16 || !WT16 || !W16 || !dU16 || (ldc & 3) || ((uintptr_t)dc & 7) || ((uintptr_t)V16 & 15) ||
+      ((uintptr_t)WT16 & 15) || ((uintptr_t)W16 & 15) || ((uintptr_t)dU16 & 7)) {
+    fbn_set_error("fbn_bilinear_fields_bwd: bf16 dc, V, W^T, W, dU16 required and aligned (16 B; dc, dU16 8 B), ldc % 4 == 0");
+    return FBN_ERR_ARG;
+  }
+  if (!likes || !views || !hmm || !ln_g || !ln_b || !w1 || !b1 || !w2 || !cate || !X || !a || !cnt || !partials ||
+      !gvec || ((uintptr_t)gvec & 15)) {
+    fbn_set_error("fbn_bilinear_fields_bwd: the fields operands, partials and gvec (16-B aligned) are required");
+    return FBN_ERR_ARG;
+  }
+  if (slot_step && (!slot_cell || ring_n < 1 || ring_stride < (long long)B * 2 * D || (ring_stride & 3))) {
+    fbn_set_error("fbn_bilinear_fields_bwd: slot form: cell; ring_n >= 1, ring_stride >= B*2*D, % 4 == 0");
+    return FBN_ERR_ARG;
+  }
+  FieldBwdArgs p = {};
+  p.likes = likes; p.views = views; p.hmm = hmm; p.ln_g = ln_g; p.ln_b = ln_b; p.w1 = w1; p.b1 = b1; p.w2 = w2;
+  p.cate = cate; p.X = X; p.a = a; p.cnt = cnt; p.dhmm = dhmm; p.dhmm16 = dhmm16; p.partials = partials;
+  p.gvec = gvec; p.gnorm = gnorm;
+  p.slot_step = slot_step; p.slot_cell = (float**)slot_cell; p.ring_n = ring_n; p.ring_stride = ring_stride;
+  p.B = B; p.R = R; p.n_cate = n_cate; p.ln_eps = ln_eps;
+  const dim3 grid((unsigned)fields_grid(B, D, FBN_FB_MAXBLK));
+  const unsigned lds = (unsigned)bilinear_fields_lds(R, n_cate);
+  hipStream_t st = (hipStream_t)stream;
+  const short* dc16 = (const short*)dc;
+  if (slot_step)
+    fbn_launch(bilinear_fields_bwd_kernel<true>, grid, dim3(256), lds, st, dc16, ldc, V16, WT16, W16, dU16, p);
+  else
+    fbn_launch(bilinear_fields_bwd_kernel<false>, grid, dim3(256), lds, st, dc16, ldc, V16, WT16, W16, dU16, p);
+  FBN_CHECK_LAUNCH();
+  if (!param_grads) return FBN_OK;
+  return fbn_fields_reduce_partials(partials, param_grads, B, D, R, n_cate, st);
+}
diff --git a/ctr_recommendation_amd/csrc/fields.hip b/ctr_recommendation_amd/csrc/fields.hip
--- a/ctr_recommendation_amd/csrc/fields.hip
+++ b/ctr_recommendation_amd/csrc/fields.hip
@@ -255,83 +255,32 @@
   }
 }
 
-struct FieldBwdArgs {
-  const int64_t* item_id; const int64_t* item_seq; const int64_t* likes; const int64_t* views;
-  const float* hmm; const float* ln_g;
-  const float* w1; const float* b1; const float* w2;
-  const float* X;
-  const float* cate;
-  const float* ln_b;
-  const float* a;
-  const float* cnt;
-  const float* dV;
-  float* dhmm;
-  short* dhmm16;
-  long long dhmm16_lo;
-  float* partials;
-  float* gtab; float* gvec;
-  double* gnorm;
-  const int* slot_step; float** slot_cell; long long ring_stride; int ring_n;
-  const int* pos; void* sendbuf;
-  long long V;
-  int B, L, R, n_cate;
-  float ln_eps;
-};
-
-template <int G>
-__device__ __forceinline__ f32x4 transpose_cols(const f32x4& v, int lane) {
-  const int base = lane - lane % G, q = lane % G;
-  f32x4 t;
-#pragma unroll
-  for (int e = 0; e < 4; ++e) {
-    const int src = base + e * (G / 4) + q / 4;
-    const float x0 = __shfl(v[0], src, 64), x1 = __shfl(v[1], src, 64);
-    const float x2 = __shfl(v[2], src, 64), x3 = __shfl(v[3], src, 64);
-    const int c = q & 3;
-    t[e] = c == 0 ? x0 : (c == 1 ? x1 : (c == 2 ? x2 : x3));
-  }
-  return t;
-}
-template <int G>
-__device__ __forceinline__ void atomic_add_row_t(float* row, const f32x4& t, int q) {
-  atomicAdd(row + q, t[0]); atomicAdd(row + G + q, t[1]); atomicAdd(row + 2 * G + q, t[2]);
-  atomicAdd(row + 3 * G + q, t[3]);
-}
 
 template <int D, int MODE, int RMAX, bool SLOT = false>
 __global__ void __launch_bounds__(256) fields_bwd_kernel(FieldBwdArgs p) {
   FBN_MAIN_PRIO();
   constexpr int G = D / 4;
   constexpr int SPW = 64 / G;
-  constexpr int NPMAX = 13 * RMAX + 6;
-  constexpr int SJ = (NPMAX + G - 1) / G;
   extern __shared__ __attribute__((aligned(16))) float sp[];
-  const int R = p.R;
-  const int NP = 13 * R + 6;
+  const int NP = 13 * p.R + 6;
   const int P = NP + 3 * D + p.n_cate * D;
   const int wave = threadIdx.x >> 6;
-  float* ws = sp + wave * P;
   float* sv = sp + 4 * P + (wave * SPW + (threadIdx.x & 63) / G) * (12 + 2 * RMAX);
   for (int i = threadIdx.x; i < 4 * P; i += blockDim.x) sp[i] = 0.f;
   __syncthreads();
-  float* w_lg = ws + NP;
-  float* w_ct = w_lg + 2 * D;
-  float* w_hb = w_ct + p.n_cate * D;
+  float* w_ct = sp + wave * P + NP + 2 * D;
 
   const int lane = threadIdx.x & 63;
   const int q = lane % G, grp = lane / G;
   const int gw = (blockIdx.x * blockDim.x + threadIdx.x) >> 6;
   const int nwaves = (gridDim.x * blockDim.x) >> 6;
-  const int L = p.L;
   float* gvec = p.gvec;
   if constexpr (SLOT) {
     gvec += (size_t)(__builtin_amdgcn_readfirstlane(*p.slot_step) % p.ring_n) * p.ring_stride;
     if (blockIdx.x == 0 && threadIdx.x == 0) *p.slot_cell = gvec;
   }
-  f32x4 acc_lg = {0.f, 0.f, 0.f, 0.f}, acc_lb = {0.f, 0.f, 0.f, 0.f}, acc_hb = {0.f, 0.f, 0.f, 0.f};
-  float acc_se[SJ];
-#pragma unroll
-  for (int j = 0; j < SJ; ++j) acc_se[j] = 0.f;
+  FieldsBwdAcc<D, RMAX> acc;
+  acc.zero();
 
   for (int b0 = gw * SPW; b0 < p.B; b0 += nwaves * SPW) {
     const int b = b0 + grp;
@@ -339,198 +288,18 @@
     f32x4 dx0 = {0.f, 0.f, 0.f, 0.f}, dx1 = {0.f, 0.f, 0.f, 0.f};
     long long lk = -1, vw = -1;
     if (live) {
-      const float* Xb = p.X + (size_t)b * 2 * D + 4 * q;
+      const FieldsBwdIn in = fields_bwd_load<D>(p, b, q);
       const float* dVb = p.dV + (size_t)b * 5 * D + 4 * q;
-      f32x4 x[5], dv[5];
-      lk = p.likes[b];
-      vw = p.views[b];
-      const long long lkc = (lk >= 0 && lk < p.n_cate) ? lk : 0, vwc = (vw >= 0 && vw < p.n_cate) ? vw : 0;
-      x[0] = *reinterpret_cast<const f32x4*>(p.cate + lkc * D + 4 * q);
-      x[1] = *reinterpret_cast<const f32x4*>(p.cate + vwc * D + 4 * q);
-      x[2] = *reinterpret_cast<const f32x4*>(Xb);
-      x[4] = *reinterpret_cast<const f32x4*>(Xb + D);
+      f32x4 dv[5];
 #pragma unroll
       for (int f = 0; f < 5; ++f) dv[f] = *reinterpret_cast<const f32x4*>(dVb + f * D);
-      const f32x4 h = *reinterpret_cast<const f32x4*>(p.hmm + (size_t)b * D + 4 * q);
-      x[3] = ln_relu<G>(h, p.ln_g, p.ln_b, p.ln_eps, q);
-      float a[6];
-#pragma unroll
-      for (int f = 0; f < 6; ++f) a[f] = p.a[(size_t)b * 6 + f];
-      float z[6];
-      z[0] = 0.f;
-#pragma unroll
-      for (int f = 0; f < 5; ++f) z[f + 1] = group_sum<G>(x[f][0] + x[f][1] + x[f][2] + x[f][3]) / (float)D;
-      float qv[RMAX], rj[RMAX], dq[RMAX];
-#pragma unroll
-      for (int j = 0; j < RMAX; ++j) {
-        float s = 0.f;
-        if (j < R) {
-          s = p.b1[j];
-#pragma unroll
-          for (int f = 0; f < 6; ++f) s += p.w1[j * 6 + f] * z[f];
-        }
-        qv[j] = s;
-        rj[j] = fmaxf(s, 0.f);
-      }
-      float ds[6];
-      ds[0] = 0.f;
-#pragma unroll
-      for (int f = 0; f < 5; ++f) {
-        const float da = group_sum<G>(dv[f][0] * x[f][0] + dv[f][1] * x[f][1] + dv[f][2] * x[f][2] + dv[f][3] * x[f][3]);
-        ds[f + 1] = da * (1.f - a[f + 1]) * a[f + 1];
-      }
-      float dz[6] = {0.f, 0.f, 0.f, 0.f, 0.f, 0.f};
-#pragma unroll
-      for (int j = 0; j < RMAX; ++j) {
-        float dr = 0.f;
-        if (j < R) {
-#pragma unroll
-          for (int f = 0; f < 6; ++f) dr += p.w2[f * R + j] * ds[f];
-        }
-        dq[j] = (j < R && qv[j] > 0.f) ? dr : 0.f;
-        if (j < R) {
-#pragma unroll
-          for (int f = 0; f < 6; ++f) dz[f] += p.w1[j * 6 + f] * dq[j];
-        }
-      }
-      if (q == 0) {
-#pragma unroll
-        for (int f = 0; f < 6; ++f) { sv[f] = ds[f]; sv[6 + f] = z[f]; }
-#pragma unroll
-        for (int jj = 0; jj < RMAX; ++jj) { sv[12 + jj] = dq[jj]; sv[12 + RMAX + jj] = rj[jj]; }
-      }
-      __builtin_amdgcn_wave_barrier();
-#pragma unroll
-      for (int j = 0; j < SJ; ++j) {
-        const int k = q + j * G;
-        float v = 0.f;
-        if (k < 6 * R) v = sv[12 + k / 6] * sv[6 + k % 6];
-        else if (k < 7 * R) v = sv[12 + (k - 6 * R)];
-        else if (k < 13 * R) v = sv[(k - 7 * R) / R] * sv[12 + RMAX + (k - 7 * R) % R];
-        else if (k < NP) v = sv[k - 13 * R];
-        acc_se[j] += v;
-      }
-      __builtin_amdgcn_wave_barrier();
-      f32x4 dx[5];
-#pragma unroll
-      for (int f = 0; f < 5; ++f) dx[f] = dv[f] * a[f + 1] + dz[f + 1] / (float)D;
-      dx0 = dx[0];
-      dx1 = dx[1];
-
-      {
-        const float mean = group_sum<G>(h[0] + h[1] + h[2] + h[3]) / (float)D;
-        const f32x4 dh = h - mean;
-        const float s2 = group_sum<G>(dh[0] * dh[0] + dh[1] * dh[1] + dh[2] * dh[2] + dh[3] * dh[3]);
-        const float rstd = 1.f / sqrtf(s2 / (float)D + p.ln_eps);
-        const f32x4 gam = *reinterpret_cast<const f32x4*>(p.ln_g + 4 * q);
-        f32x4 gl, xh, gx;
-#pragma unroll
-        for (int e = 0; e < 4; ++e) {
-          gl[e] = x[3][e] > 0.f ? dx[3][e] : 0.f;
-          xh[e] = dh[e] * rstd;
-          gx[e] = gl[e] * gam[e];
-          acc_lg[e] += gl[e] * xh[e];
-          acc_lb[e] += gl[e];
-        }
-        const float m1 = group_sum<G>(gx[0] + gx[1] + gx[2] + gx[3]) / (float)D;
-        const float m2 = group_sum<G>(gx[0] * xh[0] + gx[1] * xh[1] + gx[2] * xh[2] + gx[3] * xh[3]) / (float)D;
-        f32x4 out;
-#pragma unroll
-        for (int e = 0; e < 4; ++e) out[e] = rstd * (gx[e] - m1 - xh[e] * m2);
-        *reinterpret_cast<f32x4*>(p.dhmm + (size_t)b * D + 4 * q) = out;
-        acc_hb += out;
-        if (p.dhmm16) {
-          const bf16x4 hi = (bf16x4){f2bf(out[0]), f2bf(out[1]), f2bf(out[2]), f2bf(out[3])};
-          *reinterpret_cast<bf16x4*>(p.dhmm16 + (size_t)b * D + 4 * q) = hi;
-          if (p.dhmm16_lo)
-            *reinterpret_cast<bf16x4*>(p.dhmm16 + p.dhmm16_lo + (size_t)b * D + 4 * q) =
-                (bf16x4){f2bf(out[0] - bf2f(hi[0])), f2bf(out[1] - bf2f(hi[1])), f2bf(out[2] - bf2f(hi[2])),
-                         f2bf(out[3] - bf2f(hi[3]))};
-        }
-      }
-      const f32x4 gh = dx[4] / p.cnt[b];
-      if (MODE == 0 && p.gvec) {
-        *reinterpret_cast<f32x4*>(gvec + (size_t)b * 2 * D + 4 * q) = dx[2];
-        *reinterpret_cast<f32x4*>(gvec + ((size_t)b * 2 + 1) * D + 4 * q) = gh;
-        if (p.gnorm) {
-          double si = 0.0, sh = 0.0;
-#pragma unroll
-          for (int e = 0; e < 4; ++e) {
-            si += (double)(dx[2][e] * dx[2][e]);
-            sh += (double)(gh[e] * gh[e]);
-          }
-#pragma unroll
-          for (int o = G / 2; o > 0; o >>= 1) {
-            si += __shfl_xor(si, o, 64);
-            sh += __shfl_xor(sh, o, 64);
-          }
-          if (q == 0) {
-            p.gnorm[(size_t)b * 2] = si;
-            p.gnorm[(size_t)b * 2 + 1] = sh;
-          }
-        }
-      } else if (MODE == 0) {
-        const f32x4 ti = transpose_cols<G>(dx[2], lane);
-        const f32x4 th = transpose_cols<G>(gh, lane);
-        const long long item = p.item_id[b];
-        if (item > 0 && item < p.V) atomic_add_row_t<G>(p.gtab + item * D, ti, q);
-        for (int t = 0; t < L; ++t) {
-          const long long s = p.item_seq[(size_t)b * L + t];
-          if (s > 0 && s < p.V) atomic_add_row_t<G>(p.gtab + s * D, th, q);
-        }
-      } else {
-        const int* pb = p.pos + (size_t)b * (L + 1);
-        auto put = [&](int row, const f32x4& x) {
-          if constexpr (MODE == 2) {
-            *reinterpret_cast<bf16x4*>(reinterpret_cast<short*>(p.sendbuf) + (size_t)row * D + 4 * q) =
-                (bf16x4){f2bf(x[0]), f2bf(x[1]), f2bf(x[2]), f2bf(x[3])};
-          } else {
-            *reinterpret_cast<f32x4*>(reinterpret_cast<float*>(p.sendbuf) + (size_t)row * D + 4 * q) = x;
-          }
-        };
-        if (pb[0] >= 0) put(pb[0], dx[2]);
-        for (int t = 0; t < L; ++t)
-          if (pb[t + 1] >= 0) put(pb[t + 1], gh);
-      }
-    }
-#pragma unroll
-    for (int gi = 0; gi < SPW; ++gi) {
-      if (grp == gi && live) {
-        if (lk >= 0 && lk < p.n_cate) {
-          f32x4* c = reinterpret_cast<f32x4*>(w_ct + lk * D + 4 * q);
-          *c = *c + dx0;
-        }
-        if (vw >= 0 && vw < p.n_cate) {
-          f32x4* c = reinterpret_cast<f32x4*>(w_ct + vw * D + 4 * q);
-          *c = *c + dx1;
-        }
-      }
-    }
-  }
-#pragma unroll
-  for (int o = G; o < 64; o <<= 1) {
-#pragma unroll
-    for (int e = 0; e < 4; ++e) {
-      acc_lg[e] += __shfl_xor(acc_lg[e], o, 64);
-      acc_lb[e] += __shfl_xor(acc_lb[e], o, 64);
-      acc_hb[e] += __shfl_xor(acc_hb[e], o, 64);
-    }
-#pragma unroll
-    for (int j = 0; j < SJ; ++j) acc_se[j] += __shfl_xor(acc_se[j], o, 64);
-  }
-  if (grp == 0) {
-    *reinterpret_cast<f32x4*>(w_lg + 4 * q) = acc_lg;
-    *reinterpret_cast<f32x4*>(w_lg + D + 4 * q) = acc_lb;
-    *reinterpret_cast<f32x4*>(w_hb + 4 * q) = acc_hb;
-#pragma unroll
-    for (int j = 0; j < SJ; ++j) {
-      const int k = q + j * G;
-      if (k < NP) ws[k] = acc_se[j];
-    }
-  }
-  __syncthreads();
-  float* out = p.partials + (size_t)blockIdx.x * P;
-  for (int i = threadIdx.x; i < P; i += blockDim.x) out[i] = (sp[i] + sp[P + i]) + (sp[2 * P + i] + sp[3 * P + i]);
+      lk = in.lk;
+      vw = in.vw;
+      fields_bwd_sample<D, MODE, RMAX>(p, gvec, b, lane, in, dv, sv, acc, dx0, dx1);
+    }
+    fields_bwd_cate<D>(w_ct, p.n_cate, lane, live, lk, vw, dx0, dx1);
+  }
+  fields_bwd_fold<D, RMAX>(p, sp, acc);
 }
 
 struct GradOuts {
@@ -557,15 +326,6 @@
 }
 
 
-#ifndef FBN_FB_MAXBLK
-#define FBN_FB_MAXBLK 512
-#endif
-static int fields_grid(int B, int D, int cap = 1024) {
-  const int spw = 64 / (D / 4);
-  const int waves = (B + spw - 1) / spw;
-  int blocks = (waves + 3) / 4;
-  return blocks < 1 ? 1 : (blocks > cap ? cap : blocks);
-}
 
 template <int MODE, int HCH, bool BUF, bool HOT = false, bool CMP = false>
 static int launch_fields_fwd_hb(const FieldArgs& a, int D, hipStream_t st) {
@@ -704,8 +464,7 @@
 template <int MODE, int RMAX, bool SLOT = false>
 static int launch_fields_bwd_r(const FieldBwdArgs& a, int D, hipStream_t st) {
   const int grid = fields_grid(a.B, D, FBN_FB_MAXBLK);
-  const size_t lds = (4 * (size_t)(13 * a.R + 6 + 3 * D + a.n_cate * D) + 4 * (64 / (D / 4)) * (12 + 2 * RMAX)) *
-                     sizeof(float);
+  const size_t lds = fields_bwd_lds(D, a.R, a.n_cate, RMAX);
   switch (D) {
     case 16: fbn_launch((fields_bwd_kernel<16, MODE, RMAX, SLOT>), dim3(grid), dim3(256), lds, st, a); break;
     case 32: fbn_launch((fields_bwd_kernel<32, MODE, RMAX, SLOT>), dim3(grid), dim3(256), lds, st, a); break;
@@ -797,6 +556,11 @@
                                                                : launch_fields_bwd<1>(p, D, st);
   if (rc) return rc;
   if (!param_grads) return FBN_OK;
+  return fbn_fields_reduce_partials(partials, param_grads, B, D, R, n_cate, st);
+}
+
+int fbn_fields_reduce_partials(const float* partials, float* const* param_grads, int B, int D, int R, int n_cate,
+                               hipStream_t st) {
   const int P = 13 * R + 6 + 3 * D + n_cate * D;
   const int nblk = fields_grid(B, D, FBN_FB_MAXBLK);
 
@@ -811,7 +575,7 @@
     o.p[j] = param_grads[j];
     o.off[j + 1] = o.off[j] + sizes[j];
   }
-  fbn_launch(reduce_partials_one16, dim3(fbn_cdiv(P, 16)), dim3(1024), 0, st, (const float*)partials, nblk, P, o);
+  fbn_launch(reduce_partials_one16, dim3(fbn_cdiv(P, 16)), dim3(1024), 0, st, partials, nblk, P, o);
   FBN_CHECK_LAUNCH();
   return FBN_OK;
 }
diff --git a/ctr_recommendation_amd/csrc/fields_common.h b/ctr_recommendation_amd/csrc/fields_common.h
--- a/ctr_recommendation_amd/csrc/fields_common.h
+++ b/ctr_recommendation_amd/csrc/fields_common.h
@@ -37,3 +37,311 @@
     a[f] = 1.f / (1.f + __expf(-s));
   }
 }
+
+struct FieldBwdArgs {
+  const int64_t* item_id; const int64_t* item_seq; const int64_t* likes; const int64_t* views;
+  const float* hmm; const float* ln_g;
+  const float* w1; const float* b1; const float* w2;
+  const float* X;
+  const float* cate;
+  const float* ln_b;
+  const float* a;
+  const float* cnt;
+  const float* dV;
+  float* dhmm;
+  short* dhmm16;
+  long long dhmm16_lo;
+  float* partials;
+  float* gtab; float* gvec;
+  double* gnorm;
+  const int* slot_step; float** slot_cell; long long ring_stride; int ring_n;
+  const int* pos; void* sendbuf;
+  long long V;
+  int B, L, R, n_cate;
+  float ln_eps;
+};
+
+template <int G>
+__device__ __forceinline__ f32x4 transpose_cols(const f32x4& v, int lane) {
+  const int base = lane - lane % G, q = lane % G;
+  f32x4 t;
+#pragma unroll
+  for (int e = 0; e < 4; ++e) {
+    const int src = base + e * (G / 4) + q / 4;
+    const float x0 = __shfl(v[0], src, 64), x1 = __shfl(v[1], src, 64);
+    const float x2 = __shfl(v[2], src, 64), x3 = __shfl(v[3], src, 64);
+    const int c = q & 3;
+    t[e] = c == 0 ? x0 : (c == 1 ? x1 : (c == 2 ? x2 : x3));
+  }
+  return t;
+}
+template <int G>
+__device__ __forceinline__ void atomic_add_row_t(float* row, const f32x4& t, int q) {
+  atomicAdd(row + q, t[0]); atomicAdd(row + G + q, t[1]); atomicAdd(row + 2 * G + q, t[2]);
+  atomicAdd(row + 3 * G + q, t[3]);
+}
+
+struct FieldsBwdIn {
+  f32x4 x0, x1, x2, x4, h;
+  float a[6];
+  float cnt;
+  long long lk, vw;
+};
+template <int D>
+__device__ __forceinline__ FieldsBwdIn fields_bwd_load(const FieldBwdArgs& p, int b, int q) {
+  FieldsBwdIn in;
+  const float* Xb = p.X + (size_t)b * 2 * D + 4 * q;
+  in.lk = p.likes[b];
+  in.vw = p.views[b];
+  const long long lkc = (in.lk >= 0 && in.lk < p.n_cate) ? in.lk : 0, vwc = (in.vw >= 0 && in.vw < p.n_cate) ? in.vw : 0;
+  in.x0 = *reinterpret_cast<const f32x4*>(p.cate + lkc * D + 4 * q);
+  in.x1 = *reinterpret_cast<const f32x4*>(p.cate + vwc * D + 4 * q);
+  in.x2 = *reinterpret_cast<const f32x4*>(Xb);
+  in.x4 = *reinterpret_cast<const f32x4*>(Xb + D);
+  in.h = *reinterpret_cast<const f32x4*>(p.hmm + (size_t)b * D + 4 * q);
+#pragma unroll
+  for (int f = 0; f < 6; ++f) in.a[f] = p.a[(size_t)b * 6 + f];
+  in.cnt = p.cnt[b];
+  return in;
+}
+
+template <int D, int RMAX>
+struct FieldsBwdAcc {
+  static constexpr int SJ = (13 * RMAX + 6 + D / 4 - 1) / (D / 4);
+  f32x4 lg, lb, hb;
+  float se[SJ];
+  __device__ __forceinline__ void zero() {
+    lg = lb = hb = (f32x4){0.f, 0.f, 0.f, 0.f};
+#pragma unroll
+    for (int j = 0; j < SJ; ++j) se[j] = 0.f;
+  }
+};
+
+template <int D, int MODE, int RMAX>
+__device__ __forceinline__ void fields_bwd_sample(const FieldBwdArgs& p, float* gvec, int b, int lane,
+                                                  const FieldsBwdIn& in, const f32x4 (&dv)[5], float* sv,
+                                                  FieldsBwdAcc<D, RMAX>& acc, f32x4& dx0, f32x4& dx1) {
+  constexpr int G = D / 4;
+  constexpr int SJ = FieldsBwdAcc<D, RMAX>::SJ;
+  const int q = lane % G;
+  const int R = p.R;
+  const int NP = 13 * R + 6;
+  const int L = p.L;
+  const f32x4 h = in.h;
+  f32x4 x[5];
+  x[0] = in.x0;
+  x[1] = in.x1;
+  x[2] = in.x2;
+  x[4] = in.x4;
+  x[3] = ln_relu<G>(h, p.ln_g, p.ln_b, p.ln_eps, q);
+  float a[6];
+#pragma unroll
+  for (int f = 0; f < 6; ++f) a[f] = in.a[f];
+  float z[6];
+  z[0] = 0.f;
+#pragma unroll
+  for (int f = 0; f < 5; ++f) z[f + 1] = group_sum<G>(x[f][0] + x[f][1] + x[f][2] + x[f][3]) / (float)D;
+  float qv[RMAX], rj[RMAX], dq[RMAX];
+#pragma unroll
+  for (int j = 0; j < RMAX; ++j) {
+    float s = 0.f;
+    if (j < R) {
+      s = p.b1[j];
+#pragma unroll
+      for (int f = 0; f < 6; ++f) s += p.w1[j * 6 + f] * z[f];
+    }
+    qv[j] = s;
+    rj[j] = fmaxf(s, 0.f);
+  }
+  float ds[6];
+  ds[0] = 0.f;
+#pragma unroll
+  for (int f = 0; f < 5; ++f) {
+    const float da = group_sum<G>(dv[f][0] * x[f][0] + dv[f][1] * x[f][1] + dv[f][2] * x[f][2] + dv[f][3] * x[f][3]);
+    ds[f + 1] = da * (1.f - a[f + 1]) * a[f + 1];
+  }
+  float dz[6] = {0.f, 0.f, 0.f, 0.f, 0.f, 0.f};
+#pragma unroll
+  for (int j = 0; j < RMAX; ++j) {
+    float dr = 0.f;
+    if (j < R) {
+#pragma unroll
+      for (int f = 0; f < 6; ++f) dr += p.w2[f * R + j] * ds[f];
+    }
+    dq[j] = (j < R && qv[j] > 0.f) ? dr : 0.f;
+    if (j < R) {
+#pragma unroll
+      for (int f = 0; f < 6; ++f) dz[f] += p.w1[j * 6 + f] * dq[j];
+    }
+  }
+  if (q == 0) {
+#pragma unroll
+    for (int f = 0; f < 6; ++f) { sv[f] = ds[f]; sv[6 + f] = z[f]; }
+#pragma unroll
+    for (int jj = 0; jj < RMAX; ++jj) { sv[12 + jj] = dq[jj]; sv[12 + RMAX + jj] = rj[jj]; }
+  }
+  __builtin_amdgcn_wave_barrier();
+#pragma unroll
+  for (int j = 0; j < SJ; ++j) {
+    const int k = q + j * G;
+    float v = 0.f;
+    if (k < 6 * R) v = sv[12 + k / 6] * sv[6 + k % 6];
+    else if (k < 7 * R) v = sv[12 + (k - 6 * R)];
+    else if (k < 13 * R) v = sv[(k - 7 * R) / R] * sv[12 + RMAX + (k - 7 * R) % R];
+    else if (k < NP) v = sv[k - 13 * R];
+    acc.se[j] += v;
+  }
+  __builtin_amdgcn_wave_barrier();
+  f32x4 dx[5];
+#pragma unroll
+  for (int f = 0; f < 5; ++f) dx[f] = dv[f] * a[f + 1] + dz[f + 1] / (float)D;
+  dx0 = dx[0];
+  dx1 = dx[1];
+
+  {
+    const float mean = group_sum<G>(h[0] + h[1] + h[2] + h[3]) / (float)D;
+    const f32x4 dh = h - mean;
+    const float s2 = group_sum<G>(dh[0] * dh[0] + dh[1] * dh[1] + dh[2] * dh[2] + dh[3] * dh[3]);
+    const float rstd = 1.f / sqrtf(s2 / (float)D + p.ln_eps);
+    const f32x4 gam = *reinterpret_cast<const f32x4*>(p.ln_g + 4 * q);
+    f32x4 gl, xh, gx;
+#pragma unroll
+    for (int e = 0; e < 4; ++e) {
+      gl[e] = x[3][e] > 0.f ? dx[3][e] : 0.f;
+      xh[e] = dh[e] * rstd;
+      gx[e] = gl[e] * gam[e];
+      acc.lg[e] += gl[e] * xh[e];
+      acc.lb[e] += gl[e];
+    }
+    const float m1 = group_sum<G>(gx[0] + gx[1] + gx[2] + gx[3]) / (float)D;
+    const float m2 = group_sum<G>(gx[0] * xh[0] + gx[1] * xh[1] + gx[2] * xh[2] + gx[3] * xh[3]) / (float)D;
+    f32x4 out;
+#pragma unroll
+    for (int e = 0; e < 4; ++e) out[e] = rstd * (gx[e] - m1 - xh[e] * m2);
+    if (p.dhmm) *reinterpret_cast<f32x4*>(p.dhmm + (size_t)b * D + 4 * q) = out;
+    acc.hb += out;
+    if (p.dhmm16) {
+      const bf16x4 hi = (bf16x4){f2bf(out[0]), f2bf(out[1]), f2bf(out[2]), f2bf(out[3])};
+      *reinterpret_cast<bf16x4*>(p.dhmm16 + (size_t)b * D + 4 * q) = hi;
+      if (p.dhmm16_lo)
+        *reinterpret_cast<bf16x4*>(p.dhmm16 + p.dhmm16_lo + (size_t)b * D + 4 * q) =
+            (bf16x4){f2bf(out[0] - bf2f(hi[0])), f2bf(out[1] - bf2f(hi[1])), f2bf(out[2] - bf2f(hi[2])),
+                     f2bf(out[3] - bf2f(hi[3]))};
+    }
+  }
+  const f32x4 gh = dx[4] / in.cnt;
+  if (MODE == 0 && p.gvec) {
+    *reinterpret_cast<f32x4*>(gvec + (size_t)b * 2 * D + 4 * q) = dx[2];
+    *reinterpret_cast<f32x4*>(gvec + ((size_t)b * 2 + 1) * D + 4 * q) = gh;
+    if (p.gnorm) {
+      double si = 0.0, sh = 0.0;
+#pragma unroll
+      for (int e = 0; e < 4; ++e) {
+        si += (double)(dx[2][e] * dx[2][e]);
+        sh += (double)(gh[e] * gh[e]);
+      }
+#pragma unroll
+      for (int o = G / 2; o > 0; o >>= 1) {
+        si += __shfl_xor(si, o, 64);
+        sh += __shfl_xor(sh, o, 64);
+      }
+      if (q == 0) {
+        p.gnorm[(size_t)b * 2] = si;
+        p.gnorm[(size_t)b * 2 + 1] = sh;
+      }
+    }
+  } else if (MODE == 0) {
+    const f32x4 ti = transpose_cols<G>(dx[2], lane);
+    const f32x4 th = transpose_cols<G>(gh, lane);
+    const long long item = p.item_id[b];
+    if (item > 0 && item < p.V) atomic_add_row_t<G>(p.gtab + item * D, ti, q);
+    for (int t = 0; t < L; ++t) {
+      const long long s = p.item_seq[(size_t)b * L + t];
+      if (s > 0 && s < p.V) atomic_add_row_t<G>(p.gtab + s * D, th, q);
+    }
+  } else {
+    const int* pb = p.pos + (size_t)b * (L + 1);
+    auto put = [&](int row, const f32x4& x) {
+      if constexpr (MODE == 2) {
+        *reinterpret_cast<bf16x4*>(reinterpret_cast<short*>(p.sendbuf) + (size_t)row * D + 4 * q) =
+            (bf16x4){f2bf(x[0]), f2bf(x[1]), f2bf(x[2]), f2bf(x[3])};
+      } else {
+        *reinterpret_cast<f32x4*>(reinterpret_cast<float*>(p.sendbuf) + (size_t)row * D + 4 * q) = x;
+      }
+    };
+    if (pb[0] >= 0) put(pb[0], dx[2]);
+    for (int t = 0; t < L; ++t)
+      if (pb[t + 1] >= 0) put(pb[t + 1], gh);
+  }
+}
+
+template <int D>
+__device__ __forceinline__ void fields_bwd_cate(float* w_ct, int n_cate, int lane, bool live, long long lk,
+                                                long long vw, const f32x4& dx0, const f32x4& dx1) {
+  constexpr int G = D / 4, SPW = 64 / G;
+  const int q = lane % G, grp = lane / G;
+#pragma unroll
+  for (int gi = 0; gi < SPW; ++gi) {
+    if (grp == gi && live) {
+      if (lk >= 0 && lk < n_cate) {
+        f32x4* c = reinterpret_cast<f32x4*>(w_ct + lk * D + 4 * q);
+        *c = *c + dx0;
+      }
+      if (vw >= 0 && vw < n_cate) {
+        f32x4* c = reinterpret_cast<f32x4*>(w_ct + vw * D + 4 * q);
+        *c = *c + dx1;
+      }
+    }
+  }
+}
+
+template <int D, int RMAX>
+__device__ __forceinline__ void fields_bwd_fold(const FieldBwdArgs& p, float* sp, FieldsBwdAcc<D, RMAX>& acc) {
+  constexpr int G = D / 4;
+  constexpr int SJ = FieldsBwdAcc<D, RMAX>::SJ;
+  const int NP = 13 * p.R + 6;
+  const int P = NP + 3 * D + p.n_cate * D;
+  const int lane = threadIdx.x & 63, q = lane % G, grp = lane / G;
+  float* ws = sp + (threadIdx.x >> 6) * P;
+  float* w_lg = ws + NP;
+  float* w_hb = w_lg + 2 * D + p.n_cate * D;
+#pragma unroll
+  for (int o = G; o < 64; o <<= 1) {
+#pragma unroll
+    for (int e = 0; e < 4; ++e) {
+      acc.lg[e] += __shfl_xor(acc.lg[e], o, 64);
+      acc.lb[e] += __shfl_xor(acc.lb[e], o, 64);
+      acc.hb[e] += __shfl_xor(acc.hb[e], o, 64);
+    }
+#pragma unroll
+    for (int j = 0; j < SJ; ++j) acc.se[j] += __shfl_xor(acc.se[j], o, 64);
+  }
+  if (grp == 0) {
+    *reinterpret_cast<f32x4*>(w_lg + 4 * q) = acc.lg;
+    *reinterpret_cast<f32x4*>(w_lg + D + 4 * q) = acc.lb;
+    *reinterpret_cast<f32x4*>(w_hb + 4 * q) = acc.hb;
+#pragma unroll
+    for (int j = 0; j < SJ; ++j) {
+      const int k = q + j * G;
+      if (k < NP) ws[k] = acc.se[j];
+    }
+  }
+  __syncthreads();
+  float* out = p.partials + (size_t)blockIdx.x * P;
+  for (int i = threadIdx.x; i < P; i += blockDim.x) out[i] = (sp[i] + sp[P + i]) + (sp[2 * P + i] + sp[3 * P + i]);
+}
+
+#ifndef FBN_FB_MAXBLK
+#define FBN_FB_MAXBLK 512
+#endif
+static inline int fields_grid(int B, int D, int cap = 1024) {
+  const int spw = 64 / (D / 4);
+  const int waves = (B + spw - 1) / spw;
+  int blocks = (waves + 3) / 4;
+  return blocks < 1 ? 1 : (blocks > cap ? cap : blocks);
+}
+static inline size_t fields_bwd_lds(int D, int R, int n_cate, int rmax) {
+  return (4 * (size_t)(13 * R + 6 + 3 * D + n_cate * D) + 4 * (64 / (D / 4)) * (12 + 2 * rmax)) * sizeof(float);
+}
+int fbn_fields_reduce_partials(const float* partials, float* const* param_grads, int B, int D, int R, int n_cate,
+                               hipStream_t st);
diff --git a/ctr_recommendation_amd/csrc/plan_thunks.inc b/ctr_recommendation_amd/csrc/plan_thunks.inc
--- a/ctr_recommendation_amd/csrc/plan_thunks.inc
+++ b/ctr_recommendation_amd/csrc/plan_thunks.inc
@@ -358,6 +358,49 @@
       static_cast<int>(i[9]),
       reinterpret_cast<void*>(static_cast<uintptr_t>(i[10])));
 }
+static int th_fbn_bilinear_fields_bwd(const uint64_t* i, const double* f) {
+  return fbn_bilinear_fields_bwd(reinterpret_cast<const void*>(static_cast<uintptr_t>(i[0])),
+      static_cast<int>(i[1]),
+      reinterpret_cast<const short*>(static_cast<uintptr_t>(i[2])),
+      reinterpret_cast<const short*>(static_cast<uintptr_t>(i[3])),
+      reinterpret_cast<const short*>(static_cast<uintptr_t>(i[4])),
+      reinterpret_cast<short*>(static_cast<uintptr_t>(i[5])),
+      reinterpret_cast<const int64_t*>(static_cast<uintptr_t>(i[6])),
+      reinterpret_cast<const int64_t*>(static_cast<uintptr_t>(i[7])),
+      reinterpret_cast<const float*>(static_cast<uintptr_t>(i[8])),
+      reinterpret_cast<const float*>(static_cast<uintptr_t>(i[9])),
+      reinterpret_cast<const float*>(static_cast<uintptr_t>(i[10])),
+      plan_f32(f[0]),
+      reinterpret_cast<const float*>(static_cast<uintptr_t>(i[11])),
+      reinterpret_cast<const float*>(static_cast<uintptr_t>(i[12])),
+      reinterpret_cast<const float*>(static_cast<uintptr_t>(i[13])),
+      static_cast<int>(i[14]),
+      static_cast<int>(i[15]),
+      reinterpret_cast<const float*>(static_cast<uintptr_t>(i[16])),
+      reinterpret_cast<const float*>(static_cast<uintptr_t>(i[17])),
+      reinterpret_cast<const float*>(static_cast<uintptr_t>(i[18])),
+      reinterpret_cast<const float*>(static_cast<uintptr_t>(i[19])),
+      reinterpret_cast<float*>(static_cast<uintptr_t>(i[20])),
+      reinterpret_cast<short*>(static_cast<uintptr_t>(i[21])),
+      reinterpret_cast<float*>(static_cast<uintptr_t>(i[22])),
+      reinterpret_cast<float* const*>(static_cast<uintptr_t>(i[23])),
+      reinterpret_cast<float*>(static_cast<uintptr_t>(i[24])),
+      reinterpret_cast<const int*>(static_cast<uintptr_t>(i[25])),
+      reinterpret_cast<void*>(static_cast<uintptr_t>(i[26])),
+      static_cast<int>(i[27]),
+      static_cast<long long>(i[28]),
+      reinterpret_cast<double*>(static_cast<uintptr_t>(i[29])),
+      static_cast<int>(i[30]),
+      static_cast<int>(i[31]),
+      reinterpret_cast<void*>(static_cast<uintptr_t>(i[32])));
+}
+static int th_fbn_bilinear_fields_bwd_supported(const uint64_t* i, const double* f) {
+  (void)f;
+  return fbn_bilinear_fields_bwd_supported(static_cast<int>(i[0]),
+      static_cast<int>(i[1]),
+      static_cast<int>(i[2]),
+      static_cast<int>(i[3]));
+}
 static int th_fbn_bilinear_fwd(const uint64_t* i, const double* f) {
   (void)f;
   return fbn_bilinear_fwd(reinterpret_cast<const short*>(static_cast<uintptr_t>(i[0])),
@@ -1808,6 +1851,8 @@
     {"fbn_adam_table", th_fbn_adam_table, 15, 3},
     {"fbn_adam_touched", th_fbn_adam_touched, 15, 3},
     {"fbn_bilinear_bwd", th_fbn_bilinear_bwd, 11, 0},
+    {"fbn_bilinear_fields_bwd", th_fbn_bilinear_fields_bwd, 33, 1},
+    {"fbn_bilinear_fields_bwd_supported", th_fbn_bilinear_fields_bwd_supported, 4, 0},
     {"fbn_bilinear_fwd", th_fbn_bilinear_fwd, 7, 0},
     {"fbn_bilinear_supported", th_fbn_bilinear_supported, 1, 0},
     {"fbn_bn_act_fwd", th_fbn_bn_act_fwd, 14, 1},
diff --git a/ctr_recommendation_amd/ops.py b/ctr_recommendation_amd/ops.py
--- a/ctr_recommendation_amd/ops.py
+++ b/ctr_recommendation_amd/ops.py
@@ -23,6 +23,7 @@
 _SPLIT_BWD = os.environ.get("FBN_SPLIT_BWD", "0") == "1"
 _SPLIT3 = os.environ.get("FBN_SPLIT3", "1") != "0"
 _BN1_BWD_IN_GEMM = os.environ.get("FBN_BN1_BWD_IN_GEMM", "1") == "1"
+_FIELDS_IN_BILINEAR = os.environ.get("FBN_FIELDS_IN_BILINEAR", "1") == "1"
 
 
 def wa_remap(d: int):
@@ -803,10 +804,18 @@
         dc = torch.empty((B, KC), **f32)
         gemm(dh1pre, p["mlp.0.weight"], dc, B, KC, H1, H1, 21 * d, KC, False, False, rB=wa_remap(d), bf16=sb,
              stream=st)
-    dV = tmp("dV", (B, 5, d))
+    R = cfg.R
+    ncate = p["cate_emb.weight"].shape[0]
+    fields_in_bil = bool(_FIELDS_IN_BILINEAR and a.get("fused_bilinear") and pos is None
+                         and not (hooks and "after_bilinear_bwd" in hooks)
+                         and (gvec is not None or gslot is not None)
+                         and _lib.lib().fbn_bilinear_fields_bwd_supported(B, d, R, ncate))
+    dV = None if fields_in_bil else tmp("dV", (B, 5, d))
     v16 = bf and not cfg.bilinear_each
     dU16 = tmp("dU16", (B, 5, d), torch.bfloat16) if v16 else None
-    if a.get("fused_bilinear"):
+    if fields_in_bil:
+        pass
+    elif a.get("fused_bilinear"):
         call("fbn_bilinear_bwd", ptr(dc), KC, int(dc.dtype == torch.bfloat16), ptr(a["Vc16"]), ptr(w16["WT"]),
              ptr(w16["W"]), ptr(dV), ptr(dU16), B, d, st)
         if not sums.gemm_slabs(a["Vc16"], dU16, g["bilinear.W"], d, d, 5 * B, d, d, d, True, False, stream=st):
@@ -850,12 +859,10 @@
                  bf16=cfg.bf16, stream=st)
     if hooks and "after_bilinear_bwd" in hooks:
         hooks["after_bilinear_bwd"](sums)
-    R = cfg.R
-    ncate = p["cate_emb.weight"].shape[0]
     P = _lib.lib().fbn_fields_bwd_partials_size(d, R, ncate)
     nblk = _lib.lib().fbn_fields_bwd_grid(B, d)
     partials = tmp("partials", (nblk, P))
-    dhmm = tmp("dhmm", (B, d))
+    dhmm = None if fields_in_bil else tmp("dhmm", (B, d))
     dhmm16 = tmp("dhmm16", (B, d), torch.bfloat16) if bf else None
     dhs = img("dhmm", B, d) if s3 else None
     seq = batch.get("item_seq", None)
@@ -874,7 +881,15 @@
         _lib.keep(outs_arr)
         outs = ctypes.cast(outs_arr, ctypes.c_void_p).value
     evb = _probe_start(probe, "fields_bwd")
-    if gslot is not None:
+    if fields_in_bil:
+        ring, ring_n, ring_stride, step, cell = gslot if gslot is not None else (gvec, 0, 0, None, None)
+        call("fbn_bilinear_fields_bwd", ptr(dc), KC, ptr(a["Vc16"]), ptr(w16["WT"]), ptr(w16["W"]), ptr(dU16),
+             ptr(batch["likes_level"]), ptr(batch["views_level"]), ptr(a["hmm"]), ptr(p["mm_proj.1.weight"]),
+             ptr(p["mm_proj.1.bias"]), LN_EPS, ptr(p["senet.excitation.0.weight"]),
+             ptr(p["senet.excitation.0.bias"]), ptr(p["senet.excitation.2.weight"]), R, ncate,
+             ptr(p["cate_emb.weight"]), ptr(a["X"]), ptr(a["a"]), ptr(a["cnt"]), None, ptr(dhmm16), ptr(partials),
+             outs, ptr(ring), ptr(step), ptr(cell), ring_n, ring_stride, ptr(gnorm), B, d, st)
+    elif gslot is not None:
         ring, ring_n, ring_stride, step, cell = gslot
         call("fbn_fields_bwd_slot", ptr(batch["item_id"]), ptr(seq) if Lr else None, ptr(batch["likes_level"]),
              ptr(batch["views_level"]), ptr(a["hmm"]), ptr(p["mm_proj.1.weight"]), ptr(p["mm_proj.1.bias"]), LN_EPS,
@@ -895,6 +910,9 @@
     _probe_end(evb)
     if hooks and "after_fields_bwd" in hooks:
         hooks["after_fields_bwd"]()
+    if fields_in_bil:
+        if not sums.gemm_slabs(a["Vc16"], dU16, g["bilinear.W"], d, d, 5 * B, d, d, d, True, False, stream=st):
+            wg.run(lambda s: gemm(a["Vc16"], dU16, g["bilinear.W"], d, d, 5 * B, d, d, d, True, False, stream=s))
     if bf:
         if not sums.gemm_slabs(dhmm16, w16["x"], g["mm_proj.0.weight"], d, 128, B, d, 128, 128, True, False,
                                stream=st):
diff --git a/include/fibinet.h b/include/fibinet.h
--- a/include/fibinet.h
+++ b/include/fibinet.h
@@ -270,6 +270,14 @@
 int fbn_bilinear_fwd(const short* V16, const short* WT16, short* c, int B, int D, int ldc, void* stream);
 int fbn_bilinear_bwd(const void* dc, int ldc, int dc_bf16, const short* V16, const short* WT16, const short* W16,
                      float* dV, short* dU16, int B, int D, void* stream);
+int fbn_bilinear_fields_bwd_supported(int B, int D, int R, int n_cate);
+int fbn_bilinear_fields_bwd(const void* dc, int ldc, const short* V16, const short* WT16, const short* W16,
+                            short* dU16, const int64_t* likes, const int64_t* views, const float* hmm,
+                            const float* ln_g, const float* ln_b, float ln_eps, const float* w1, const float* b1,
+                            const float* w2, int R, int n_cate, const float* cate, const float* X, const float* a,
+                            const float* cnt, float* dhmm, short* dhmm16, float* partials,
+                            float* const* param_grads, float* gvec, const int* slot_step, void* slot_cell, int ring_n,
+                            long long ring_stride, double* gnorm, int B, int D, void* stream);
 
 int fbn_collate(const int64_t* perm, int B, const int64_t* item, const int64_t* seq, int Ls, int L,
                 const int64_t* likes, const int64_t* views, const int64_t* user, const float* label,
```

New measurement: 21.03 million samples/s, median of 6. 1.03x the previous value.
